# sabarim/STEm-Seg

Measured on AMD Instinct MI355X. Metric: clips/sec (T=8, 480p) embed+cluster, higher is better.
Workload: dtype f16x3: fp32 emulated from 2 fp16 terms per operand (22-bit operand significands; fp32 has 24), power-of-two operand scaling, 3 fp16 MFMA products per fp32 product, fp32 accumulate; |activation| >= 2.6e5 -> non-finite, flagged on the device, clip re-run in bf16x6

## Files before the change

### include/stemseg_hip.h

```cpp
#ifndef STEMSEG_HIP_H
#define STEMSEG_HIP_H

#include <stddef.h>
#include <stdint.h>

#ifdef __cplusplus
extern "C" {
#endif

#define STEMSEG_HIP_ABI_VERSION 11

#define STEMSEG_OK              0
#define STEMSEG_E_INVALID      -1
#define STEMSEG_E_HIP          -2
#define STEMSEG_E_WORKSPACE    -3
#define STEMSEG_E_UNSUPPORTED  -4

#define STEMSEG_MAX_HEAD_OUT   10
#define STEMSEG_MAX_INSTANCES  64
#define STEMSEG_MAX_EMB_DIMS    8
#define STEMSEG_MAX_SEMSEG_CLASSES 128

int         stemseg_hip_version(void);
const char* stemseg_hip_last_error(void);
// ... 62 lines not shown
int stemseg_hip_heads(const float* x, int32_t Cin, int32_t T, int32_t H, int32_t W,
                      const float* w, const float* bias, int32_t n_out, const int32_t* act_host,
                      const int32_t* grid_axis_host, const float* grid_t, const float* grid_y, const float* grid_x,
                      float* out, void* stream);

int stemseg_hip_nonfinite_flags(const float* x, int64_t n, int32_t* flags, int32_t n_flags, void* stream);

typedef struct StemsegDecoderDesc {
    int32_t struct_bytes;
    int32_t in_channels;
    int32_t inter[4];
    int32_t T, H4, W4;
    int32_t gn_groups;
    float   gn_eps;
    int32_t pool[3];
    int32_t t_scale[3];
    int32_t n_out;
    int32_t act[STEMSEG_MAX_EMB_DIMS * 2];
    int32_t grid_axis[STEMSEG_MAX_EMB_DIMS * 2];
    int32_t input_layout;
    int32_t concurrency;
    int32_t detached;
    int32_t precision;
    int32_t n_clips;
    int64_t feat_clip_stride[4];
    int64_t out_clip_stride;
} StemsegDecoderDesc;

typedef struct StemsegDecoderWeights {
    const float* conv_w[7];
    const float* conv_b[7];
    const float* gn_w[7];
    const float* gn_b[7];
    const float* fuse_w[3];
    const float* head_w;
    const float* head_b;
    const float* grid_t;
    const float* grid_y;
    const float* grid_x;
} StemsegDecoderWeights;

size_t stemseg_hip_decoder_workspace_bytes(const StemsegDecoderDesc* desc);
int stemseg_hip_decoder_init_workspace(const StemsegDecoderDesc* desc, void* workspace, size_t ws_bytes, void* stream);
int stemseg_hip_decoder_check_workspace(const StemsegDecoderDesc* desc, const void* workspace, size_t ws_bytes, int32_t* n_bad_host,
                                        int64_t* first_bad_host, void* stream);
int stemseg_hip_decoder_forward(const StemsegDecoderDesc* desc, const StemsegDecoderWeights* weights,
                                const float* const feats[4], float* out,
                                void* workspace, size_t ws_bytes, void* stream);

int stemseg_hip_decoder_join(int32_t concurrency, void* stream);

#define STEMSEG_MAX_ENCODER_BLOCKS 40

typedef struct StemsegEncoderDesc {
    int32_t struct_bytes;
    int32_t blocks[4];
    int32_t T, H, W;
    int32_t out_channels;
    int32_t precision;
    int32_t n_clips;
    int32_t clip_frames;
    int32_t clip_stride;
    int32_t plan_frames;
    int32_t fuse_tail;
    int32_t conv2_groups;
    int32_t width_per_group;
    int32_t stride_in_3x3;
} StemsegEncoderDesc;

typedef struct StemsegEncoderWeights {
    const float* stem_w;
    const float* stem_b;
    const float* stem_w_s2d;
    const float* conv1_w[STEMSEG_MAX_ENCODER_BLOCKS];   const float* conv1_b[STEMSEG_MAX_ENCODER_BLOCKS];
    const float* conv2_w[STEMSEG_MAX_ENCODER_BLOCKS];   const float* conv2_b[STEMSEG_MAX_ENCODER_BLOCKS];
    const float* conv3_w[STEMSEG_MAX_ENCODER_BLOCKS];   const float* conv3_b[STEMSEG_MAX_ENCODER_BLOCKS];
    const float* down_w[STEMSEG_MAX_ENCODER_BLOCKS];    const float* down_b[STEMSEG_MAX_ENCODER_BLOCKS];
    const float* fpn_inner_w[4]; const float* fpn_inner_b[4];
    const float* fpn_layer_w[4]; const float* fpn_layer_b[4];
} StemsegEncoderWeights;

size_t stemseg_hip_encoder_workspace_bytes(const StemsegEncoderDesc* desc);
int stemseg_hip_encoder_plan_offsets(const StemsegEncoderDesc* desc, int64_t* out25);

int stemseg_hip_stem_conv(const float* frames, const float* w_tap_major, const float* bias, float* out, int32_t T, int32_t H, int32_t W,
                          void* stream);
int stemseg_hip_encoder_init_workspace(const StemsegEncoderDesc* desc, void* workspace, size_t ws_bytes, void* stream);
int stemseg_hip_encoder_check_workspace(const StemsegEncoderDesc* desc, const void* workspace, size_t ws_bytes, int32_t* n_bad_host,
                                        int64_t* first_bad_host, void* stream);
int stemseg_hip_encoder_forward(const StemsegEncoderDesc* desc, const StemsegEncoderWeights* weights, const float* frames,
                                const StemsegVolume* out, void* workspace, size_t ws_bytes, void* stream);


int stemseg_hip_seediness_accumulate(float* acc, const float* plane, int64_t n, int32_t first, void* stream);
int stemseg_hip_fg_mask(const float* acc, float count, float thr, uint8_t* mask, int64_t n, void* stream);
int stemseg_hip_fg_mask_frames(const float* acc, const float* counts, float thr, uint8_t* mask, int32_t F, int64_t HW,
                               void* stream);

int stemseg_hip_fg_gather(const float* emb, const float* bw, const float* seed, const uint8_t* fg,
                          int32_t E, int32_t Ev, int32_t T, int64_t HW,
                          float* emb_out, float* bw_out, float* seed_out, int32_t* voxel_index,
                          int64_t* frame_offsets, void* scratch, void* stream);

typedef struct StemsegClusterParams {
    float   primary_prob_thresh;
    float   secondary_prob_thresh;
    float   min_seediness_prob;
    int32_t max_instances;
    int32_t n_free_dims;
    float   free_dim_bandwidths[STEMSEG_MAX_EMB_DIMS];
} StemsegClusterParams;

typedef struct StemsegClusterMeta {
    int32_t K;
    int32_t exhausted;
    int64_t n_points;
    int64_t n_unassigned_last;
    float   centers[STEMSEG_MAX_INSTANCES][STEMSEG_MAX_EMB_DIMS];
    float   bandwidths[STEMSEG_MAX_INSTANCES][STEMSEG_MAX_EMB_DIMS];
    float   seed_prob[STEMSEG_MAX_INSTANCES];
} StemsegClusterMeta;

size_t stemseg_hip_cluster_workspace_bytes(int64_t n_max);
int stemseg_hip_cluster(const float* emb, const float* bw, const float* seed, int64_t n_max,
                        const int64_t* n_points_dev, int32_t E, int32_t Ev,
                        const StemsegClusterParams* params, int64_t label_start,
                        int64_t* labels, StemsegClusterMeta* meta_dev,
                        uint8_t* opt_masks, float* opt_probs,
                        void* workspace, size_t ws_bytes, void* stream);

typedef struct StemsegClusterItem {
    const float*   emb;
    const float*   bw;
    const float*   seed;
    int64_t        n_max;
    const int64_t* n_points_dev;
    int64_t        label_start;
    int64_t*       labels;
    StemsegClusterMeta* meta_dev;
    uint8_t*       opt_masks;
    float*         opt_probs;
    void*          workspace;
    size_t         ws_bytes;
} StemsegClusterItem;
int stemseg_hip_cluster_batch(const StemsegClusterItem* items, int32_t n_items, int32_t E, int32_t Ev,
                              const StemsegClusterParams* params, void* stream);

int stemseg_hip_overlap_counts(const int64_t* labels_a, const int64_t* labels_b, int64_t n,
                               const int32_t* lut_a, int32_t lut_a_len, const int32_t* lut_b, int32_t lut_b_len,
                               int32_t Ka, int32_t Kb, int64_t* inter, int64_t* cnt_a, int64_t* cnt_b, void* stream);

int stemseg_hip_label_presence(const int64_t* labels, int64_t n, uint8_t* present, int32_t cap,
                               int64_t* max_plus_1, int32_t accumulate, void* stream);

int stemseg_hip_relabel(int64_t* labels, int64_t n, const int64_t* map, int32_t map_len, void* stream);


int stemseg_hip_fg_compact(const uint8_t* fg, int32_t T, int64_t HW, int32_t* voxel_index, int64_t* frame_offsets, void* scratch,
                           void* stream);

int stemseg_hip_labels_to_codes(const int64_t* labels, const int32_t* voxel_index, const int64_t* n_points_dev, int64_t n_max,
                                int64_t label_start, uint8_t* codes, int64_t V, void* stream);

int stemseg_hip_pair_tables(const uint8_t* codes, const int32_t* plane_a, const int32_t* plane_b, int32_t n_items, int64_t HW,
                            int32_t B, int32_t* tables, void* stream);

// ... 131 lines not shown
```

### stem-seg_amd/csrc/bottleneck_fused.hip

```cpp
#include "common.h"
#include "split_operand.h"

namespace stemseg {

typedef float f32x16 __attribute__((ext_vector_type(16)));
typedef _Float16 f16x8 __attribute__((ext_vector_type(8)));
typedef unsigned int u32x4 __attribute__((ext_vector_type(4)));

struct FusedTailParams {
    const unsigned int* x16;
    const char* w3;
    const float* b3;
    const float* res;
    float* y;
    const char* w1;
    const float* b1;
    float* z;
    int64_t z_cs, z_ts, z_ys;
    int dec_H, dec_W;
    int V;
    const float* xs;
    const char* wd;
    const float* bd;
};

constexpr SplitLayout FT_WL = SplitLayout(1, STEMSEG_PRECISION_F16X3);
static_assert(FT_WL.CK == 32 && FT_WL.G == 2 && FT_WL.NPL == 2, "the fused tail walks 32-channel chunks of two k-groups, two planes");

template <int MID_, int CT_, int P_, int DS_ = 0>
struct FusedTailCfg {
    static constexpr int MID = MID_, CT = CT_, COUT = 4 * MID_;
    static constexpr int DS = DS_, NCD = DS_ / 32;
    static constexpr int P = P_, NW = P_ / 32, NTHREADS = 64 * NW;
    static constexpr int NC3 = MID / 32;
    static constexpr int NCT = COUT / CT;
    static constexpr int MI3 = CT / 32, MI1 = MID / 32;
    static constexpr int NH = 2 * MI3;
    static constexpr int X_BYTES = 2 * 4 * P * 16;
    static constexpr int W3_BYTES = 8 * CT * 16;
    static constexpr int W1_HALF = 4 * MID * 16;
    static constexpr int LDS_BYTES = 2 * X_BYTES + 2 * W3_BYTES + 2 * W1_HALF;
    static constexpr int NQ = P / 64;
    static constexpr int X_PIECES = X_BYTES / 1024, W3_PIECES = W3_BYTES / 1024, W1_PIECES = W1_HALF / 1024;
    static_assert(NC3 == FT_WL.chunks(MID) && W3_BYTES == FT_WL.slab_bytes(CT, 32) && W1_HALF * FT_WL.G == FT_WL.slab_bytes(MID, 32), "tile byte sizes follow the packed-weight layout");
    static_assert(P % 64 == 0 && MID % 32 == 0 && CT % 32 == 0 && COUT % CT == 0, "tile shapes");
    static_assert(LDS_BYTES <= (P <= 128 ? 80 : 160) * 1024, "LDS: two 128-position workgroups, or one 256-position workgroup, per CU");
    static_assert(W3_BYTES % 1024 == 0 && W1_HALF % 1024 == 0 && X_PIECES % NW == 0, "whole DMA pieces");
    static_assert(MI1 * 16 + MI3 * 16 + (DS ? MI3 * 16 : 0) <= 176, "accumulators must leave room for fragments at 256 registers");
    static_assert(DS % 32 == 0 && 2 * CT * 4 <= W1_HALF, "shortcut: whole K-chunks; its (1 / scale, bias) table waits in a w1 buffer");
};

template <class C>
__global__ __launch_bounds__(C::NTHREADS, 2) void fused_tail_kernel(const FusedTailParams p) {
#pragma clang fp contract(off)
    __shared__ __attribute__((aligned(1024))) char smem[C::LDS_BYTES];
    char* const xbuf = smem;
    char* const w3buf = smem + 2 * C::X_BYTES;
    char* const w1buf = smem + 2 * C::X_BYTES + 2 * C::W3_BYTES;

    const int tid = threadIdx.x, lane = tid & 63;
    const int wave = __builtin_amdgcn_readfirstlane(tid >> 6);
    const int half = lane >> 5, l31 = lane & 31;
    const int pos0 = blockIdx.x * C::P;
    const int pos = pos0 + wave * 32 + l31;
    const bool pos_ok = pos < p.V;
    const int pos_c = min(pos, p.V - 1);
    const int64_t V = p.V;
    const unsigned int lane_off = (unsigned int)(((int64_t)(4 * half) * V + pos_c) * 4);
    auto opaque = [](unsigned int v) __attribute__((always_inline)) { asm volatile("" : "+v"(v)); return v; };

    typedef const __attribute__((address_space(1))) void* gptr_t;
    typedef __attribute__((address_space(3))) void* lptr_t;
    const float* inv3 = reinterpret_cast<const float*>(p.w3 + FT_WL.inv_offset(C::COUT, C::MID));
    const float* inv1 = reinterpret_cast<const float*>(p.w1 + FT_WL.inv_offset(C::MID, C::COUT));

    const int xpos = min(pos0 + lane, p.V - 1);
    auto dma_x = [&](const int c, const int buf) __attribute__((always_inline)) {
#pragma unroll
        for (int k = 0; k < C::X_PIECES / C::NW; ++k) {
            const int idx = wave * (C::X_PIECES / C::NW) + k, q = idx % C::NQ, o = (idx / C::NQ) & 3, pl = idx / (4 * C::NQ);
            const unsigned int xp = (unsigned int)min((int)opaque((unsigned int)xpos) + q * 64, p.V - 1);
            const char* src = reinterpret_cast<const char*>(p.x16) + ((int64_t)(pl * (C::MID / 8) + 4 * c + o)) * V * 16 + (size_t)(xp * 16u);
            __builtin_amdgcn_global_load_lds((gptr_t)src, (lptr_t)(xbuf + buf * C::X_BYTES + ((pl * 4 + o) * C::P + q * 64) * 16), 16, 0, 0);
        }
    };
    auto dma_wc = [&](const char* blob, const int j, const int c, const int buf) __attribute__((always_inline)) {
        constexpr int PER_ROW = C::CT * 16 / 1024;
#pragma unroll
        for (int k = 0; k < (C::W3_PIECES + C::NW - 1) / C::NW; ++k) {
            const int idx = wave + k * C::NW;
            if (idx < C::W3_PIECES) {
                const int row = idx / PER_ROW, part = idx % PER_ROW;
                const char* src = blob + ((int64_t)c * 8 + row) * (C::COUT * 16) + (int64_t)j * (C::CT * 16) + part * 1024 + (size_t)(opaque((unsigned int)lane) * 16u);
                __builtin_amdgcn_global_load_lds((gptr_t)src, (lptr_t)(w3buf + buf * C::W3_BYTES + idx * 1024), 16, 0, 0);
            }
        }
    };
    auto dma_w3 = [&](const int j, const int c, const int buf) __attribute__((always_inline)) { dma_wc(p.w3, j, c, buf); };
    auto dma_wd = [&](const int j, const int c, const int buf) __attribute__((always_inline)) { dma_wc(p.wd, j, c, buf); };
    auto dma_w1 = [&](const int j, const int h, const int buf) __attribute__((always_inline)) {
#pragma unroll
        for (int k = 0; k < (C::W1_PIECES + C::NW - 1) / C::NW; ++k) {
            const int idx = wave + k * C::NW;
            if (idx < C::W1_PIECES) {
                const char* src = p.w1 + ((int64_t)j * C::NH + h) * C::W1_HALF + (int64_t)idx * 1024 + (size_t)(opaque((unsigned int)lane) * 16u);
                __builtin_amdgcn_global_load_lds((gptr_t)src, (lptr_t)(w1buf + buf * C::W1_HALF + idx * 1024), 16, 0, 0);
            }
        }
    };
    auto dma_tab = [&](const int j, const int buf) __attribute__((always_inline)) {
        static_assert(2 * (C::CT / 4) <= 64 && 2 * C::CT * 4 <= C::W3_BYTES, "the table is one DMA piece");
        if (wave == 0 && lane < 2 * (C::CT / 4)) {
            const unsigned int l = opaque((unsigned int)lane);
            const float* src = (l < C::CT / 4 ? inv3 : p.b3 - C::CT) + (int64_t)j * C::CT + (size_t)(l * 4u);
            __builtin_amdgcn_global_load_lds((gptr_t)src, (lptr_t)(w3buf + buf * C::W3_BYTES), 16, 0, 0);
        }
    };
    auto dma_dtab = [&](const int j) __attribute__((always_inline)) {
        if (wave == 0 && lane < 2 * (C::CT / 4)) {
            const unsigned int l = opaque((unsigned int)lane);
            const float* invd = reinterpret_cast<const float*>(p.wd + FT_WL.inv_offset(C::COUT, C::DS));
            const float* src = (l < C::CT / 4 ? invd : p.bd - C::CT) + (int64_t)j * C::CT + (size_t)(l * 4u);
            __builtin_amdgcn_global_load_lds((gptr_t)src, (lptr_t)(w1buf + C::W1_HALF), 16, 0, 0);
        }
    };
    constexpr int NXS = C::DS > 0 ? C::DS / 2 : 1;
    auto load_xs = [&](float (&xr)[NXS]) __attribute__((always_inline)) {
        const unsigned int V4 = (unsigned int)p.V * 4u;
        const __amdgpu_buffer_rsrc_t rs = __builtin_amdgcn_make_buffer_rsrc(const_cast<float*>(p.xs), 0, (int)((unsigned int)C::DS * V4), 0x00020000);
        const unsigned int off = (unsigned int)(8 * half) * V4 + (unsigned int)pos_c * 4u;
#pragma unroll
        for (int i = 0; i < C::DS / 2; ++i)
            xr[i] = __builtin_bit_cast(float, __builtin_amdgcn_raw_buffer_load_b32(rs, off, (unsigned int)(16 * (i >> 3) + (i & 7)) * V4, 0));
    };
    auto dma_tail_tab = [&]() __attribute__((always_inline)) {
        constexpr int PIECES = (2 * C::MID + 255) / 256;
        if (wave < PIECES) {
            const unsigned int f0 = (unsigned int)wave * 256u + opaque((unsigned int)lane) * 4u;
            if (f0 < 2u * C::MID) {
                const float* src = (f0 < (unsigned int)C::MID ? inv1 : p.b1 - C::MID) + (size_t)f0;
                __builtin_amdgcn_global_load_lds((gptr_t)src, (lptr_t)(xbuf + wave * 1024), 16, 0, 0);
            }
        }
    };
    auto stage_sync = [&]() __attribute__((always_inline)) {
        __builtin_amdgcn_s_waitcnt(0x0f70);
        __syncthreads();
    };
    auto load_identity = [&](const int co_first, float (&rres)[16]) __attribute__((always_inline)) {
#pragma unroll
        for (int r = 0; r < 16; ++r)
            rres[r] = *reinterpret_cast<const float*>(reinterpret_cast<const char*>(p.res + (int64_t)(co_first + (r & 3) + 8 * (r >> 2)) * V) + (size_t)lane_off);
    };

    f32x16 acc1[C::MI1];
#pragma unroll
    for (int m = 0; m < C::MI1; ++m)
#pragma unroll
        for (int r = 0; r < 16; ++r) acc1[m][r] = 0.f;

    const f16x8 k2048 = {(_Float16)(1.0f / F16X3_LO_SCALE), (_Float16)(1.0f / F16X3_LO_SCALE), (_Float16)(1.0f / F16X3_LO_SCALE), (_Float16)(1.0f / F16X3_LO_SCALE),
                         (_Float16)(1.0f / F16X3_LO_SCALE), (_Float16)(1.0f / F16X3_LO_SCALE), (_Float16)(1.0f / F16X3_LO_SCALE), (_Float16)(1.0f / F16X3_LO_SCALE)};

    auto mma3 = [&](f32x16& acc, const f16x8 a_hi, const f16x8 a_lo, const f16x8 b_hi, const f16x8 b_lo) __attribute__((always_inline)) {
        const f16x8 a_his = a_hi * k2048;
        acc = __builtin_amdgcn_mfma_f32_32x32x16_f16(a_lo, b_hi, acc, 0, 0, 0);
        acc = __builtin_amdgcn_mfma_f32_32x32x16_f16(a_his, b_lo, acc, 0, 0, 0);
        acc = __builtin_amdgcn_mfma_f32_32x32x16_f16(a_hi, b_hi, acc, 0, 0, 0);
    };

    constexpr bool DSV = C::DS > 0;
    float xr[NXS];
    if constexpr (DSV) { dma_wd(0, 0, 0); load_xs(xr); }
    else { dma_x(0, 0); dma_w3(0, 0, 0); }
    stage_sync();
    int sb = 0;
#pragma unroll 1
    for (int j = 0; j < C::NCT; ++j) {
        f32x16 accd[DSV ? C::MI3 : 1];
        if constexpr (DSV) {
            f16x8 d_hi[2 * C::NCD], d_lo[2 * C::NCD];
#pragma unroll
            for (int G = 0; G < 2 * C::NCD; ++G) {
                u32x4 hw4, lw4;
#pragma unroll
                for (int i = 0; i < 4; ++i) {
                    unsigned int hwd, lwd;
                    split_pair_f16(xr[8 * G + 2 * i], xr[8 * G + 2 * i + 1], hwd, lwd);
                    hw4[i] = hwd; lw4[i] = lwd;
                }
                d_hi[G] = __builtin_bit_cast(f16x8, hw4);
                d_lo[G] = __builtin_bit_cast(f16x8, lw4);
            }
#pragma unroll
            for (int m = 0; m < C::MI3; ++m)
#pragma unroll
                for (int r = 0; r < 16; ++r) accd[m][r] = 0.f;
#pragma unroll
            for (int c = 0; c < C::NCD; ++c) {
                if (c + 1 < C::NCD) dma_wd(j, c + 1, sb ^ 1);
                else { dma_x(0, sb ^ 1); dma_w3(j, 0, sb ^ 1); }
                if (c == 0) dma_dtab(j);
                const char* wb = w3buf + sb * C::W3_BYTES + (half * C::CT + l31) * 16;
                constexpr int NS = 2 * C::MI3;
                f16x8 a_hi[2], a_lo[2];
                auto ld_a = [&](const int st, const int k) __attribute__((always_inline)) {
                    const int g = st / C::MI3, m = st % C::MI3;
                    a_hi[k] = *reinterpret_cast<const f16x8*>(wb + (((g * 2 + 0) * 2) * C::CT + m * 32) * 16);
                    a_lo[k] = *reinterpret_cast<const f16x8*>(wb + (((g * 2 + 1) * 2) * C::CT + m * 32) * 16);
                };
                ld_a(0, 0);
#pragma unroll
                for (int st = 0; st < NS; ++st) {
                    if (st + 1 < NS) ld_a(st + 1, (st + 1) & 1);
                    __builtin_amdgcn_sched_barrier(0);
                    mma3(accd[st % C::MI3], a_hi[st & 1], a_lo[st & 1], d_hi[2 * c + st / C::MI3], d_lo[2 * c + st / C::MI3]);
                    __builtin_amdgcn_sched_barrier(0);
                }
                stage_sync();
                sb ^= 1;
            }
            const float* dtab = reinterpret_cast<const float*>(w1buf + C::W1_HALF);
#pragma unroll
            for (int m = 0; m < C::MI3; ++m)
#pragma unroll
                for (int q = 0; q < 4; ++q) {
                    const float4 sc = *reinterpret_cast<const float4*>(dtab + m * 32 + 8 * q + 4 * half);
                    const float4 bv = *reinterpret_cast<const float4*>(dtab + C::CT + m * 32 + 8 * q + 4 * half);
                    accd[m][4 * q + 0] = __fadd_rn(__fmul_rn(accd[m][4 * q + 0], sc.x), bv.x);
                    accd[m][4 * q + 1] = __fadd_rn(__fmul_rn(accd[m][4 * q + 1], sc.y), bv.y);
                    accd[m][4 * q + 2] = __fadd_rn(__fmul_rn(accd[m][4 * q + 2], sc.z), bv.z);
                    accd[m][4 * q + 3] = __fadd_rn(__fmul_rn(accd[m][4 * q + 3], sc.w), bv.w);
                }
#pragma unroll
            for (int m = 0; m < C::MI3; ++m) asm volatile("" : "+v"(accd[m]));
            __builtin_amdgcn_sched_barrier(0);
        }
        f32x16 acc3[C::MI3];
#pragma unroll
        for (int m = 0; m < C::MI3; ++m)
#pragma unroll
            for (int r = 0; r < 16; ++r) acc3[m][r] = 0.f;
        const int co_j = j * C::CT;
        float rres[16];
#pragma unroll 1
        for (int c = 0; c < C::NC3; ++c) {
            if (c + 1 < C::NC3) { dma_x(c + 1, sb ^ 1); dma_w3(j, c + 1, sb ^ 1); }
            else { dma_w1(j, 0, 0); dma_tab(j, sb ^ 1); if constexpr (!DSV) load_identity(co_j, rres); }
            const char* xb = xbuf + sb * C::X_BYTES + (half * C::P + wave * 32 + l31) * 16;
            const char* wb = w3buf + sb * C::W3_BYTES + (half * C::CT + l31) * 16;
            constexpr int NS = 2 * C::MI3;
            f16x8 b_hi[2], b_lo[2], a_hi[2], a_lo[2];
            auto ld_b = [&](const int g, const int k) __attribute__((always_inline)) {
                b_hi[k] = *reinterpret_cast<const f16x8*>(xb + ((0 * 4 + 2 * g) * C::P) * 16);
                b_lo[k] = *reinterpret_cast<const f16x8*>(xb + ((1 * 4 + 2 * g) * C::P) * 16);
            };
            auto ld_a = [&](const int st, const int k) __attribute__((always_inline)) {
                const int g = st / C::MI3, m = st % C::MI3;
                a_hi[k] = *reinterpret_cast<const f16x8*>(wb + (((g * 2 + 0) * 2) * C::CT + m * 32) * 16);
                a_lo[k] = *reinterpret_cast<const f16x8*>(wb + (((g * 2 + 1) * 2) * C::CT + m * 32) * 16);
            };
            ld_b(0, 0);
            ld_b(1, 1);
            ld_a(0, 0);
#pragma unroll
            for (int st = 0; st < NS; ++st) {
                if (st + 1 < NS) ld_a(st + 1, (st + 1) & 1);
                __builtin_amdgcn_sched_barrier(0);
                mma3(acc3[st % C::MI3], a_hi[st & 1], a_lo[st & 1], b_hi[st / C::MI3], b_lo[st / C::MI3]);
                __builtin_amdgcn_sched_barrier(0);
            }
            stage_sync();
            sb ^= 1;
        }
        f16x8 b_hi[2], b_lo[2];
#pragma unroll
        for (int h = 0; h < C::NH; ++h) {
            const int m = h >> 1, g = h & 1;
            if (g == 0) {
                const int co_m = co_j + m * 32;
                unsigned int hw[8], lw[8];
                const float* tab = reinterpret_cast<const float*>(w3buf + sb * C::W3_BYTES);
                if constexpr (DSV) {
#pragma unroll
                    for (int r = 0; r < 16; ++r) rres[r] = accd[m][r];
                }
                __builtin_amdgcn_sched_barrier(0);
#pragma unroll
                for (int q = 0; q < 4; ++q) {
                    const int co4 = co_m + 8 * q + 4 * half;
                    const float4 sc = *reinterpret_cast<const float4*>(tab + (co4 - co_j));
                    const float4 bv = *reinterpret_cast<const float4*>(tab + C::CT + (co4 - co_j));
                    float v0 = __fmul_rn(acc3[m][4 * q + 0], sc.x), v1 = __fmul_rn(acc3[m][4 * q + 1], sc.y), v2 = __fmul_rn(acc3[m][4 * q + 2], sc.z),
                          v3 = __fmul_rn(acc3[m][4 * q + 3], sc.w);
                    v0 = relu_keep_nan(__fadd_rn(__fadd_rn(v0, bv.x), rres[4 * q + 0]));
                    v1 = relu_keep_nan(__fadd_rn(__fadd_rn(v1, bv.y), rres[4 * q + 1]));
                    v2 = relu_keep_nan(__fadd_rn(__fadd_rn(v2, bv.z), rres[4 * q + 2]));
                    v3 = relu_keep_nan(__fadd_rn(__fadd_rn(v3, bv.w), rres[4 * q + 3]));
                    if (pos_ok) {
                        char* yo = reinterpret_cast<char*>(p.y + (int64_t)(co_m + 8 * q) * V);
                        *reinterpret_cast<float*>(yo + (size_t)lane_off) = v0;
                        *reinterpret_cast<float*>(yo + V * 4 + (size_t)lane_off) = v1;
                        *reinterpret_cast<float*>(yo + V * 8 + (size_t)lane_off) = v2;
                        *reinterpret_cast<float*>(yo + V * 12 + (size_t)lane_off) = v3;
                    }
                    split_pair_f16(v0, v1, hw[2 * q], lw[2 * q]);
                    split_pair_f16(v2, v3, hw[2 * q + 1], lw[2 * q + 1]);
                }
                __builtin_amdgcn_sched_barrier(0);
#pragma unroll
                for (int gg = 0; gg < 2; ++gg) {
                    unsigned int xh[2], yh[2], xl[2], yl[2];
#pragma unroll
                    for (int i = 0; i < 2; ++i) {
                        auto sh = __builtin_amdgcn_permlane32_swap(hw[4 * gg + i], hw[4 * gg + 2 + i], false, false);
                        xh[i] = sh[0]; yh[i] = sh[1];
                        auto sl = __builtin_amdgcn_permlane32_swap(lw[4 * gg + i], lw[4 * gg + 2 + i], false, false);
                        xl[i] = sl[0]; yl[i] = sl[1];
                    }
                    const u32x4 bh = {xh[0], xh[1], yh[0], yh[1]}, bl = {xl[0], xl[1], yl[0], yl[1]};
                    b_hi[gg] = __builtin_bit_cast(f16x8, bh);
                    b_lo[gg] = __builtin_bit_cast(f16x8, bl);
                }
            } else if (m + 1 < C::MI3) {
                if constexpr (!DSV) load_identity(co_j + (m + 1) * 32, rres);
            }
            __builtin_amdgcn_sched_barrier(0);
            if (h + 1 < C::NH) dma_w1(j, h + 1, (h + 1) & 1);
            else if (j + 1 < C::NCT) {
                if constexpr (DSV) { dma_wd(j + 1, 0, sb); load_xs(xr); }
                else { dma_x(0, sb); dma_w3(j + 1, 0, sb); }
            } else dma_tail_tab();
            const char* w1b = w1buf + (h & 1) * C::W1_HALF + (half * C::MID + l31) * 16;
            f16x8 a_hi[2], a_lo[2];
            auto ld_a1 = [&](const int m1, const int k) __attribute__((always_inline)) {
                a_hi[k] = *reinterpret_cast<const f16x8*>(w1b + ((0 * 2) * C::MID + m1 * 32) * 16);
                a_lo[k] = *reinterpret_cast<const f16x8*>(w1b + ((1 * 2) * C::MID + m1 * 32) * 16);
            };
            ld_a1(0, 0);
#pragma unroll
            for (int m1 = 0; m1 < C::MI1; ++m1) {
                if (m1 + 1 < C::MI1) ld_a1(m1 + 1, (m1 + 1) & 1);
                __builtin_amdgcn_sched_barrier(0);
                mma3(acc1[m1], a_hi[m1 & 1], a_lo[m1 & 1], b_hi[g], b_lo[g]);
                __builtin_amdgcn_sched_barrier(0);
            }
            stage_sync();
        }
    }
    if (pos_ok) {
        const int hwp = p.dec_H * p.dec_W;
        const int t2 = pos / hwp, r2 = pos - t2 * hwp, y2 = r2 / p.dec_W, x2 = r2 - y2 * p.dec_W;
        const unsigned int z_off = (unsigned int)(((int64_t)(4 * half) * p.z_cs + (int64_t)t2 * p.z_ts + (int64_t)y2 * p.z_ys + x2) * 4);
#pragma unroll
        for (int m1 = 0; m1 < C::MI1; ++m1)
#pragma unroll
            for (int q = 0; q < 4; ++q) {
                const int co4 = m1 * 32 + 8 * q + 4 * half;
                const float4 sc = *reinterpret_cast<const float4*>(reinterpret_cast<const float*>(xbuf) + co4);
                const float4 bv = *reinterpret_cast<const float4*>(reinterpret_cast<const float*>(xbuf) + C::MID + co4);
                char* zo = reinterpret_cast<char*>(p.z + (int64_t)(m1 * 32 + 8 * q) * p.z_cs);
                *reinterpret_cast<float*>(zo + (size_t)z_off) = relu_keep_nan(__fadd_rn(__fmul_rn(acc1[m1][4 * q + 0], sc.x), bv.x));
                *reinterpret_cast<float*>(zo + p.z_cs * 4 + (size_t)z_off) = relu_keep_nan(__fadd_rn(__fmul_rn(acc1[m1][4 * q + 1], sc.y), bv.y));
                *reinterpret_cast<float*>(zo + p.z_cs * 8 + (size_t)z_off) = relu_keep_nan(__fadd_rn(__fmul_rn(acc1[m1][4 * q + 2], sc.z), bv.z));
                *reinterpret_cast<float*>(zo + p.z_cs * 12 + (size_t)z_off) = relu_keep_nan(__fadd_rn(__fmul_rn(acc1[m1][4 * q + 3], sc.w), bv.w));
            }
    }
}


typedef float f32x4 __attribute__((ext_vector_type(4)));

template <int MID_>
struct FusedTail16Cfg {
    static constexpr int MID = MID_, COUT = 4 * MID_, CT = 128;
    static constexpr int NW = 8, NTHREADS = 512, P = 16 * NW;
    static constexpr int NC3 = MID / 32, NCT = COUT / CT;
    static constexpr int NT3 = CT / 16, NT1 = MID / 16;
    static constexpr int SC = 2;
    static constexpr int NS = NC3 / SC, NU = CT / 32;
    static constexpr int W3_CHUNK = 8 * CT * 16;
    static constexpr int W3_BYTES = SC * W3_CHUNK;
    static constexpr int W1_BYTES = 8 * MID * 16;
    static constexpr int TAB_BYTES = 2 * CT * 4;
    static constexpr int LDS_BYTES = 2 * W3_BYTES + 2 * W1_BYTES + 2 * TAB_BYTES;
    static_assert(NC3 % SC == 0 && W3_BYTES % (1024 * NW) == 0 && W1_BYTES % (1024 * NW) == 0 && TAB_BYTES == 1024, "whole DMA pieces per wave");
    static_assert(W3_CHUNK == FT_WL.slab_bytes(CT, FT_WL.CK) && W1_BYTES == FT_WL.slab_bytes(MID, FT_WL.CK), "tile byte sizes follow the packed-weight layout");
    static_assert(LDS_BYTES <= 160 * 1024 && 2 * MID * 4 <= W3_BYTES, "LDS");
};

template <class C>
__global__ __launch_bounds__(C::NTHREADS, 2) void fused_tail16_kernel(const FusedTailParams p) {
#pragma clang fp contract(off)
    __shared__ __attribute__((aligned(1024))) char smem[C::LDS_BYTES];
    char* const w3buf = smem;
    char* const w1buf = smem + 2 * C::W3_BYTES;
    char* const tabbuf = smem + 2 * C::W3_BYTES + 2 * C::W1_BYTES;

    const int tid = threadIdx.x, lane = tid & 63;
    const int wave = __builtin_amdgcn_readfirstlane(tid >> 6);
    const int n = lane & 15, kb = lane >> 4;
    const int pos = blockIdx.x * C::P + wave * 16 + n;
    const bool pos_ok = pos < p.V;
    const int pos_c = min(pos, p.V - 1);
    const int64_t V = p.V;
    const unsigned int lane_off = (unsigned int)(((int64_t)(4 * kb) * V + pos_c) * 4);
    auto opaque = [](unsigned int v) __attribute__((always_inline)) { asm volatile("" : "+v"(v)); return v; };
    typedef const __attribute__((address_space(1))) void* gptr_t;
    typedef __attribute__((address_space(3))) void* lptr_t;
    const float* inv3 = reinterpret_cast<const float*>(p.w3 + FT_WL.inv_offset(C::COUT, C::MID));
    const float* inv1 = reinterpret_cast<const float*>(p.w1 + FT_WL.inv_offset(C::MID, C::COUT));

    auto dma_w3 = [&](const int j, const int st, const int buf) __attribute__((always_inline)) {
        constexpr int PER_ROW = C::CT * 16 / 1024, PER_CHUNK = C::W3_CHUNK / 1024;
#pragma unroll
        for (int k = 0; k < C::W3_BYTES / 1024 / C::NW; ++k) {
            const int idx = wave + k * C::NW, sc = idx / PER_CHUNK, r = idx % PER_CHUNK, row = r / PER_ROW, part = r % PER_ROW;
            const char* src = p.w3 + ((int64_t)(st * C::SC + sc) * 8 + row) * (C::COUT * 16) + (int64_t)j * (C::CT * 16) + part * 1024 + (size_t)(opaque((unsigned int)lane) * 16u);
            __builtin_amdgcn_global_load_lds((gptr_t)src, (lptr_t)(w3buf + buf * C::W3_BYTES + idx * 1024), 16, 0, 0);
        }
    };
    auto dma_w1 = [&](const int cc, const int buf) __attribute__((always_inline)) {
#pragma unroll
        for (int k = 0; k < C::W1_BYTES / 1024 / C::NW; ++k) {
            const int idx = wave + k * C::NW;
            const char* src = p.w1 + (int64_t)cc * C::W1_BYTES + (int64_t)idx * 1024 + (size_t)(opaque((unsigned int)lane) * 16u);
            __builtin_amdgcn_global_load_lds((gptr_t)src, (lptr_t)(w1buf + buf * C::W1_BYTES + idx * 1024), 16, 0, 0);
        }
    };
    auto dma_tab = [&](const int j) __attribute__((always_inline)) {
        if (wave == 0) {
            const unsigned int l = opaque((unsigned int)lane);
            const float* src = (l < 32 ? inv3 : p.b3 - C::CT) + (int64_t)j * C::CT + (size_t)(l * 4u);
            __builtin_amdgcn_global_load_lds((gptr_t)src, (lptr_t)(tabbuf + (j & 1) * C::TAB_BYTES), 16, 0, 0);
        }
    };
    auto dma_tail_tab = [&]() __attribute__((always_inline)) {
        constexpr int PIECES = (2 * C::MID + 255) / 256;
        if (wave < PIECES) {
            const unsigned int f0 = (unsigned int)wave * 256u + opaque((unsigned int)lane) * 4u;
            if (f0 < 2u * C::MID) {
                const float* src = (f0 < (unsigned int)C::MID ? inv1 : p.b1 - C::MID) + (size_t)f0;
                __builtin_amdgcn_global_load_lds((gptr_t)src, (lptr_t)(w3buf + wave * 1024), 16, 0, 0);
            }
        }
    };
    auto stage_sync = [&]() __attribute__((always_inline)) {
        __builtin_amdgcn_s_waitcnt(0x0f70);
// ... 74 lines not shown
#pragma unroll
            for (int tt = 0; tt < 2; ++tt) {
                const int t = 2 * u + tt, co4 = 16 * t + 4 * kb;
                const float4 sc = *reinterpret_cast<const float4*>(tab + co4);
                const float4 bv = *reinterpret_cast<const float4*>(tab + C::CT + co4);
                float v0 = __fmul_rn(acc3[t][0], sc.x), v1 = __fmul_rn(acc3[t][1], sc.y), v2 = __fmul_rn(acc3[t][2], sc.z), v3 = __fmul_rn(acc3[t][3], sc.w);
                v0 = relu_keep_nan(__fadd_rn(__fadd_rn(v0, bv.x), rres[4 * tt + 0]));
                v1 = relu_keep_nan(__fadd_rn(__fadd_rn(v1, bv.y), rres[4 * tt + 1]));
                v2 = relu_keep_nan(__fadd_rn(__fadd_rn(v2, bv.z), rres[4 * tt + 2]));
                v3 = relu_keep_nan(__fadd_rn(__fadd_rn(v3, bv.w), rres[4 * tt + 3]));
                if (pos_ok) {
                    char* yo = reinterpret_cast<char*>(p.y + (int64_t)(co_j + 16 * t) * V);
                    *reinterpret_cast<float*>(yo + (size_t)lane_off) = v0;
                    *reinterpret_cast<float*>(yo + V * 4 + (size_t)lane_off) = v1;
                    *reinterpret_cast<float*>(yo + V * 8 + (size_t)lane_off) = v2;
                    *reinterpret_cast<float*>(yo + V * 12 + (size_t)lane_off) = v3;
                }
                split_pair_f16(v0, v1, hw[2 * tt], lw[2 * tt]);
                split_pair_f16(v2, v3, hw[2 * tt + 1], lw[2 * tt + 1]);
            }
            unsigned int bw[2][4];
#pragma unroll
            for (int pl = 0; pl < 2; ++pl)
#pragma unroll
                for (int i = 0; i < 2; ++i) {
                    const unsigned int t0 = pl ? lw[i] : hw[i], t1 = pl ? lw[2 + i] : hw[2 + i];
                    auto s32 = __builtin_amdgcn_permlane32_swap(t0, t1, false, false);
                    auto s16 = __builtin_amdgcn_permlane16_swap(s32[0], s32[1], false, false);
                    bw[pl][i] = s16[0];
                    bw[pl][2 + i] = s16[1];
                }
            const u32x4 bh = {bw[0][0], bw[0][1], bw[0][2], bw[0][3]}, bl = {bw[1][0], bw[1][1], bw[1][2], bw[1][3]};
            const f16x8 b_hi = __builtin_bit_cast(f16x8, bh), b_lo = __builtin_bit_cast(f16x8, bl);
            __builtin_amdgcn_sched_barrier(0);
            if (u + 1 < C::NU) { dma_w1(j * C::NU + u + 1, eb ^ 1); load_identity(co_j + 32 * (u + 1), rres); }
            else if (j + 1 < C::NCT) dma_w3(j + 1, 0, sb);
            else dma_tail_tab();
            __builtin_amdgcn_sched_barrier(0);
            const char* w1b = w1buf + eb * C::W1_BYTES + (((kb >> 1) * 2 * 2 + (kb & 1)) * C::MID + n) * 16;
            f16x8 a_hi[1][2], a_lo[1][2];
            auto ld_a1 = [&](const int i, const int k) __attribute__((always_inline)) {
#pragma unroll
                for (int e = 0; e < 2; ++e) {
                    a_hi[k][e] = *reinterpret_cast<const f16x8*>(w1b + (0 * 2 * C::MID + (2 * i + e) * 16) * 16);
                    a_lo[k][e] = *reinterpret_cast<const f16x8*>(w1b + (1 * 2 * C::MID + (2 * i + e) * 16) * 16);
                }
            };
#pragma unroll
            for (int i = 0; i < C::NT1 / 2; ++i) {
                ld_a1(i, 0);
                __builtin_amdgcn_sched_barrier(0);
                mma3x2(acc1[2 * i], acc1[2 * i + 1], a_hi[0][0], a_lo[0][0], a_hi[0][1], a_lo[0][1], b_hi, b_lo);
                __builtin_amdgcn_sched_barrier(0);
            }
            stage_sync();
            eb ^= 1;
        }
    }
    if (pos_ok) {
        const int hwp = p.dec_H * p.dec_W;
        const int t2 = pos / hwp, r2 = pos - t2 * hwp, y2 = r2 / p.dec_W, x2 = r2 - y2 * p.dec_W;
        const unsigned int z_off = (unsigned int)(((int64_t)(4 * kb) * p.z_cs + (int64_t)t2 * p.z_ts + (int64_t)y2 * p.z_ys + x2) * 4);
        const float* ttab = reinterpret_cast<const float*>(w3buf);
#pragma unroll
        for (int m1 = 0; m1 < C::NT1; ++m1) {
            const int co4 = m1 * 16 + 4 * kb;
            const float4 sc = *reinterpret_cast<const float4*>(ttab + co4);
            const float4 bv = *reinterpret_cast<const float4*>(ttab + C::MID + co4);
            char* zo = reinterpret_cast<char*>(p.z + (int64_t)(m1 * 16) * p.z_cs);
            *reinterpret_cast<float*>(zo + (size_t)z_off) = relu_keep_nan(__fadd_rn(__fmul_rn(acc1[m1][0], sc.x), bv.x));
            *reinterpret_cast<float*>(zo + p.z_cs * 4 + (size_t)z_off) = relu_keep_nan(__fadd_rn(__fmul_rn(acc1[m1][1], sc.y), bv.y));
            *reinterpret_cast<float*>(zo + p.z_cs * 8 + (size_t)z_off) = relu_keep_nan(__fadd_rn(__fmul_rn(acc1[m1][2], sc.z), bv.z));
            *reinterpret_cast<float*>(zo + p.z_cs * 12 + (size_t)z_off) = relu_keep_nan(__fadd_rn(__fmul_rn(acc1[m1][3], sc.w), bv.w));
        }
    }
}


typedef __amdgpu_buffer_rsrc_t ft_rsrc_t;
#define FT_VMCNT_(n) __builtin_amdgcn_s_waitcnt(((n) & 15) | (((n) >> 4) << 14) | 0x0F70)
#define FT_VMCNT(n) FT_VMCNT_(n)
#define FT_SGB(mask, n) __builtin_amdgcn_sched_group_barrier(mask, n, 0)

template <int MID_, int CT_, int DS_ = 0>
struct FusedTailR1Cfg {
    static constexpr int MID = MID_, CT = CT_, COUT = 4 * MID_;
    static constexpr int DS = DS_, NGD = DS_ / 16;
    static constexpr int NW = 4, NTHREADS = 64 * NW, P = 32 * NW;
    static constexpr int NC3 = MID / 32, NG = MID / 16, NCT = COUT / CT;
    static constexpr int MI3 = CT / 32, MI1 = MID / 32;
    static constexpr int SC = 2;
    static constexpr int NS = NC3 / SC, NU = CT / 32;
    static constexpr int NSD = DS / 32 / SC;
    static_assert(DS % (32 * SC) == 0, "shortcut: whole stages");
    static constexpr int NX3 = SC * 2 * (MI3 / 2), NX1 = 2 * (MI1 / 2);
    static constexpr int W3_CHUNK = 8 * CT * 16, W3_BYTES = SC * W3_CHUNK;
    static constexpr int W1_BYTES = 8 * MID * 16;
    static_assert(W3_CHUNK == FT_WL.slab_bytes(CT, FT_WL.CK) && W1_BYTES == FT_WL.slab_bytes(MID, FT_WL.CK), "tile byte sizes follow the packed-weight layout");
    static constexpr int TAB_BYTES = 1024;
    static constexpr int LDS_BYTES = 2 * W3_BYTES + 2 * W1_BYTES + 2 * TAB_BYTES;
    static constexpr int W3_PIECES = W3_BYTES / 1024 / NW, W1_PIECES = W1_BYTES / 1024 / NW;
    static constexpr int SL = 8 / NX1, S0 = NX1 / 4, M_PPS = 8 / S0;
    static_assert(NC3 % SC == 0 && MI3 % 2 == 0 && MI1 % 2 == 0 && W3_BYTES % (1024 * NW) == 0 && W1_BYTES % (1024 * NW) == 0 && 2 * CT * 4 <= TAB_BYTES, "whole DMA pieces per wave");
    static_assert(LDS_BYTES <= 160 * 1024 && 2 * MID * 4 <= W3_BYTES && (NX1 == 8 || NX1 == 4) && NX3 == 8 && MI3 == 4 && NS >= 2 && NU >= 2 && NU % 2 == 0, "LDS / slice placement / identity buffer parity");
    static_assert(W3_PIECES == 8 && W1_PIECES <= 8, "the pieces of a stage are requested in its first steps");
    static_assert(NG * 8 + MI1 * 16 <= 256, "the conv3 input and conv1's accumulators are the AGPR half of the register file");
};

template <class C>
__global__ __launch_bounds__(C::NTHREADS, 1) void fused_tail_r1_kernel(const FusedTailParams p) {
#pragma clang fp contract(off)
    __shared__ __attribute__((aligned(1024))) char smem[C::LDS_BYTES];
    char* const w3buf = smem;
    char* const w1buf = smem + 2 * C::W3_BYTES;
    char* const tabbuf = smem + 2 * C::W3_BYTES + 2 * C::W1_BYTES;

    const int tid = threadIdx.x, lane = tid & 63;
    const int wave = __builtin_amdgcn_readfirstlane(tid >> 6);
    const int half = lane >> 5, l31 = lane & 31;
    const int pos = blockIdx.x * C::P + wave * 32 + l31;
    const bool pos_ok = pos < p.V;
    const int pos_c = min(pos, p.V - 1);
    const int64_t V = p.V;
    const unsigned int V4 = (unsigned int)p.V * 4u;
    const unsigned int lane_ld = (unsigned int)(4 * half) * V4 + (unsigned int)pos_c * 4u;
    const unsigned int lane_st = pos_ok ? lane_ld : 0xFFFFFF00u;
    const unsigned int tile_bytes = (unsigned int)C::CT * V4;
    typedef __attribute__((address_space(3))) void* lptr_t;
    const float* inv3 = reinterpret_cast<const float*>(p.w3 + FT_WL.inv_offset(C::COUT, C::MID));
    const float* inv1 = reinterpret_cast<const float*>(p.w1 + FT_WL.inv_offset(C::MID, C::COUT));

    const unsigned int lane16 = (unsigned int)lane * 16u;
    const unsigned int lds_w3 = (unsigned int)(uintptr_t)(lptr_t)w3buf, lds_w1 = (unsigned int)(uintptr_t)(lptr_t)w1buf;
    auto dma_piece = [&](const char* sbase, const unsigned int lds_addr) __attribute__((always_inline)) {
        asm volatile("s_mov_b32 m0, %0\n\ts_nop 0\n\tglobal_load_lds_dwordx4 %1, %2" : : "s"(lds_addr), "v"(lane16), "s"(sbase) : "memory");
    };
    auto dma_w3 = [&](const int j, const int st, const int buf, const int k) __attribute__((always_inline)) {
        constexpr int PER_ROW = C::CT * 16 / 1024, PER_CHUNK = C::W3_CHUNK / 1024;
        const int idx = wave + k * C::NW, sc = idx / PER_CHUNK, r = idx % PER_CHUNK, row = r / PER_ROW, part = r % PER_ROW;
        dma_piece(p.w3 + ((int64_t)(st * C::SC + sc) * 8 + row) * (C::COUT * 16) + (int64_t)j * (C::CT * 16) + part * 1024, lds_w3 + buf * C::W3_BYTES + idx * 1024);
    };
    auto dma_wd = [&](const int j, const int st, const int buf, const int k) __attribute__((always_inline)) {
        constexpr int PER_ROW = C::CT * 16 / 1024, PER_CHUNK = C::W3_CHUNK / 1024;
        const int idx = wave + k * C::NW, sc = idx / PER_CHUNK, r = idx % PER_CHUNK, row = r / PER_ROW, part = r % PER_ROW;
        dma_piece(p.wd + ((int64_t)(st * C::SC + sc) * 8 + row) * (C::COUT * 16) + (int64_t)j * (C::CT * 16) + part * 1024, lds_w3 + buf * C::W3_BYTES + idx * 1024);
    };
    auto dma_w1 = [&](const int cc, const int buf, const int k) __attribute__((always_inline)) {
        const int idx = wave + k * C::NW;
        dma_piece(p.w1 + (int64_t)cc * C::W1_BYTES + (int64_t)idx * 1024, lds_w1 + buf * C::W1_BYTES + idx * 1024);
    };
    float4 tabv = {0.f, 0.f, 0.f, 0.f};
    auto tab_fetch = [&](const int j) __attribute__((always_inline)) {
        if (wave == 0 && lane < 2 * (C::CT / 4))
            tabv = *reinterpret_cast<const float4*>((lane < C::CT / 4 ? inv3 : p.b3 - C::CT) + (int64_t)j * C::CT + lane * 4);
    };
    auto tab_store = [&](const int j) __attribute__((always_inline)) {
        if (wave == 0 && lane < 2 * (C::CT / 4)) *reinterpret_cast<float4*>(tabbuf + (j & 1) * C::TAB_BYTES + lane * 16) = tabv;
    };
    constexpr bool DSV = C::DS > 0;
    float4 tabdv = {0.f, 0.f, 0.f, 0.f};
    auto tabd_fetch = [&](const int j) __attribute__((always_inline)) {
        const float* invd = reinterpret_cast<const float*>(p.wd + FT_WL.inv_offset(C::COUT, C::DS));
        if (wave == 0 && lane < 2 * (C::CT / 4))
            tabdv = *reinterpret_cast<const float4*>((lane < C::CT / 4 ? invd : p.bd - C::CT) + (int64_t)j * C::CT + lane * 4);
    };
    auto tabd_store = [&](const int j) __attribute__((always_inline)) {
        if (wave == 0 && lane < 2 * (C::CT / 4)) *reinterpret_cast<float4*>(tabbuf + ((j + 1) & 1) * C::TAB_BYTES + lane * 16) = tabdv;
    };
    auto rsrc_of = [&](const float* base, const int jj) __attribute__((always_inline)) {
        return __builtin_amdgcn_make_buffer_rsrc(const_cast<float*>(base + (int64_t)jj * C::CT * V), 0, (int)tile_bytes, 0x00020000);
    };
    auto load_identity = [&](const int jj, const int u, float (&rr)[16]) __attribute__((always_inline)) {
        const ft_rsrc_t rs = rsrc_of(p.res, jj);
#pragma unroll
        for (int r = 0; r < 16; ++r)
            rr[r] = __builtin_bit_cast(float, __builtin_amdgcn_raw_buffer_load_b32(rs, lane_ld, (unsigned int)(32 * u + (r & 3) + 8 * (r >> 2)) * V4, 0));
    };
    const f16x8 k2048 = {(_Float16)(1.0f / F16X3_LO_SCALE), (_Float16)(1.0f / F16X3_LO_SCALE), (_Float16)(1.0f / F16X3_LO_SCALE), (_Float16)(1.0f / F16X3_LO_SCALE),
                         (_Float16)(1.0f / F16X3_LO_SCALE), (_Float16)(1.0f / F16X3_LO_SCALE), (_Float16)(1.0f / F16X3_LO_SCALE), (_Float16)(1.0f / F16X3_LO_SCALE)};
    auto mma6 = [&](f32x16& c0, f32x16& c1, const f16x8 (&a_hi)[2], const f16x8 (&a_lo)[2], const f16x8 (&a_his)[2], const f16x8 b_hi, const f16x8 b_lo)
        __attribute__((always_inline)) {
        c0 = __builtin_amdgcn_mfma_f32_32x32x16_f16(a_lo[0], b_hi, c0, 0, 0, 0);
        c1 = __builtin_amdgcn_mfma_f32_32x32x16_f16(a_lo[1], b_hi, c1, 0, 0, 0);
        c0 = __builtin_amdgcn_mfma_f32_32x32x16_f16(a_his[0], b_lo, c0, 0, 0, 0);
        c1 = __builtin_amdgcn_mfma_f32_32x32x16_f16(a_his[1], b_lo, c1, 0, 0, 0);
        c0 = __builtin_amdgcn_mfma_f32_32x32x16_f16(a_hi[0], b_hi, c0, 0, 0, 0);
        c1 = __builtin_amdgcn_mfma_f32_32x32x16_f16(a_hi[1], b_hi, c1, 0, 0, 0);
    };

#pragma unroll
    for (int k = 0; k < C::W3_PIECES; ++k) {
        if constexpr (DSV) dma_wd(0, 0, 0, k);
        else dma_w3(0, 0, 0, k);
    }
    float rres[2][16];
    if constexpr (!DSV) {
        load_identity(0, 0, rres[0]);
        load_identity(0, 1, rres[1]);
    }
    f16x8 xh[C::NG], xl[C::NG];
    {
        const char* xs = reinterpret_cast<const char*>(p.x16) + (size_t)((unsigned int)pos_c * 16u);
#pragma unroll
        for (int G = 0; G < C::NG; ++G) {
            xh[G] = *reinterpret_cast<const f16x8*>(xs + ((int64_t)(2 * G + half)) * V * 16);
            xl[G] = *reinterpret_cast<const f16x8*>(xs + ((int64_t)(C::MID / 8 + 2 * G + half)) * V * 16);
        }
    }
    f16x8 xdh[DSV ? C::NGD : 1], xdl[DSV ? C::NGD : 1];
    if constexpr (DSV) {
        const ft_rsrc_t rx = __builtin_amdgcn_make_buffer_rsrc(const_cast<float*>(p.xs), 0, (int)((unsigned int)C::DS * V4), 0x00020000);
        const unsigned int lane_xs = (unsigned int)(8 * half) * V4 + (unsigned int)pos_c * 4u;
#pragma unroll
// ... 14 lines not shown
    }
    f32x16 acc1[C::MI1];
#pragma unroll
    for (int m = 0; m < C::MI1; ++m)
#pragma unroll
        for (int r = 0; r < 16; ++r) acc1[m][r] = 0.f;
    FT_VMCNT(0);
    __syncthreads();
    int sb = 0, eb = 0;
#pragma unroll 1
    for (int j = 0; j < C::NCT; ++j) {
        f32x16 accd[DSV ? C::MI3 : 1];
        if constexpr (DSV) {
#pragma unroll
            for (int m = 0; m < C::MI3; ++m)
#pragma unroll
                for (int r = 0; r < 16; ++r) accd[m][r] = 0.f;
#pragma unroll
            for (int st = 0; st < C::NSD; ++st) {
                if (st == 0) tabd_fetch(j);
                const char* wb = w3buf + sb * C::W3_BYTES + (half * C::CT + l31) * 16;
                f16x8 a_hi[3][2], a_lo[3][2], a_his[2][2];
                auto ld3 = [&](const int s, const int k) __attribute__((always_inline)) {
                    const int mp = s / (2 * C::SC), sc = (s % (2 * C::SC)) / 2, g = s % 2;
#pragma unroll
                    for (int e = 0; e < 2; ++e) {
                        a_hi[k][e] = *reinterpret_cast<const f16x8*>(wb + sc * C::W3_CHUNK + (((g * 2 + 0) * 2) * C::CT + (2 * mp + e) * 32) * 16);
                        a_lo[k][e] = *reinterpret_cast<const f16x8*>(wb + sc * C::W3_CHUNK + (((g * 2 + 1) * 2) * C::CT + (2 * mp + e) * 32) * 16);
                    }
                };
                ld3(0, 0);
                ld3(1, 1);
                a_his[0][0] = a_hi[0][0] * k2048;
                a_his[0][1] = a_hi[0][1] * k2048;
#pragma unroll
                for (int s = 0; s < C::NX3; ++s) {
                    __builtin_amdgcn_sched_barrier(0);
                    if (s < 2) {
#pragma unroll
                        for (int k = 4 * s; k < 4 * s + 4; ++k) {
                            if (st + 1 < C::NSD) dma_wd(j, st + 1, sb ^ 1, k);
                            else dma_w3(j, 0, sb ^ 1, k);
                        }
                    }
                    if (s + 2 < C::NX3) ld3(s + 2, (s + 2) % 3);
                    if (s + 1 < C::NX3) {
                        a_his[(s + 1) & 1][0] = a_hi[(s + 1) % 3][0] * k2048;
                        a_his[(s + 1) & 1][1] = a_hi[(s + 1) % 3][1] * k2048;
                    }
                    const int mp = s / (2 * C::SC), sc = (s % (2 * C::SC)) / 2, g = s % 2, G = 2 * (st * C::SC + sc) + g;
                    mma6(accd[2 * mp], accd[2 * mp + 1], a_hi[s % 3], a_lo[s % 3], a_his[s & 1], xdh[G], xdl[G]);
#pragma unroll
                    for (int i = 0; i < 6; ++i) { FT_SGB(0x008, 1); FT_SGB(0x100, 1); FT_SGB(0x002, 2); }
                }
                __builtin_amdgcn_sched_barrier(0);
                FT_VMCNT(0);
                if (st == 0) tabd_store(j);
                __syncthreads();
                sb ^= 1;
            }
            const float* tabd = reinterpret_cast<const float*>(tabbuf + ((j + 1) & 1) * C::TAB_BYTES) + 4 * half;
#pragma unroll
            for (int u = 0; u < C::MI3; ++u)
#pragma unroll
                for (int q4 = 0; q4 < 4; ++q4) {
                    const float4 sc = *reinterpret_cast<const float4*>(tabd + 32 * u + 8 * q4);
                    const float4 bv = *reinterpret_cast<const float4*>(tabd + C::CT + 32 * u + 8 * q4);
                    accd[u][4 * q4 + 0] = __fadd_rn(__fmul_rn(accd[u][4 * q4 + 0], sc.x), bv.x);
                    accd[u][4 * q4 + 1] = __fadd_rn(__fmul_rn(accd[u][4 * q4 + 1], sc.y), bv.y);
                    accd[u][4 * q4 + 2] = __fadd_rn(__fmul_rn(accd[u][4 * q4 + 2], sc.z), bv.z);
                    accd[u][4 * q4 + 3] = __fadd_rn(__fmul_rn(accd[u][4 * q4 + 3], sc.w), bv.w);
                }
#pragma unroll
            for (int u = 0; u < C::MI3; ++u) asm volatile("" : "+v"(accd[u]));
            __builtin_amdgcn_sched_barrier(0);
        }
        f32x16 acc3[C::MI3];
#pragma unroll
        for (int m = 0; m < C::MI3; ++m)
#pragma unroll
            for (int r = 0; r < 16; ++r) acc3[m][r] = 0.f;
        const float* tab = reinterpret_cast<const float*>(tabbuf + (j & 1) * C::TAB_BYTES) + 4 * half;
        const ft_rsrc_t ry = rsrc_of(p.y, j);
        unsigned int hw[8], lw[8];
        f16x8 b_hi[2][2], b_lo[2][2];
        auto e_slice = [&](const int u, const int q4) __attribute__((always_inline)) {
            const int c4 = 32 * u + 8 * q4;
            const float4 sc = *reinterpret_cast<const float4*>(tab + c4);
            const float4 bv = *reinterpret_cast<const float4*>(tab + C::CT + c4);
            float rr[4];
#pragma unroll
            for (int i = 0; i < 4; ++i) rr[i] = DSV ? accd[DSV ? u : 0][4 * q4 + i] : rres[u & 1][4 * q4 + i];
            float v0 = __fmul_rn(acc3[u][4 * q4 + 0], sc.x), v1 = __fmul_rn(acc3[u][4 * q4 + 1], sc.y), v2 = __fmul_rn(acc3[u][4 * q4 + 2], sc.z),
                  v3 = __fmul_rn(acc3[u][4 * q4 + 3], sc.w);
            v0 = relu_keep_nan(__fadd_rn(__fadd_rn(v0, bv.x), rr[0]));
            v1 = relu_keep_nan(__fadd_rn(__fadd_rn(v1, bv.y), rr[1]));
            v2 = relu_keep_nan(__fadd_rn(__fadd_rn(v2, bv.z), rr[2]));
            v3 = relu_keep_nan(__fadd_rn(__fadd_rn(v3, bv.w), rr[3]));
            __builtin_amdgcn_raw_buffer_store_b32(__builtin_bit_cast(unsigned int, v0), ry, lane_st, (unsigned int)(c4 + 0) * V4, 0);
            __builtin_amdgcn_raw_buffer_store_b32(__builtin_bit_cast(unsigned int, v1), ry, lane_st, (unsigned int)(c4 + 1) * V4, 0);
            __builtin_amdgcn_raw_buffer_store_b32(__builtin_bit_cast(unsigned int, v2), ry, lane_st, (unsigned int)(c4 + 2) * V4, 0);
            __builtin_amdgcn_raw_buffer_store_b32(__builtin_bit_cast(unsigned int, v3), ry, lane_st, (unsigned int)(c4 + 3) * V4, 0);
            split_pair_f16(v0, v1, hw[2 * q4], lw[2 * q4]);
            split_pair_f16(v2, v3, hw[2 * q4 + 1], lw[2 * q4 + 1]);
        };
        auto e_perm = [&](const int gg, f16x8& bh, f16x8& bl) __attribute__((always_inline)) {
            unsigned int xh_[2], yh_[2], xl_[2], yl_[2];
#pragma unroll
            for (int i = 0; i < 2; ++i) {
                auto sh = __builtin_amdgcn_permlane32_swap(hw[4 * gg + i], hw[4 * gg + 2 + i], false, false);
                xh_[i] = sh[0]; yh_[i] = sh[1];
                auto sl = __builtin_amdgcn_permlane32_swap(lw[4 * gg + i], lw[4 * gg + 2 + i], false, false);
                xl_[i] = sl[0]; yl_[i] = sl[1];
            }
            const u32x4 bh4 = {xh_[0], xh_[1], yh_[0], yh_[1]}, bl4 = {xl_[0], xl_[1], yl_[0], yl_[1]};
            bh = __builtin_bit_cast(f16x8, bh4);
            bl = __builtin_bit_cast(f16x8, bl4);
        };
#pragma unroll
        for (int st = 0; st < C::NS; ++st) {
            if (st + 2 == C::NS) tab_fetch(j);
            const char* wb = w3buf + sb * C::W3_BYTES + (half * C::CT + l31) * 16;
            f16x8 a_hi[3][2], a_lo[3][2], a_his[2][2];
            auto ld3 = [&](const int s, const int k) __attribute__((always_inline)) {
                const int mp = s / (2 * C::SC), sc = (s % (2 * C::SC)) / 2, g = s % 2;
#pragma unroll
                for (int e = 0; e < 2; ++e) {
                    a_hi[k][e] = *reinterpret_cast<const f16x8*>(wb + sc * C::W3_CHUNK + (((g * 2 + 0) * 2) * C::CT + (2 * mp + e) * 32) * 16);
                    a_lo[k][e] = *reinterpret_cast<const f16x8*>(wb + sc * C::W3_CHUNK + (((g * 2 + 1) * 2) * C::CT + (2 * mp + e) * 32) * 16);
                }
            };
            ld3(0, 0);
            ld3(1, 1);
            a_his[0][0] = a_hi[0][0] * k2048;
            a_his[0][1] = a_hi[0][1] * k2048;
#pragma unroll
            for (int s = 0; s < C::NX3; ++s) {
                __builtin_amdgcn_sched_barrier(0);
                if (s < 2) {
#pragma unroll
                    for (int k = 4 * s; k < 4 * s + 4; ++k) {
                        if (st + 1 < C::NS) dma_w3(j, st + 1, sb ^ 1, k);
                        else if (k < C::W1_PIECES) dma_w1(j * C::NU, eb, k);
                    }
                }
                if (s + 2 < C::NX3) ld3(s + 2, (s + 2) % 3);
                if (s + 1 < C::NX3) {
                    a_his[(s + 1) & 1][0] = a_hi[(s + 1) % 3][0] * k2048;
                    a_his[(s + 1) & 1][1] = a_hi[(s + 1) % 3][1] * k2048;
                }
                if (st + 1 == C::NS && s >= C::NX3 / 2) e_slice(0, s - C::NX3 / 2);
                const int mp = s / (2 * C::SC), sc = (s % (2 * C::SC)) / 2, g = s % 2, G = 2 * (st * C::SC + sc) + g;
                mma6(acc3[2 * mp], acc3[2 * mp + 1], a_hi[s % 3], a_lo[s % 3], a_his[s & 1], xh[G], xl[G]);
#pragma unroll
                for (int i = 0; i < 6; ++i) {
                    FT_SGB(0x008, 1); FT_SGB(0x100, 1);
                    if (st + 1 == C::NS && s >= C::NX3 / 2) { FT_SGB(0x002, 7); FT_SGB(0x040, 1); }
                    else FT_SGB(0x002, 2);
                }
            }
            __builtin_amdgcn_sched_barrier(0);
            if (st + 1 == C::NS) FT_VMCNT(16);
            else FT_VMCNT(0);
            if (st + 2 == C::NS) tab_store(j);
            __syncthreads();
            sb ^= 1;
        }
        e_perm(0, b_hi[0][0], b_lo[0][0]);
        e_perm(1, b_hi[0][1], b_lo[0][1]);
#pragma unroll
        for (int u = 0; u < C::NU; ++u) {
            const char* w1b = w1buf + eb * C::W1_BYTES + (half * C::MID + l31) * 16;
            f16x8 a_hi[3][2], a_lo[3][2], a_his[2][2];
            auto ld1 = [&](const int s, const int k) __attribute__((always_inline)) {
                const int g = s / (C::MI1 / 2), mp = s % (C::MI1 / 2);
#pragma unroll
                for (int e = 0; e < 2; ++e) {
                    a_hi[k][e] = *reinterpret_cast<const f16x8*>(w1b + (((g * 2 + 0) * 2) * C::MID + (2 * mp + e) * 32) * 16);
                    a_lo[k][e] = *reinterpret_cast<const f16x8*>(w1b + (((g * 2 + 1) * 2) * C::MID + (2 * mp + e) * 32) * 16);
                }
            };
            ld1(0, 0);
            ld1(1, 1);
            a_his[0][0] = a_hi[0][0] * k2048;
            a_his[0][1] = a_hi[0][1] * k2048;
#pragma unroll
            for (int s = 0; s < C::NX1; ++s) {
                __builtin_amdgcn_sched_barrier(0);
                if (s < C::S0) {
#pragma unroll
                    for (int k = C::M_PPS * s; k < C::M_PPS * s + C::M_PPS; ++k) {
                        if (u + 1 < C::NU) { if (k < C::W1_PIECES) dma_w1(j * C::NU + u + 1, eb ^ 1, k); }
                        else if (j + 1 < C::NCT) { if constexpr (DSV) dma_wd(j + 1, 0, sb, k); else dma_w3(j + 1, 0, sb, k); }
                    }
                }
                if (!DSV && s == C::S0) load_identity(u + 2 < C::NU ? j : min(j + 1, C::NCT - 1), (u + 2) % C::NU, rres[u & 1]);
                if (s + 2 < C::NX1) ld1(s + 2, (s + 2) % 3);
                if (s + 1 < C::NX1) {
                    a_his[(s + 1) & 1][0] = a_hi[(s + 1) % 3][0] * k2048;
                    a_his[(s + 1) & 1][1] = a_hi[(s + 1) % 3][1] * k2048;
                }
                if (u + 1 < C::NU) {
                    constexpr int SE = C::S0 + 4 / C::SL;
                    if (s >= C::S0 && s < SE) {
#pragma unroll
                        for (int q = 0; q < C::SL; ++q) e_slice(u + 1, (s - C::S0) * C::SL + q);
                    }
                    if (C::SL == 1 ? s == SE : s == SE) e_perm(0, b_hi[(u + 1) & 1][0], b_lo[(u + 1) & 1][0]);
                    if (C::SL == 1 ? s == SE + 1 : s == SE) e_perm(1, b_hi[(u + 1) & 1][1], b_lo[(u + 1) & 1][1]);
                }
                const int g = s / (C::MI1 / 2), mp = s % (C::MI1 / 2);
                mma6(acc1[2 * mp], acc1[2 * mp + 1], a_hi[s % 3], a_lo[s % 3], a_his[s & 1], b_hi[u & 1][g], b_lo[u & 1][g]);
#pragma unroll
                for (int i = 0; i < 6; ++i) { FT_SGB(0x008, 1); FT_SGB(0x100, 1); FT_SGB(0x002, 7 * C::SL); FT_SGB(0x040, C::SL); FT_SGB(0x020, 3); }
            }
            __builtin_amdgcn_sched_barrier(0);
            if (u + 1 < C::NU) FT_VMCNT(DSV ? 16 : 32);
            else FT_VMCNT(DSV ? 0 : 16);
            __syncthreads();
            eb ^= 1;
        }
    }
    static_assert(C::MID / 4 <= 64, "one lane per four channels");
    if (wave < 2 && lane < C::MID / 4)
        *reinterpret_cast<float4*>(w3buf + wave * (C::MID * 4) + lane * 16) = *reinterpret_cast<const float4*>((wave == 0 ? inv1 : p.b1) + lane * 4);
    __syncthreads();
    if (pos_ok) {
        const int hwp = p.dec_H * p.dec_W;
        const int t2 = pos / hwp, r2 = pos - t2 * hwp, y2 = r2 / p.dec_W, x2 = r2 - y2 * p.dec_W;
        const unsigned int z_off = (unsigned int)(((int64_t)(4 * half) * p.z_cs + (int64_t)t2 * p.z_ts + (int64_t)y2 * p.z_ys + x2) * 4);
        const float* ttab = reinterpret_cast<const float*>(w3buf);
#pragma unroll
        for (int m1 = 0; m1 < C::MI1; ++m1)
#pragma unroll
            for (int q = 0; q < 4; ++q) {
                const int co4 = m1 * 32 + 8 * q + 4 * half;
                const float4 sc = *reinterpret_cast<const float4*>(ttab + co4);
                const float4 bv = *reinterpret_cast<const float4*>(ttab + C::MID + co4);
                char* zo = reinterpret_cast<char*>(p.z + (int64_t)(m1 * 32 + 8 * q) * p.z_cs);
                *reinterpret_cast<float*>(zo + (size_t)z_off) = relu_keep_nan(__fadd_rn(__fmul_rn(acc1[m1][4 * q + 0], sc.x), bv.x));
                *reinterpret_cast<float*>(zo + p.z_cs * 4 + (size_t)z_off) = relu_keep_nan(__fadd_rn(__fmul_rn(acc1[m1][4 * q + 1], sc.y), bv.y));
                *reinterpret_cast<float*>(zo + p.z_cs * 8 + (size_t)z_off) = relu_keep_nan(__fadd_rn(__fmul_rn(acc1[m1][4 * q + 2], sc.z), bv.z));
                *reinterpret_cast<float*>(zo + p.z_cs * 12 + (size_t)z_off) = relu_keep_nan(__fadd_rn(__fmul_rn(acc1[m1][4 * q + 3], sc.w), bv.w));
            }
    }
}

template <class C>
static int launch_fused_r1_cfg(const FusedTailParams& p, hipStream_t s) {
    const double flops = 2.0 * 2.0 * (double)C::MID * C::COUT * (double)p.V;
    void* ev = profile_begin(19, flops, s);
    hipLaunchKernelGGL(fused_tail_r1_kernel<C>, dim3((unsigned)ceil_div(p.V, C::P)), dim3(C::NTHREADS), 0, s, p);
    profile_end(ev, s);
    SS_LAUNCH_CHECK();
    return STEMSEG_OK;
}

template <class C>
static int launch_fused16_cfg(const FusedTailParams& p, hipStream_t s) {
    const double flops = 2.0 * 2.0 * (double)C::MID * C::COUT * (double)p.V;
    void* ev = profile_begin(19, flops, s);
    hipLaunchKernelGGL(fused_tail16_kernel<C>, dim3((unsigned)ceil_div(p.V, C::P)), dim3(C::NTHREADS), 0, s, p);
    profile_end(ev, s);
    SS_LAUNCH_CHECK();
    return STEMSEG_OK;
}

template <class C>
static int launch_fused_cfg(const FusedTailParams& p, hipStream_t s) {
    const double flops = 2.0 * 2.0 * (double)C::MID * C::COUT * (double)p.V;
    void* ev = profile_begin(19, flops, s);
    hipLaunchKernelGGL(fused_tail_kernel<C>, dim3((unsigned)ceil_div(p.V, C::P)), dim3(C::NTHREADS), 0, s, p);
    profile_end(ev, s);
    SS_LAUNCH_CHECK();
    return STEMSEG_OK;
}

bool fused_tail_supported(int mid) { return mid == 64 || mid == 128 || mid == 256; }

bool fused_shortcut_supported(int mid, int cin, int64_t V) {
    return ((mid == 64 && cin == 64) || (mid == 128 && cin == 256)) && (int64_t)cin * V * 4 < (1ll << 32) - (1 << 20) && (int64_t)128 * V * 4 < (1ll << 32) - (1 << 20);
}

int launch_fused_tail(int mid, const unsigned int* x16, const float* w3, const float* b3, const float* res, float* y, const float* w1, const float* b1,
                      const StemsegVolume& z, int dec_H, int dec_W, int64_t V, int form, hipStream_t s, const float* ds_x, int ds_cin, const float* ds_w,
                      const float* ds_b) {
    SS_CHECK_ARG(x16 && w3 && b3 && y && w1 && b1 && z.ptr, "fused_tail: null pointer");
    SS_CHECK_ARG(ds_x ? (!res && ds_w && ds_b && fused_shortcut_supported(mid, ds_cin, V) && reinterpret_cast<uintptr_t>(ds_w) % 16 == 0 && reinterpret_cast<uintptr_t>(ds_b) % 16 == 0)
                      : res != nullptr, "fused_tail: identity map, or a shortcut (mid %d, %d input channels) this library has a kernel for", mid, ds_cin);
    SS_CHECK_ARG(fused_tail_supported(mid), "fused_tail: mid = %d (64, 128 or 256)", mid);
    SS_CHECK_ARG(V > 0 && V <= (1ll << 27) && z.c_stride <= (1ll << 27) && dec_H > 0 && dec_W > 0 && V % ((int64_t)dec_H * dec_W) == 0, "fused_tail: V = %lld positions of %d x %d planes",
                 (long long)V, dec_H, dec_W);
    SS_CHECK_ARG(z.C == mid, "fused_tail: consumer volume has %d channels, conv1 makes %d", z.C, mid);
    SS_CHECK_ARG(reinterpret_cast<uintptr_t>(x16) % 16 == 0 && reinterpret_cast<uintptr_t>(w3) % 16 == 0 && reinterpret_cast<uintptr_t>(w1) % 16 == 0 &&
                 reinterpret_cast<uintptr_t>(b3) % 16 == 0 && reinterpret_cast<uintptr_t>(b1) % 16 == 0, "fused_tail: 16-byte aligned operands");
    FusedTailParams p;
    p.x16 = x16; p.w3 = reinterpret_cast<const char*>(w3); p.b3 = b3; p.res = res; p.y = y;
    p.w1 = reinterpret_cast<const char*>(w1); p.b1 = b1;
    p.z = z.ptr; p.z_cs = z.c_stride; p.z_ts = z.t_stride; p.z_ys = z.y_stride; p.dec_H = dec_H; p.dec_W = dec_W;
    p.V = (int)V;
    p.xs = ds_x; p.wd = reinterpret_cast<const char*>(ds_w); p.bd = ds_b;
    if (ds_x && mid == 128) return launch_fused_r1_cfg<FusedTailR1Cfg<128, 128, 256>>(p, s);
    if (ds_x) return launch_fused_cfg<FusedTailCfg<64, 128, 128, 64>>(p, s);
    if (mid == 256) {
        const bool r1_fits = (int64_t)128 * V * 4 < (1ll << 32) - (1 << 20);
        if (form != 1 && r1_fits) return launch_fused_r1_cfg<FusedTailR1Cfg<256, 128>>(p, s);
        return launch_fused16_cfg<FusedTail16Cfg<256>>(p, s);
    }
    if (mid == 128 && form != 1 && (int64_t)128 * V * 4 < (1ll << 32) - (1 << 20)) return launch_fused_r1_cfg<FusedTailR1Cfg<128, 128>>(p, s);
    if (mid == 128) return launch_fused_cfg<FusedTailCfg<128, 128, 128>>(p, s);
    return launch_fused_cfg<FusedTailCfg<64, 128, 128>>(p, s);
}

}
```

### stem-seg_amd/csrc/common.h

```cpp
#pragma once
#include <hip/hip_runtime.h>
#include <cstdarg>
#include <cstdint>
#include <cstdio>
#include <cstring>

#include "../../include/stemseg_hip.h"

#if defined(__HIP_DEVICE_COMPILE__) && defined(__AMDGCN_WAVEFRONT_SIZE) && __AMDGCN_WAVEFRONT_SIZE != 64
#error "libstemseg_hip is written for 64-lane wavefronts (gfx950): shuffles, ballots and MFMA layouts assume it"
#endif

namespace stemseg {

void set_error(const char* fmt, ...);

#define SS_CHECK_ARG(cond, ...)                                     \
    do {                                                            \
        if (!(cond)) {                                              \
            ::stemseg::set_error(__VA_ARGS__);                      \
            return STEMSEG_E_INVALID;                               \
        }                                                           \
    } while (0)

#define SS_HIP(call)                                                                            \
    do {                                                                                        \
        hipError_t e_ = (call);                                                                 \
        if (e_ != hipSuccess) {                                                                 \
            ::stemseg::set_error("%s failed: %s (%s:%d)", #call, hipGetErrorString(e_),         \
                                 __FILE__, __LINE__);                                           \
            return STEMSEG_E_HIP;                                                               \
        }                                                                                       \
    } while (0)

#define SS_LAUNCH_CHECK() SS_HIP(hipGetLastError())

static inline hipStream_t as_stream(void* s) { return reinterpret_cast<hipStream_t>(s); }
static inline int64_t ceil_div(int64_t a, int64_t b) { return (a + b - 1) / b; }
static inline int64_t round_up(int64_t a, int64_t b) { return ceil_div(a, b) * b; }

__device__ __forceinline__ float relu_keep_nan(float v) { return v < 0.f ? 0.f : v; }
__device__ __forceinline__ float max_keep_nan(float a, float b) { return (a > b || a != a) ? a : b; }

struct PaddedGeom {
    int64_t pitch, ts, cs, total, interior;
    PaddedGeom() = default;
    PaddedGeom(int C, int T, int H, int W) {
        pitch = round_up((int64_t)W + 2, 4);
        ts = (int64_t)(H + 2) * pitch;
        cs = (int64_t)(T + 2) * ts;
        total = (int64_t)C * cs + 64;
        interior = ts + pitch + 1;
    }
};

static inline StemsegVolume make_volume(float* ptr, int64_t cs, int64_t ts, int64_t ys, int C, int T, int H, int W,
                                        int64_t limit) {
    StemsegVolume v;
    v.ptr = ptr; v.c_stride = cs; v.t_stride = ts; v.y_stride = ys; v.C = C; v.T = T; v.H = H; v.W = W; v.limit = limit;
    return v;
}
static inline StemsegVolume dense_volume(float* ptr, int C, int T, int H, int W) {
    return make_volume(ptr, (int64_t)T * H * W, (int64_t)H * W, W, C, T, H, W, (int64_t)C * T * H * W);
}
static inline StemsegVolume padded_halo_view(float* base, int C, int T, int H, int W) {
    PaddedGeom g(C, T, H, W);
    return make_volume(base, g.cs, g.ts, g.pitch, C, T + 2, H + 2, W + 2, g.total);
}
static inline StemsegVolume padded_interior_view(float* base, int C, int T, int H, int W) {
    PaddedGeom g(C, T, H, W);
    return make_volume(base + g.interior, g.cs, g.ts, g.pitch, C, T, H, W, g.total - g.interior);
}

constexpr int WS_GUARD_FLOATS = 64;
constexpr uint32_t WS_CANARY = 0x7fc5ca7au;
constexpr int WS_MAX_GUARDS = 64;
struct GuardList {
    int n = 0;
    int64_t off[WS_MAX_GUARDS];
    bool full = false;
    void push(int64_t o) { if (n < WS_MAX_GUARDS) off[n++] = o; else full = true; }
};
int launch_canary_fill(float* ws, const GuardList& g, hipStream_t s);
int canary_check(const float* ws, const GuardList& g, int32_t* n_bad_host, int64_t* first_bad_host, hipStream_t s);

void* profile_begin(int tag, double work, hipStream_t s);
void profile_end(void* handle, hipStream_t s);

struct ConvEpilogue {
    int relu = 0;
    const float* res = nullptr;
    int64_t res_cs = 0, res_ts = 0, res_ys = 0;
    int dec_H = 0, dec_W = 0;
    int precision = 0;
    int frames = 0, plan_frames = 0;
    int64_t plan_scratch_floats = 0;
    double* gn_part = nullptr;
    int gn_cpg = 0, gn_cap = 0;
    int* gn_used = nullptr;
    int nb = 1;
    int64_t in_bs = 0, out_bs = 0, gn_bs = 0;
    unsigned int* p16_out = nullptr;
    int* p16_done = nullptr;
    int zero_t_halo = 0;
};
int launch_conv3d(const StemsegVolume& in, const float* packed_w, const float* bias, const StemsegVolume& out,
                  int kt, int kh, int kw, int tile_cfg, hipStream_t s, float* splitk_scratch = nullptr, int64_t splitk_scratch_floats = 0,
                  const ConvEpilogue* epi = nullptr);
int launch_grouped_conv(const StemsegVolume& in, const void* packed_w, const float* bias, const StemsegVolume& out, int groups, int stride,
                        int relu, int precision, hipStream_t s);
bool fused_tail_supported(int mid);
int launch_fused_tail(int mid, const unsigned int* x16, const float* w3, const float* b3, const float* res, float* y, const float* w1, const float* b1,
                      const StemsegVolume& z, int dec_H, int dec_W, int64_t V, int form, hipStream_t s, const float* ds_x = nullptr, int ds_cin = 0,
                      const float* ds_w = nullptr, const float* ds_b = nullptr);
bool fused_shortcut_supported(int mid, int cin, int64_t V);
int launch_gn_stats(const float* x, int C, int64_t S, int groups, float eps, float* stats, double* scratch, hipStream_t s);
constexpr int GN_SLOT_CAP = 32768;
static inline int64_t gn_scratch_doubles(int Cout, int groups) { return (int64_t)groups * GN_SLOT_CAP * 2 > (int64_t)groups * 128 ? (int64_t)groups * GN_SLOT_CAP * 2 : (int64_t)groups * 128; }
int launch_conv3d_gn(const StemsegVolume& in, const float* packed_w, const float* bias, const StemsegVolume& out, int kt, int kh, int kw,
                     int tile_cfg, hipStream_t s, float* splitk_scratch, int64_t splitk_scratch_floats, const ConvEpilogue* epi, int groups,
                     float eps, float* stats, double* gn_scratch, int64_t stats_bs = 0);
int launch_gn_identity_stats(float* stats, int groups, hipStream_t s);
struct ClipBatch {
    int nb = 1;
    int64_t in_bs = 0, out_bs = 0, stats_bs = 0;
};
int launch_gn_finalize_slots(const double* part, int groups, int cap, int used, double group_elems, float eps, float* stats, hipStream_t s,
                             int nb = 1, int64_t part_bs = 0, int64_t stats_bs = 0);
int launch_gn_relu_pool(const float* x, int C, int T, int H, int W, int groups, const float* stats, const float* gamma,
                        const float* beta, int pool, const StemsegVolume& out, hipStream_t s, const ClipBatch& cb = ClipBatch());
int launch_upsample(const float* in, int C, int T, int H, int W, int st, int sy, int sx, const StemsegVolume& out,
                    hipStream_t s, const ClipBatch& cb = ClipBatch());
int launch_copy_to_volume(const float* in, int layout, const StemsegVolume& out, hipStream_t s);
int launch_copy_strided(const float* in, int64_t in_c_stride, int64_t in_t_stride, const StemsegVolume& out, hipStream_t s);
struct HeadSpec {
    int n_out;
    int act[STEMSEG_MAX_EMB_DIMS * 2];
    int grid_axis[STEMSEG_MAX_EMB_DIMS * 2];
};
struct HeadsGN {
    const float* stats;
    const float* gamma;
    const float* beta;
    int cpg;
    int64_t stats_bs;
};
int launch_heads(const float* x, int Cin, int T, int H, int W, const float* w, const float* bias, const HeadSpec& hs,
                 const float* gt, const float* gy, const float* gx, float* out, hipStream_t s, const ClipBatch& cb = ClipBatch(),
                 const float* add = nullptr, int64_t add_bs = 0, const HeadsGN* gn = nullptr);
int launch_level_head(const float* x, int Cin, int64_t V, const float* w, int n_out, const float* add, float* out, hipStream_t s, int nb, int64_t x_bs,
                      int64_t add_bs, int64_t out_bs);

}
```

### stem-seg_amd/csrc/conv_igemm.h

```cpp
#pragma once
#include "common.h"
#include "split_operand.h"
#include <algorithm>
#include <type_traits>

namespace stemseg {

typedef float f32x16 __attribute__((ext_vector_type(16)));

constexpr int MIN_WG4 = 4;

struct ConvKParams {
    const float* in;
    int64_t in_cs, in_ts, in_ys, in_limit;
    int in_H;
    const float* wpk;
    const float* bias;
    float* out;
    int64_t out_cs, out_ts, out_ys;
    int Cin, Cout, T, H, W;
    int tiles_x, tiles_y;
    int vec4;
    int chunks_per_split;
    int64_t out_split_stride;
// ... 879 lines not shown
        }
        if (y < p.H && x < p.W) {
            int64_t off, roff = 0;
            if (p.dec_W > 0) {
                const int hw = p.dec_H * p.dec_W;
                const int t2 = x / hw, r2 = x - t2 * hw, y2 = r2 / p.dec_W, x2 = r2 - y2 * p.dec_W;
                off = (int64_t)t2 * p.out_ts + (int64_t)y2 * p.out_ys + x2;
                roff = (int64_t)t2 * p.res_ts + (int64_t)y2 * p.res_ys + x2;
            } else {
                off = (int64_t)te * p.out_ts + (int64_t)y * p.out_ys + x;
                roff = (int64_t)te * p.res_ts + (int64_t)y * p.res_ys + x;
            }
            if constexpr (C::F16) {
                if (p.out_p16) {
                    const int64_t plane_words = (int64_t)(p.Cout / 8) * p.out_cs * 4;
#pragma unroll
                    for (int mi = 0; mi < C::MI; ++mi)
#pragma unroll
                        for (int q = 0; q < 4; ++q) {
                            const int co4 = co_base + mi * 32 + 8 * q + 4 * half;
                            if (co4 < p.Cout) {
                                float v[4];
#pragma unroll
                                for (int k = 0; k < 4; ++k) {
                                    v[k] = acc[mi][ni][4 * q + k] + (p.bias ? p.bias[co4 + k] : 0.f);
                                    if (p.relu) v[k] = relu_keep_nan(v[k]);
                                }
                                uint2 hw, lw;
                                split_pair_f16(v[0], v[1], hw.x, lw.x);
                                split_pair_f16(v[2], v[3], hw.y, lw.y);
                                unsigned int* d = p.out_p16 + ((int64_t)(co4 / 8) * p.out_cs + off) * 4 + 2 * half;
                                *reinterpret_cast<uint2*>(d) = hw;
                                *reinterpret_cast<uint2*>(d + plane_words) = lw;
                            }
                        }
                    continue;
                }
            }
            float* o = p.out + (int64_t)blockIdx.y * p.out_bs + (int64_t)blockIdx.z * p.out_split_stride + off;
#pragma unroll
            for (int mi = 0; mi < C::MI; ++mi) {
#pragma unroll
                for (int r = 0; r < 16; ++r) {
                    const int co = co_base + mi * 32 + (r & 3) + 8 * (r >> 2) + 4 * half;
                    if (co < p.Cout) {
                        float v = acc[mi][ni][r] + (p.bias ? p.bias[co] : 0.f);
                        if (p.res) v += p.res[(int64_t)co * p.res_cs + roff];
                        if (p.relu) v = relu_keep_nan(v);
                        o[(int64_t)co * p.out_cs] = v;
                    }
                }
            }
        }
    }
}

struct SplitReduceParams {
    const float* partial;
    const float* bias;
    const float* res;
    float* out;
    int64_t out_cs, out_ts, out_ys, res_cs, res_ts, res_ys, slab;
    int C, H, W, ksplit, relu;
    int64_t V;
    unsigned per_c;
    double* gn_part;
    int gn_cpg, gn_cap, gn_slot0;
    int64_t part_bs, out_bs, gn_bs;
};
void launch_splitk_reduce(const SplitReduceParams& rp, bool vec, unsigned blocks_per_channel, unsigned clips, hipStream_t s);

constexpr double CU_FLOPS_F32 = 0.46e12;

struct PlanCtx {
    ConvKParams shape;
    int64_t scratch_floats;
};

struct LaunchCtx {
    hipStream_t s;
    float* scratch;
    int64_t scratch_floats;
    const PlanCtx* plan;
    LaunchCtx without_scratch() const { return LaunchCtx{s, nullptr, 0, plan}; }
    LaunchCtx without_plan() const { return LaunchCtx{s, scratch, scratch_floats, nullptr}; }
};

template <class C>
static int64_t tile_workgroups(const ConvKParams& d, int flat_t = 0) {
    int64_t tx = C::FLAT ? ceil_div((int64_t)d.H * d.in_ys, C::NT) : ceil_div(d.W, C::TW);
    const int64_t ty = C::FLAT ? 1 : ceil_div(d.H, C::ROWS);
    int64_t T = d.T;
    if (C::FLAT && flat_t) { tx = ceil_div((int64_t)d.T * d.in_ts, C::NT); T = 1; }
    return tx * ty * T * ceil_div(d.Cout, C::MT);
}

template <class C>
static int plan_ksplit(const ConvKParams& p, const LaunchCtx& L, int flat_t, int nchunks) {
    int ksplit = 1;
    const PlanCtx* plan = L.plan;
    float* const scratch = L.scratch;
    const ConvKParams& d = plan ? plan->shape : p;
    const int64_t d_T = plan ? d.T : p.T_all;
    ConvKParams dd = d;
    dd.T = (int)d_T;
    const int64_t wgs = tile_workgroups<C>(dd, flat_t);
    const int64_t slab_plan = (int64_t)d.Cout * d_T * d.H * d.W;
    const int64_t plan_scratch = plan ? plan->scratch_floats : L.scratch_floats / p.nb;
    const int64_t wg_target = (C::X6 && C::NWAVES >= 8) ? 320 : 640;
    while (scratch && ksplit * 2 <= 16 && ksplit * 2 <= nchunks && wgs * ksplit * 2 <= wg_target && slab_plan * ksplit * 2 <= plan_scratch) ksplit *= 2;
    if (p.out_p16 && C::F16 && wgs >= 128) ksplit = 1;
    return ksplit;
}

template <class C>
static int launch_cfg(ConvKParams p, const LaunchCtx& L, int force_ksplit = 0) {
    hipStream_t s = L.s;
    float* const scratch = L.scratch;
    const int64_t scratch_floats = L.scratch_floats;
    p.tiles_x = C::FLAT ? (int)ceil_div((int64_t)p.H * p.in_ys, C::NT) : (int)ceil_div(p.W, C::TW);
    p.tiles_y = C::FLAT ? 1 : (int)ceil_div(p.H, C::ROWS);
    p.T_all = p.T;
    const int flat_t = (C::FLAT && p.flat_t) ? 1 : 0;
    if (flat_t) {
        p.tiles_x = (int)ceil_div((int64_t)p.T * p.in_ts, C::NT);
        p.T = 1;
    }
    p.flat_t = flat_t;
    const int out_vec = p.vec_epi;
    if (C::FLAT) p.vec_epi = 0;
    const int nchunks = (int)ceil_div(p.Cin, C::CK);
    const int64_t slab = (int64_t)p.Cout * p.T_all * p.H * p.W;
    int ksplit = plan_ksplit<C>(p, L, flat_t, nchunks);
    if (force_ksplit > 0) ksplit = (scratch && (int64_t)p.nb * force_ksplit * slab <= scratch_floats) ? std::min(force_ksplit, nchunks) : 1;
    p.chunks_per_split = (int)ceil_div(nchunks, ksplit);
    ksplit = (int)ceil_div(nchunks, p.chunks_per_split);
    SS_CHECK_ARG(ksplit == 1 || (int64_t)p.nb * ksplit * slab <= scratch_floats, "conv3d: split-K scratch too small (%lld floats needed, %lld given)",
                 (long long)((int64_t)p.nb * ksplit * slab), (long long)scratch_floats);
    if (p.out_p16) {
        if (ksplit > 1 || !C::F16) p.out_p16 = nullptr;
        else { p.vec_epi = 0; if (p.gn_used_host) *p.gn_used_host = 1; }
    }
    SplitReduceParams rp;
    const bool rp_vec = out_vec && p.dec_W == 0 && (reinterpret_cast<uintptr_t>(scratch) % 16 == 0) && (slab % 4 == 0);
    if (ksplit > 1) {
        rp.partial = scratch; rp.bias = p.bias; rp.res = p.res; rp.out = p.out;
        rp.out_cs = p.out_cs; rp.out_ts = p.out_ts; rp.out_ys = p.out_ys; rp.res_cs = p.res_cs; rp.res_ts = p.res_ts; rp.res_ys = p.res_ys;
        rp.slab = slab; rp.C = p.Cout; rp.V = (int64_t)p.T_all * p.H * p.W; rp.ksplit = ksplit; rp.relu = p.relu;
        rp.H = p.dec_W > 0 ? p.dec_H : p.H; rp.W = p.dec_W > 0 ? p.dec_W : p.W;
        rp.gn_part = nullptr; rp.gn_cpg = rp.gn_cap = rp.gn_slot0 = 0;
        rp.part_bs = (int64_t)ksplit * slab; rp.out_bs = p.out_bs; rp.gn_bs = p.gn_bs;
        p.out_bs = (int64_t)ksplit * slab;
        p.out = scratch; p.bias = nullptr; p.res = nullptr; p.relu = 0; p.dec_H = p.dec_W = 0;
        p.out_cs = (int64_t)p.T_all * p.H * p.W; p.out_ts = (int64_t)p.H * p.W; p.out_ys = p.W;
        p.out_split_stride = slab;
        p.vec_epi = !C::FLAT && (p.W % 4 == 0) && (reinterpret_cast<uintptr_t>(scratch) % 16 == 0);
    } else p.out_split_stride = 0;
    p.n_co = (int)ceil_div(p.Cout, C::MT);
    const int64_t red_items = slab / p.Cout / (rp_vec ? 4 : 1);
    const unsigned red_bx = (unsigned)ceil_div(red_items, 256);
    if (p.gn_part) {
        const int slot0 = *p.gn_used_host;
        const int64_t slots = ksplit > 1 ? (int64_t)p.gn_cpg * red_bx : (int64_t)p.tiles_x * p.tiles_y * p.T;
        SS_CHECK_ARG(slot0 + slots <= p.gn_cap, "conv3d: GroupNorm partial table too small (%lld slots needed, %d available)",
                     (long long)(slot0 + slots), p.gn_cap);
        if (ksplit > 1) { rp.gn_part = p.gn_part; rp.gn_cpg = p.gn_cpg; rp.gn_cap = p.gn_cap; rp.gn_slot0 = slot0; p.gn_part = nullptr; }
        else p.gn_slot0 = slot0;
        *p.gn_used_host = slot0 + (int)slots;
    }
    dim3 grid((unsigned)((int64_t)p.tiles_x * p.tiles_y * p.T * p.n_co), (unsigned)p.nb, (unsigned)ksplit);
    const double flops = 2.0 * p.Cin * C::TAPS * (double)p.Cout * p.T_all * p.H * p.W * p.nb;
    constexpr int tile_rows = (C::FLAT || C::BLK) ? C::NSEG : C::ROWS;
    const int tag = C::TAPS == 16 ? -1 : C::TAPS == 1 ? 10 + C::NSEG : (C::KT == 1 ? 20 + tile_rows : (tile_rows == 16 ? 9 : tile_rows));
    void* ev = profile_begin(tag, flops, s);
    hipLaunchKernelGGL(conv_igemm_kernel<C>, grid, dim3(C::NTHREADS), 0, s, p);
    if (ksplit > 1) {
        SS_CHECK_ARG(red_items < (1ll << 32) - 256 && p.Cout <= 65535, "conv3d: split-K output too large (%lld elements)", (long long)slab);
        rp.per_c = (unsigned)red_items;
        launch_splitk_reduce(rp, rp_vec, red_bx, (unsigned)p.nb, s);
    }
    profile_end(ev, s);
    SS_LAUNCH_CHECK();
    return STEMSEG_OK;
}

struct RowPlan { double cost; int nA, k; };

template <class C>
static RowPlan plan_rows(const ConvKParams& d, bool have_scratch, int64_t scratch_floats, double cu_flops, int occ, double eff) {
    const int64_t slots = 256 * occ;
    const int tiles_x = (int)ceil_div(d.W, C::TW);
    const int n = (int)ceil_div(d.H, C::ROWS);
    const int64_t c = (int64_t)tiles_x * d.T * ceil_div(d.Cout, C::MT);
    const int nchunks = (int)ceil_div(d.Cin, C::CK);
// ... 62 lines not shown
```

### stem-seg_amd/csrc/conv_igemm.hip

```cpp
#include "conv_igemm.h"

namespace stemseg {

template <bool VEC>
__global__ __launch_bounds__(256) void splitk_reduce_kernel(const SplitReduceParams p) {
    constexpr int VW = VEC ? 4 : 1;
    const unsigned wq = (unsigned)p.W / VW;
    const unsigned c = blockIdx.y;
    const unsigned j = blockIdx.x * 256u + threadIdx.x;
    const bool active = j < p.per_c;
    const float* const partial = p.partial + (int64_t)blockIdx.z * p.part_bs;
    float* const outp = p.out + (int64_t)blockIdx.z * p.out_bs;
    float s1 = 0.f, s2 = 0.f;
    if (active) {
        const unsigned r2 = j / wq, x = (j - r2 * wq) * VW;
        const unsigned t = r2 / (unsigned)p.H, y = r2 - t * (unsigned)p.H;
        const int64_t i = (int64_t)c * p.V + (int64_t)r2 * p.W + x;
        const int64_t o = (int64_t)c * p.out_cs + (int64_t)t * p.out_ts + (int64_t)y * p.out_ys + x;
        if constexpr (VEC) {
            float4 acc = *reinterpret_cast<const float4*>(partial + i);
            for (int z = 1; z < p.ksplit; ++z) {
                const float4 v = *reinterpret_cast<const float4*>(partial + (int64_t)z * p.slab + i);
                acc.x += v.x; acc.y += v.y; acc.z += v.z; acc.w += v.w;
            }
// ... 70 lines not shown
template <class GLCfg, class Cfg>
static int launch_gl(const ConvKParams& p, const LaunchCtx& L) {
    if (p.vec4 && p.Cin % GLCfg::CK == 0 && p.Cout % GLCfg::MT == 0) return launch_cfg<GLCfg>(p, L);
    return launch_cfg<Cfg>(p, L);
}

int launch_conv3d(const StemsegVolume& in, const float* packed_w, const float* bias, const StemsegVolume& out,
                  int kt, int kh, int kw, int tile_cfg, hipStream_t s, float* scratch, int64_t scratch_floats, const ConvEpilogue* epi) {
    SS_CHECK_ARG(in.ptr && out.ptr && packed_w, "conv3d: null pointer");
    const int prec = epi ? epi->precision : STEMSEG_PRECISION_F32;
    SS_CHECK_ARG(prec == STEMSEG_PRECISION_F32 || prec == STEMSEG_PRECISION_BF16X6 || prec == STEMSEG_PRECISION_F16X3,
                 "conv3d: precision %d (0 f32, 2 bf16x6, 3 f16x3)", prec);
    const bool k3 = (kt == 3 && kh == 3 && kw == 3), k1 = (kt == 1 && kh == 1 && kw == 1), k2 = (kt == 1 && kh == 3 && kw == 3);
    const bool k4 = (kt == 1 && kh == 4 && kw == 4);
    SS_CHECK_ARG(k3 || k1 || k2 || (k4 && prec == STEMSEG_PRECISION_F16X3), "conv3d: kernel %dx%dx%d unsupported (3x3x3, 1x3x3, 1x1x1; 1x4x4 in f16x3 mode)", kt, kh, kw);
    const bool flat = epi && epi->dec_W > 0;
    if (flat) {
        SS_CHECK_ARG(k1 && in.T == 1 && in.H == 1 && epi->dec_H > 0 && (int64_t)out.T * out.H * out.W == in.W &&
                     out.H == epi->dec_H && out.W == epi->dec_W, "conv3d: flat-decode epilogue needs a 1x1x1 conv on a [C][V] input with V == T*H*W of `out`");
    } else {
        SS_CHECK_ARG(in.T == out.T + kt - 1 && in.H == out.H + kh - 1 && in.W == out.W + kw - 1,
                     "conv3d: input extents (%d,%d,%d) must be output (%d,%d,%d) + kernel - 1", in.T, in.H, in.W, out.T, out.H, out.W);
    }
    SS_CHECK_ARG(in.C % 4 == 0 && out.C % 32 == 0, "conv3d: Cin %% 4 == 0 and Cout %% 32 == 0 required (got %d, %d)", in.C, out.C);
    ConvKParams p;
    p.in = in.ptr; p.in_cs = in.c_stride; p.in_ts = in.t_stride; p.in_ys = in.y_stride; p.in_limit = in.limit; p.in_H = in.H;
    p.wpk = packed_w; p.bias = bias;
    p.out = out.ptr; p.out_cs = out.c_stride; p.out_ts = out.t_stride; p.out_ys = out.y_stride;
    p.Cin = in.C; p.Cout = out.C; p.T = out.T; p.H = out.H; p.W = out.W;
    if (flat) { p.T = 1; p.H = 1; p.W = in.W; }
    p.relu = epi ? epi->relu : 0;
    p.res = epi ? epi->res : nullptr;
    p.res_cs = epi ? epi->res_cs : 0; p.res_ts = epi ? epi->res_ts : 0; p.res_ys = epi ? epi->res_ys : 0;
    p.dec_H = flat ? epi->dec_H : 0; p.dec_W = flat ? epi->dec_W : 0;
    p.gn_part = epi ? epi->gn_part : nullptr;
    p.gn_cpg = epi ? epi->gn_cpg : 0; p.gn_cap = epi ? epi->gn_cap : 0; p.gn_slot0 = 0;
    p.gn_used_host = epi ? epi->gn_used : nullptr;
    p.zero_t_halo = (epi && epi->zero_t_halo && k3) ? 1 : 0;
    p.out_p16 = nullptr;
    if (epi && epi->p16_out) {
        const bool dense = out.t_stride == (int64_t)out.H * out.W && out.y_stride == out.W && out.c_stride == (int64_t)out.T * out.H * out.W;
        SS_CHECK_ARG(epi->p16_done && dense && !flat && !epi->res && !epi->gn_part && out.C % 8 == 0 && prec == STEMSEG_PRECISION_F16X3 && (!epi || epi->nb <= 1),
                     "conv3d: the pair-plane output needs f16x3, a dense output volume, no residual / statistics / clip batch");
        *epi->p16_done = 0;
        p.out_p16 = epi->p16_out;
        p.gn_used_host = epi->p16_done;
    }
    p.nb = (epi && epi->nb > 1) ? epi->nb : 1;
    p.in_bs = p.nb > 1 ? epi->in_bs : 0; p.out_bs = p.nb > 1 ? epi->out_bs : 0; p.gn_bs = p.nb > 1 ? epi->gn_bs : 0;
    SS_CHECK_ARG(p.nb == 1 || (!p.res && p.nb <= 65535 && p.in_bs % 4 == 0 && p.out_bs % 4 == 0), "conv3d: a clip batch takes no residual and 16-byte aligned clip strides");
    SS_CHECK_ARG(!p.gn_part || ((p.gn_cpg == 4 || p.gn_cpg == 8) && p.gn_used_host && p.Cout % p.gn_cpg == 0 && !(epi->relu || epi->res)),
                 "conv3d: fused GroupNorm statistics need groups of 4 or 8 channels and a plain (bias-only) epilogue");
    auto al16 = [](const void* ptr, int64_t cs, int64_t ts, int64_t ys, int T, int H) {
        return (reinterpret_cast<uintptr_t>(ptr) % 16 == 0) && (cs % 4 == 0) && (T == 1 || ts % 4 == 0) && (H == 1 || ys % 4 == 0);
    };
    p.vec_epi = (!flat && p.W % 4 == 0 && al16(p.out, p.out_cs, p.out_ts, p.out_ys, p.T, p.H) &&
                 (!p.res || al16(p.res, p.res_cs, p.res_ts, p.res_ys, p.T, p.H))) ? 1 : 0;
    p.tiles_x = p.tiles_y = 0;
    p.t_fastest = 1;
    p.flat_t = 0; p.T_all = p.T;
    const bool aligned = (reinterpret_cast<uintptr_t>(in.ptr) % 16 == 0) && (in.c_stride % 4 == 0) &&
                         (in.T == 1 || in.t_stride % 4 == 0) && (in.H == 1 || in.y_stride % 4 == 0);
    p.vec4 = aligned ? 1 : 0;
    SS_CHECK_ARG(reinterpret_cast<uintptr_t>(packed_w) % 16 == 0, "conv3d: packed weights must be 16-byte aligned");
    PlanCtx pc_store;
    const PlanCtx* pc = nullptr;
    if (epi && epi->plan_frames > 0) {
        SS_CHECK_ARG(epi->frames > 0 && epi->plan_scratch_floats >= 0, "conv3d: plan_frames needs the launch's own frame count");
        pc_store.shape = p;
        pc_store.scratch_floats = epi->plan_scratch_floats;
        if (p.T == 1 && p.H == 1) {
            SS_CHECK_ARG(p.W % epi->frames == 0, "conv3d: flat volume of %d voxels is not %d whole frames", p.W, epi->frames);
            const int64_t Wp = (int64_t)(p.W / epi->frames) * epi->plan_frames;
            SS_CHECK_ARG(Wp < (1ll << 31), "conv3d: planning volume too large");
            pc_store.shape.W = (int)Wp;
        } else {
            SS_CHECK_ARG(p.T == epi->frames, "conv3d: launch of %d t-planes announced as %d frames", p.T, epi->frames);
            pc_store.shape.T = epi->plan_frames;
        }
        pc_store.shape.T_all = pc_store.shape.T;
        pc = &pc_store;
    }
    const ConvKParams& d = pc ? pc->shape : p;
    const LaunchCtx L{s, scratch, scratch_floats, pc};
    if (k4) return launch_stem_f16x3(p, L);
    if (prec == STEMSEG_PRECISION_BF16X6) return launch_split_family<2>(p, d, L, tile_cfg, k3, k2);
    if (prec == STEMSEG_PRECISION_F16X3) return launch_split_family<3>(p, d, L, tile_cfg, k3, k2);
    const bool auto_cfg = tile_cfg <= 0 || tile_cfg > 3;
    if (k3) {
        int cfg = tile_cfg;
        if (auto_cfg) {
            if (tile_workgroups<K3Big>(d) >= 512) cfg = 1;
            else if (tile_workgroups<K3Med>(d) >= 384) cfg = 2;
            else cfg = 3;
        }
        if (cfg == 2 && prefer_flat<K3FlatMed56, K3Med>(p, tile_cfg)) return launch_cfg<K3FlatMed56>(p, L);
        if (cfg == 3 && prefer_flat<K3FlatSmall56, K3Small>(p, tile_cfg)) return launch_cfg<K3FlatSmall56>(p, L);
        if (cfg == 2 && prefer_flat<K3FlatMed, K3Med>(p, tile_cfg)) return launch_cfg<K3FlatMed>(p, L);
        if (cfg == 3 && prefer_flat<K3FlatSmall, K3Small>(p, tile_cfg)) return launch_cfg<K3FlatSmall>(p, L);
        if (cfg == 1 && p.vec4 && p.Cout % 128 == 0) {
            if (auto_cfg) return launch_planned<K3BigGL, K3Med>(p, d, L, 2, 2);
            return launch_cfg<K3BigGL>(p, L);
        }
        if (cfg == 1 && auto_cfg) return launch_planned<K3Big, K3Med>(p, d, L, 2, 2);
        if (cfg == 1) return launch_cfg<K3Big>(p, L);
        if (cfg == 2) return launch_cfg<K3Med>(p, L);
        return launch_cfg<K3Small>(p, L);
    }
    if (k2) {
        if (p.Cout <= 64) return launch_cfg<K2M64>(p, L);
        int cfg = tile_cfg;
        if (auto_cfg) {
            const int64_t need = scratch ? 96 : 384;
            if (tile_workgroups<K2Big>(d) >= need) cfg = 1;
            else if (tile_workgroups<K2Med>(d) >= need) cfg = 2;
            else cfg = 3;
        }
        if (cfg == 1 && prefer_flat<K2FlatBig56, K2Big>(p, tile_cfg)) return launch_cfg<K2FlatBig56>(p, L);
        if (cfg >= 2 && prefer_flat<K2FlatMed56, K2Med>(p, tile_cfg)) return launch_cfg<K2FlatMed56>(p, L);
        if (cfg == 1 && prefer_flat<K2FlatBig, K2Big>(p, tile_cfg)) return launch_cfg<K2FlatBig>(p, L);
        if (cfg >= 2 && prefer_flat<K2FlatMed, K2Med>(p, tile_cfg)) return launch_cfg<K2FlatMed>(p, L);
        if (cfg == 1 && auto_cfg && tile_workgroups<K2Big>(d) >= 512) return launch_planned<K2Big, K2Med>(p, d, L, 3, 3);
        if (cfg == 1) return launch_cfg<K2Big>(p, L);
        if (cfg == 2) return launch_cfg<K2Med>(p, L);
        return launch_cfg<K2Small>(p, L);
    }
    if (p.Cout <= 64) return launch_gl<K1M64GL, K1M64>(p, L);
    int cfg = tile_cfg;
    if (cfg <= 0 || cfg > 2) {
        cfg = (tile_workgroups<K1Big>(d) >= (scratch ? 96 : 512)) ? 1 : 2;
        if (p.Cin <= 256 && p.Cout >= 4 * p.Cin && tile_workgroups<K1Big>(d) < 2048) cfg = 2;
    }
    if (cfg == 1) return launch_gl<K1BigGL, K1Big>(p, L);
    return launch_gl<K1SmallGL, K1Small>(p, L);
}

int launch_conv3d_gn(const StemsegVolume& in, const float* packed_w, const float* bias, const StemsegVolume& out, int kt, int kh, int kw,
                     int tile_cfg, hipStream_t s, float* splitk_scratch, int64_t splitk_scratch_floats, const ConvEpilogue* epi, int groups,
                     float eps, float* stats, double* gn_scratch, int64_t stats_bs) {
    SS_CHECK_ARG(stats && gn_scratch && groups > 0 && out.C % groups == 0, "conv3d_gn: bad GroupNorm arguments");
    const int cpg = out.C / groups;
    const int64_t S = (int64_t)out.T * out.H * out.W;
    const bool dense = out.t_stride == (int64_t)out.H * out.W && out.y_stride == out.W && out.c_stride == S;
    const int64_t slot_bound = ceil_div(out.W, 32) * ceil_div(out.H, 2) * out.T + (int64_t)cpg * ceil_div(S, 256);
    if ((cpg != 4 && cpg != 8) || slot_bound > GN_SLOT_CAP || (epi && (epi->relu || epi->res || epi->dec_W > 0))) {
        SS_CHECK_ARG(dense, "conv3d_gn: the separate statistics pass needs a dense output");
        int rc = launch_conv3d(in, packed_w, bias, out, kt, kh, kw, tile_cfg, s, splitk_scratch, splitk_scratch_floats, epi);
        const int nb = (epi && epi->nb > 1) ? epi->nb : 1;
        for (int b = 0; b < nb && !rc; ++b)
            rc = launch_gn_stats(out.ptr + (nb > 1 ? b * epi->out_bs : 0), out.C, S, groups, eps, stats + (int64_t)b * stats_bs, gn_scratch + (nb > 1 ? b * epi->gn_bs : 0), s);
        return rc;
    }
    ConvEpilogue e = epi ? *epi : ConvEpilogue();
    int used = 0;
    e.gn_part = gn_scratch; e.gn_cpg = cpg; e.gn_cap = GN_SLOT_CAP; e.gn_used = &used;
    const int rc = launch_conv3d(in, packed_w, bias, out, kt, kh, kw, tile_cfg, s, splitk_scratch, splitk_scratch_floats, &e);
    if (rc) return rc;
    return launch_gn_finalize_slots(gn_scratch, groups, GN_SLOT_CAP, used, (double)cpg * (double)S, eps, stats, s, e.nb, e.gn_bs, stats_bs);
}

static ConvEpilogue epilogue_from_abi(const StemsegConvEpilogue* epilogue) {
    ConvEpilogue e;
    if (epilogue) {
        e.relu = epilogue->relu; e.res = epilogue->residual; e.res_cs = epilogue->res_c_stride; e.res_ts = epilogue->res_t_stride;
        e.res_ys = epilogue->res_y_stride; e.dec_H = epilogue->decode_H; e.dec_W = epilogue->decode_W;
        e.precision = epilogue->precision;
        e.frames = epilogue->frames; e.plan_frames = epilogue->plan_frames; e.plan_scratch_floats = epilogue->plan_scratch_floats;
// ... 46 lines not shown
```

### stem-seg_amd/csrc/encoder.hip

```cpp
#include "common.h"
#include <algorithm>
#include <cstddef>

namespace stemseg {

struct Padded2D {
    int64_t pitch, ts, cs, total, interior;
    Padded2D() = default;
    Padded2D(int C, int T, int H, int W) {
        pitch = round_up((int64_t)W + 2, 4);
        ts = (int64_t)(H + 2) * pitch;
        cs = (int64_t)T * ts;
        total = (int64_t)C * cs + 64;
        interior = pitch + 1;
    }
};
static inline StemsegVolume halo2d_view(float* base, int C, int T, int H, int W) {
    Padded2D g(C, T, H, W);
    return make_volume(base, g.cs, g.ts, g.pitch, C, T, H + 2, W + 2, g.total);
}
static inline StemsegVolume interior2d_view(float* base, int C, int T, int H, int W) {
    Padded2D g(C, T, H, W);
    return make_volume(base + g.interior, g.cs, g.ts, g.pitch, C, T, H, W, g.total - g.interior);
}
// ... 247 lines not shown
    const int m = (int)(rowp - pl * (unsigned)(Hc + 1));
    const bool row_a = m >= 1, row_b = m < Hc;
    const int y0 = m >= 1 ? m - 1 : 0, y1 = y0 + (y0 < Hc - 1 ? 1 : 0);
    const float wy_a = 0.25f, wy_b = m >= 1 ? 0.75f : 0.f;
    const float* c0 = coarse + (int64_t)pl * c_ts + (int64_t)y0 * c_pitch;
    const float* c1 = coarse + (int64_t)pl * c_ts + (int64_t)y1 * c_pitch;
    const int xa = min(max(2 * k - 1, 0), Wc - 1), xb = min(2 * k, Wc - 1), xc = min(2 * k + 1, Wc - 1);
    const float a0 = c0[xa], b0 = c0[xb], d0 = c0[xc], a1 = c1[xa], b1 = c1[xb], d1 = c1[xc];
    float* fbase = fine_halo + (int64_t)pl * f_ts + 4 * k;
    float4 fa = {0.f, 0.f, 0.f, 0.f}, fb = {0.f, 0.f, 0.f, 0.f};
    if (row_a) fa = *reinterpret_cast<const float4*>(fbase + (int64_t)(2 * m) * f_pitch);
    if (row_b) fb = *reinterpret_cast<const float4*>(fbase + (int64_t)(2 * m + 1) * f_pitch);
    float* va = reinterpret_cast<float*>(&fa);
    float* vb = reinterpret_cast<float*>(&fb);
#pragma unroll
    for (int j = 0; j < 4; ++j) {
        const int x = 4 * k - 1 + j;
        if (x < 0 || x >= W) continue;
        const bool first = j < 2 && x > 0;
        const float p0 = first ? a0 : (x == 0 ? a0 : b0), p1 = first ? b0 : d0;
        const float q0 = first ? a1 : (x == 0 ? a1 : b1), q1 = first ? b1 : d1;
        const float wx = x == 0 ? 0.f : ((x & 1) ? 0.25f : 0.75f);
        if (row_a) va[j] = __fadd_rn(va[j], up2_blend(p0, p1, q0, q1, wx, wy_a));
        if (row_b) vb[j] = __fadd_rn(vb[j], up2_blend(p0, p1, q0, q1, wx, wy_b));
    }
    if (row_a) *reinterpret_cast<float4*>(fbase + (int64_t)(2 * m) * f_pitch) = fa;
    if (row_b) *reinterpret_cast<float4*>(fbase + (int64_t)(2 * m + 1) * f_pitch) = fb;
}

__global__ __launch_bounds__(256) void upsample2x_add_dense_vec4x2_kernel(float* __restrict__ fine_halo, const float* __restrict__ fine_dense,
                                                                           const float* __restrict__ coarse, int H, int W, unsigned gq, unsigned n_items,
                                                                           int64_t f_ts, int f_pitch, int64_t c_ts, int c_pitch) {
    const unsigned idx = blockIdx.x * 256u + threadIdx.x;
    if (idx >= n_items) return;
    const int Hc = H / 2, Wc = W / 2;
    const unsigned rowp = idx / gq;
    const int k = (int)(idx - rowp * gq);
    const unsigned pl = rowp / (unsigned)(Hc + 1);
    const int m = (int)(rowp - pl * (unsigned)(Hc + 1));
    const bool row_a = m >= 1, row_b = m < Hc;
    const int y0 = m >= 1 ? m - 1 : 0, y1 = y0 + (y0 < Hc - 1 ? 1 : 0);
    const float wy_a = 0.25f, wy_b = m >= 1 ? 0.75f : 0.f;
    const float* c0 = coarse + (int64_t)pl * c_ts + (int64_t)y0 * c_pitch;
    const float* c1 = coarse + (int64_t)pl * c_ts + (int64_t)y1 * c_pitch;
    const int xa = min(max(2 * k - 1, 0), Wc - 1), xb = min(2 * k, Wc - 1), xc = min(2 * k + 1, Wc - 1);
    const float a0 = c0[xa], b0 = c0[xb], d0 = c0[xc], a1 = c1[xa], b1 = c1[xb], d1 = c1[xc];
    const float* dbase = fine_dense + (int64_t)pl * H * W;
    float va[4] = {0.f, 0.f, 0.f, 0.f}, vb[4] = {0.f, 0.f, 0.f, 0.f};
    const bool g_lo = k >= 1, g_hi = 4 * k < W;
    if (row_a) {
        const float* r = dbase + (int64_t)(2 * m - 1) * W;
        if (g_lo) va[0] = reinterpret_cast<const float4*>(r)[k - 1].w;
        if (g_hi) { const float4 q = reinterpret_cast<const float4*>(r)[k]; va[1] = q.x; va[2] = q.y; va[3] = q.z; }
    }
    if (row_b) {
        const float* r = dbase + (int64_t)(2 * m) * W;
        if (g_lo) vb[0] = reinterpret_cast<const float4*>(r)[k - 1].w;
        if (g_hi) { const float4 q = reinterpret_cast<const float4*>(r)[k]; vb[1] = q.x; vb[2] = q.y; vb[3] = q.z; }
    }
#pragma unroll
    for (int j = 0; j < 4; ++j) {
        const int x = 4 * k - 1 + j;
        if (x < 0 || x >= W) { va[j] = 0.f; vb[j] = 0.f; continue; }
        const bool first = j < 2 && x > 0;
        const float p0 = first ? a0 : (x == 0 ? a0 : b0), p1 = first ? b0 : d0;
        const float q0 = first ? a1 : (x == 0 ? a1 : b1), q1 = first ? b1 : d1;
        const float wx = x == 0 ? 0.f : ((x & 1) ? 0.25f : 0.75f);
        if (row_a) va[j] = __fadd_rn(va[j], up2_blend(p0, p1, q0, q1, wx, wy_a));
        if (row_b) vb[j] = __fadd_rn(vb[j], up2_blend(p0, p1, q0, q1, wx, wy_b));
    }
    float* fbase = fine_halo + (int64_t)pl * f_ts + 4 * k;
    if (row_a) *reinterpret_cast<float4*>(fbase + (int64_t)(2 * m) * f_pitch) = make_float4(va[0], va[1], va[2], va[3]);
    if (row_b) *reinterpret_cast<float4*>(fbase + (int64_t)(2 * m + 1) * f_pitch) = make_float4(vb[0], vb[1], vb[2], vb[3]);
}

static int grid1d(int64_t n) { return (int)std::max<int64_t>(1, std::min<int64_t>(ceil_div(n, 256), 256 * 16)); }

struct EncoderPlan {
    GuardList guards;
    int T, H, W, nblk[4], total_blocks;
    int h[4], w[4];
    int64_t V[4];
    int64_t S0, X1, A, B, Cst[4], M1[4], M2, DS, XS, L[4], FO[4], SK, SKfloats, total;
    int64_t S2D, s2d_ts, s2d_pitch;
    int groups, s3, mid[4];
    int64_t M1S[4];
    int plan_frames;
    int64_t plan_SKfloats;
};
constexpr int64_t ENC_PLAN_SK_FLOATS = 32ll << 20;

static int make_encoder_plan(const StemsegEncoderDesc* d, EncoderPlan& p) {
    SS_CHECK_ARG(d, "encoder: null descriptor");
    constexpr int32_t old_bytes = (int32_t)offsetof(StemsegEncoderDesc, conv2_groups);
    SS_CHECK_ARG(d->struct_bytes == (int32_t)sizeof(StemsegEncoderDesc) || d->struct_bytes == old_bytes,
                 "encoder: descriptor size mismatch (%d vs %d or %d): ABI skew", d->struct_bytes, (int)sizeof(StemsegEncoderDesc), (int)old_bytes);
    const bool has_arch = d->struct_bytes == (int32_t)sizeof(StemsegEncoderDesc);
    const int groups = has_arch && d->conv2_groups > 0 ? d->conv2_groups : 1;
    const int wpg = has_arch && d->width_per_group > 0 ? d->width_per_group : 64;
    SS_CHECK_ARG(!has_arch || (d->conv2_groups >= 0 && d->width_per_group >= 0 && (d->stride_in_3x3 == 0 || d->stride_in_3x3 == 1)),
                 "encoder: conv2_groups=%d width_per_group=%d stride_in_3x3=%d", d->conv2_groups, d->width_per_group, d->stride_in_3x3);
    if (groups == 1) {
        SS_CHECK_ARG(wpg == 64, "encoder: width_per_group=%d with one group (64 only)", wpg);
    } else {
        SS_CHECK_ARG((wpg == 4 || wpg == 8) && groups <= 1024 && (groups * wpg) % 32 == 0,
                     "encoder: %d groups x %d channels (width_per_group 4 or 8: 4..64 channels per group over the stages; groups x width a multiple of 32)",
                     groups, wpg);
    }
    p.groups = groups;
    p.s3 = has_arch ? d->stride_in_3x3 : 0;
    for (int i = 0; i < 4; ++i) p.mid[i] = (groups * wpg) << i;
    SS_CHECK_ARG(d->n_clips >= 1 && d->clip_frames >= 0 && d->clip_stride >= 0, "encoder: bad clip layout");
    if (d->clip_frames > 0) {
        SS_CHECK_ARG(d->clip_stride > 0 && (d->n_clips - 1) * d->clip_stride + d->clip_frames == d->T,
                     "encoder: %d windows of %d frames every %d frames do not cover T=%d", d->n_clips, d->clip_frames, d->clip_stride, d->T);
    } else {
        SS_CHECK_ARG(d->T % d->n_clips == 0, "encoder: T=%d is not n_clips=%d whole clips", d->T, d->n_clips);
    }
    SS_CHECK_ARG(d->T >= 1 && d->H >= 32 && d->W >= 32 && d->H % 32 == 0 && d->W % 32 == 0, "encoder: T=%d H=%d W=%d (H, W multiples of 32)", d->T, d->H, d->W);
    p.T = d->T; p.H = d->H; p.W = d->W;
    p.total_blocks = 0;
    for (int i = 0; i < 4; ++i) {
        SS_CHECK_ARG(d->blocks[i] >= 1 && d->blocks[i] <= 64, "encoder: blocks[%d]=%d", i, d->blocks[i]);
        p.nblk[i] = d->blocks[i];
        p.total_blocks += d->blocks[i];
        p.h[i] = d->H >> (2 + i); p.w[i] = d->W >> (2 + i);
        p.V[i] = (int64_t)d->T * p.h[i] * p.w[i];
    }
    SS_CHECK_ARG(p.total_blocks <= STEMSEG_MAX_ENCODER_BLOCKS, "encoder: more than %d bottleneck blocks", STEMSEG_MAX_ENCODER_BLOCKS);
    int64_t off = 0;
    p.guards.n = 0;
    auto take = [&](int64_t floats) {
        int64_t o = off;
        off += round_up(floats, 64);
        p.guards.push(off);
        off += WS_GUARD_FLOATS;
        return o;
    };
    p.S0 = take(64 * 4 * p.V[0]);
    p.s2d_pitch = round_up(d->W / 2 + 3, 4);
    p.s2d_ts = (int64_t)(d->H / 2 + 3) * p.s2d_pitch;
    p.S2D = take(12 * (int64_t)d->T * p.s2d_ts + 64);
    p.X1 = take(64 * p.V[0]);
    p.A = take(256 * p.V[0]);
    p.B = take(256 * p.V[0]);
    for (int i = 0; i < 4; ++i) {
        p.Cst[i] = take((int64_t)(256 << i) * p.V[i]);
        p.M1[i] = take(Padded2D(p.mid[i], p.T, p.h[i], p.w[i]).total);
    }
    p.M2 = take((int64_t)p.mid[0] * p.V[0]);
    p.DS = take(256 * p.V[0]);
    p.XS = take(256 * p.V[1]);
    for (int i = 0; i < 4; ++i) p.L[i] = take(Padded2D(256, p.T, p.h[i], p.w[i]).total);
    const bool shared_out = d->clip_frames > 0 && d->clip_stride < d->clip_frames && d->n_clips > 1;
    for (int i = 0; i < 4; ++i) p.FO[i] = shared_out ? take(256 * p.V[i]) : -1;
    for (int i = 0; i < 4; ++i) p.M1S[i] = (p.s3 && i > 0) ? take(Padded2D(p.mid[i], p.T, p.h[i - 1], p.w[i - 1]).total) : -1;
    SS_CHECK_ARG(d->plan_frames >= 0 && d->plan_frames <= 4096, "encoder: plan_frames=%d", d->plan_frames);
    p.plan_frames = d->plan_frames;
    p.plan_SKfloats = ENC_PLAN_SK_FLOATS;
    p.SKfloats = ENC_PLAN_SK_FLOATS * (d->plan_frames > 0 ? std::max<int64_t>(1, ceil_div(d->T, d->plan_frames)) : 1);
    p.SK = take(p.SKfloats);
    p.total = off;
    SS_CHECK_ARG(!p.guards.full, "encoder: the plan has more than %d workspace slices (GuardList)", WS_MAX_GUARDS);
    return STEMSEG_OK;
}

}

using namespace stemseg;

extern "C" size_t stemseg_hip_encoder_workspace_bytes(const StemsegEncoderDesc* desc) {
    EncoderPlan p;
    if (make_encoder_plan(desc, p) != STEMSEG_OK) return 0;
    return (size_t)p.total * sizeof(float);
}

extern "C" int stemseg_hip_encoder_plan_offsets(const StemsegEncoderDesc* desc, int64_t* out25) {
    EncoderPlan p;
    int rc = make_encoder_plan(desc, p);
    if (rc) return rc;
    SS_CHECK_ARG(out25, "encoder_plan_offsets: null pointer");
    int n = 0;
    out25[n++] = p.S0; out25[n++] = p.X1; out25[n++] = p.A; out25[n++] = p.B;
    for (int i = 0; i < 4; ++i) out25[n++] = p.Cst[i];
    for (int i = 0; i < 4; ++i) out25[n++] = p.M1[i];
    out25[n++] = p.M2; out25[n++] = p.DS; out25[n++] = p.XS;
    for (int i = 0; i < 4; ++i) out25[n++] = p.L[i];
    for (int i = 0; i < 4; ++i) out25[n++] = p.FO[i];
    out25[n++] = p.SK; out25[n++] = p.total;
    return STEMSEG_OK;
}

extern "C" int stemseg_hip_encoder_init_workspace(const StemsegEncoderDesc* desc, void* workspace, size_t ws_bytes, void* stream) {
    EncoderPlan p;
    int rc = make_encoder_plan(desc, p);
    if (rc) return rc;
    SS_CHECK_ARG(workspace && (reinterpret_cast<uintptr_t>(workspace) % 256 == 0), "encoder: workspace must be 256-byte aligned");
    if (ws_bytes < (size_t)p.total * sizeof(float)) {
        set_error("encoder: workspace too small (%zu < %zu bytes)", ws_bytes, (size_t)p.total * sizeof(float));
        return STEMSEG_E_WORKSPACE;
    }
    SS_HIP(hipMemsetAsync(workspace, 0, (size_t)p.total * sizeof(float), as_stream(stream)));
    return launch_canary_fill(reinterpret_cast<float*>(workspace), p.guards, as_stream(stream));
}

extern "C" int stemseg_hip_encoder_check_workspace(const StemsegEncoderDesc* desc, const void* workspace, size_t ws_bytes, int32_t* n_bad_host,
                                                   int64_t* first_bad_host, void* stream) {
    EncoderPlan p;
    int rc = make_encoder_plan(desc, p);
    if (rc) return rc;
    SS_CHECK_ARG(workspace && ws_bytes >= (size_t)p.total * sizeof(float), "encoder_check_workspace: bad workspace");
    return canary_check(reinterpret_cast<const float*>(workspace), p.guards, n_bad_host, first_bad_host, as_stream(stream));
}

extern "C" int stemseg_hip_stem_conv(const float* frames, const float* w_tap_major, const float* bias, float* out, int32_t T, int32_t H, int32_t W,
                                     void* stream) {
    SS_CHECK_ARG(frames && w_tap_major && bias && out, "stem_conv: null pointer");
    SS_CHECK_ARG(T >= 1 && H >= 2 && W >= 2 && H % 2 == 0 && W % 2 == 0, "stem_conv: T=%d H=%d W=%d (H, W even)", T, H, W);
    const int Ho = H / 2, Wo = W / 2;
    const int64_t blocks = ceil_div(Wo, ST_COLS) * ceil_div(Ho, ST_ROWS) * T;
    SS_CHECK_ARG(blocks < (1ll << 31), "stem_conv: too many tiles");
    hipLaunchKernelGGL(stem_conv7x7_mfma_kernel, dim3((unsigned)blocks), dim3(256), 0, as_stream(stream), frames, w_tap_major, bias, out, T, H, W);
    SS_LAUNCH_CHECK();
    return STEMSEG_OK;
}

extern "C" int stemseg_hip_encoder_forward(const StemsegEncoderDesc* desc, const StemsegEncoderWeights* wts, const float* frames,
                                           const StemsegVolume* out, void* workspace, size_t ws_bytes, void* stream) {
    EncoderPlan p;
    int rc = make_encoder_plan(desc, p);
    if (rc) return rc;
    SS_CHECK_ARG(wts && frames && out && workspace, "encoder_forward: null pointer");
    if (ws_bytes < (size_t)p.total * sizeof(float)) {
        set_error("encoder: workspace too small (%zu < %zu bytes)", ws_bytes, (size_t)p.total * sizeof(float));
        return STEMSEG_E_WORKSPACE;
    }
    SS_CHECK_ARG(wts->stem_w && wts->stem_b, "encoder_forward: null stem weights");
    for (int i = 0; i < 4; ++i) {
        for (int c = 0; c < desc->n_clips; ++c) {
            const StemsegVolume& o = out[4 * c + i];
            const int Tc_ = desc->clip_frames > 0 ? desc->clip_frames : p.T / desc->n_clips;
            SS_CHECK_ARG(o.ptr && o.C == desc->out_channels && o.T == Tc_ && o.H == p.h[i] && o.W == p.w[i],
                         "encoder_forward: output volume %d of clip %d must be [%d][%d][%d][%d]", i, c, desc->out_channels, Tc_, p.h[i], p.w[i]);
        }
        SS_CHECK_ARG(wts->fpn_inner_w[i] && wts->fpn_inner_b[i] && wts->fpn_layer_w[i] && wts->fpn_layer_b[i], "encoder_forward: null FPN weights %d", i);
    }
    SS_CHECK_ARG(desc->out_channels == 256, "encoder: out_channels must be 256");
    SS_CHECK_ARG(desc->precision == STEMSEG_PRECISION_F32 || desc->precision == STEMSEG_PRECISION_BF16X6 || desc->precision == STEMSEG_PRECISION_F16X3,
                 "encoder: precision must be 0 (f32), 2 (bf16x6) or 3 (f16x3)");
    const int prec = desc->precision;
    auto epi_for = [&](int frames) {
        ConvEpilogue e;
        e.precision = prec;
        if (p.plan_frames > 0) { e.frames = frames; e.plan_frames = p.plan_frames; e.plan_scratch_floats = p.plan_SKfloats; }
        return e;
    };
    hipStream_t s = as_stream(stream);
    float* ws = reinterpret_cast<float*>(workspace);
    const int T = p.T;

    {
        const int Ho = p.H / 2, Wo = p.W / 2;
        const int blocks = (int)(ceil_div(Wo, ST_COLS) * ceil_div(Ho, ST_ROWS) * T);
        void* ev = profile_begin(47, 4.0 * ((double)3 * T * p.H * p.W + 64.0 * T * Ho * Wo), s);
        if (wts->stem_w_s2d && prec == STEMSEG_PRECISION_F16X3 && p.W % 2 == 0) {
            hipLaunchKernelGGL(stem_s2d_kernel, dim3(grid1d((int64_t)T * 3 * p.H * (p.W / 2))), dim3(256), 0, s, frames, ws + p.S2D, T, p.H, p.W, p.s2d_ts, (int)p.s2d_pitch);
            SS_LAUNCH_CHECK();
            const StemsegVolume in = make_volume(ws + p.S2D, (int64_t)T * p.s2d_ts, p.s2d_ts, p.s2d_pitch, 12, T, Ho + 3, Wo + 3, 12 * (int64_t)T * p.s2d_ts + 64);
            ConvEpilogue es = epi_for(T);
            es.relu = 1;
            rc = launch_conv3d(in, wts->stem_w_s2d, wts->stem_b, dense_volume(ws + p.S0, 64, T, Ho, Wo), 1, 4, 4, 0, s, nullptr, 0, &es);
            if (rc) return rc;
        } else {
            hipLaunchKernelGGL(stem_conv7x7_mfma_kernel, dim3((unsigned)blocks), dim3(256), 0, s, frames, wts->stem_w, wts->stem_b, ws + p.S0, T, p.H, p.W);
        }
        profile_end(ev, s);
        SS_LAUNCH_CHECK();
        ev = profile_begin(48, 4.0 * 64.0 * T * ((double)Ho * Wo + (double)p.V[0] / T), s);
        const int64_t mp_items = (int64_t)64 * T * (Ho / 2) * (Wo / 8);
        if (Wo % 8 == 0 && mp_items < (1ll << 31))
            hipLaunchKernelGGL(maxpool3x3s2_vec4_kernel, dim3((unsigned)ceil_div(mp_items, 256)), dim3(256), 0, s, (const float*)(ws + p.S0), ws + p.X1, Ho,
                               Wo, (unsigned)mp_items);
        else
            hipLaunchKernelGGL(maxpool3x3s2_kernel, dim3(grid1d(64 * p.V[0])), dim3(256), 0, s, (const float*)(ws + p.S0), ws + p.X1, (int64_t)64 * T, Ho, Wo);
        profile_end(ev, s);
        SS_LAUNCH_CHECK();
    }
    float* x = ws + p.X1;
    int cin = 64, bi = 0;
    bool conv1_done = false;
    for (int st = 0; st < 4; ++st) {
        const int mid = p.mid[st], cout = 256 << st, h = p.h[st], w = p.w[st];
        const int64_t V = p.V[st];
        for (int b = 0; b < p.nblk[st]; ++b, ++bi) {
            const bool first = (b == 0), stride2 = first && st > 0;
            const bool s3 = stride2 && p.s3;
            const bool grouped = p.groups > 1 || s3;
            SS_CHECK_ARG(wts->conv1_w[bi] && wts->conv1_b[bi] && wts->conv2_w[bi] && wts->conv2_b[bi] && wts->conv3_w[bi] && wts->conv3_b[bi],
                         "encoder_forward: null weights for block %d", bi);
            SS_CHECK_ARG(!first || (wts->down_w[bi] && wts->down_b[bi]), "encoder_forward: block %d needs a projection shortcut", bi);
            float* xin = x;
            if (stride2) {
                void* ev = profile_begin(49, 4.0 * 2.0 * (double)cin * V, s);
                const int64_t ss_items = (int64_t)cin * T * h * (w / 4);
                if (w % 4 == 0 && ss_items < (1ll << 31))
                    hipLaunchKernelGGL(subsample2_vec4_kernel, dim3((unsigned)ceil_div(ss_items, 256)), dim3(256), 0, s, (const float*)x, ws + p.XS, 2 * h,
                                       2 * w, (unsigned)ss_items);
                else
                    hipLaunchKernelGGL(subsample2_kernel, dim3(grid1d((int64_t)cin * V)), dim3(256), 0, s, (const float*)x, ws + p.XS, (int64_t)cin * T, 2 * h, 2 * w);
                profile_end(ev, s);
                SS_LAUNCH_CHECK();
                xin = ws + p.XS;
            }
            float* y = (b == p.nblk[st] - 1) ? ws + p.Cst[st] : ((b & 1) ? ws + p.B : ws + p.A);
            const int h1 = s3 ? 2 * h : h, w1 = s3 ? 2 * w : w;
            float* m1 = ws + (s3 ? p.M1S[st] : p.M1[st]);
            if (!conv1_done) {
                ConvEpilogue e1 = epi_for(T);
                e1.relu = 1; e1.dec_H = h1; e1.dec_W = w1;
                rc = launch_conv3d(flat_view(s3 ? x : xin, cin, (int64_t)T * h1 * w1), wts->conv1_w[bi], wts->conv1_b[bi], interior2d_view(m1, mid, T, h1, w1), 1, 1,
                                   1, 0, s, ws + p.SK, p.SKfloats, &e1);
                if (rc) return rc;
            }
            const bool want_fuse = ((desc->fuse_tail >> st) & 1) && prec == STEMSEG_PRECISION_F16X3 && b + 1 < p.nblk[st] && !grouped && p.groups == 1 &&
                                   mid * 4 == cout && fused_tail_supported(mid) && V <= (1ll << 27) && (int64_t)T * (h + 2) * (w + 4) <= (1ll << 27);
            int p16_done = 0;
            if (grouped) {
                rc = launch_grouped_conv(halo2d_view(m1, mid, T, h1, w1), wts->conv2_w[bi], wts->conv2_b[bi], dense_volume(ws + p.M2, mid, T, h, w), p.groups,
                                         s3 ? 2 : 1, 1, prec, s);
            } else {
                ConvEpilogue e2 = epi_for(T);
                e2.relu = 1;
                if (want_fuse) { e2.p16_out = reinterpret_cast<unsigned int*>(ws + p.M2); e2.p16_done = &p16_done; }
                rc = launch_conv3d(halo2d_view(m1, mid, T, h, w), wts->conv2_w[bi], wts->conv2_b[bi], dense_volume(ws + p.M2, mid, T, h, w), 1, 3, 3, 0, s,
                                   ws + p.SK, p.SKfloats, &e2);
            }
            if (rc) return rc;
            const float* idt = xin;
            ConvEpilogue ed = epi_for(T);
            const bool ds_in_tail = first && want_fuse && p16_done && !(desc->fuse_tail & 32) && st < 2 && !(st == 1 && ((desc->fuse_tail >> 3) & 3) == 1) &&
                                    fused_shortcut_supported(mid, cin, V);
            if (first && !ds_in_tail) {
                rc = launch_conv3d(flat_view(xin, cin, V), wts->down_w[bi], wts->down_b[bi], flat_view(ws + p.DS, cout, V), 1, 1, 1, 0, s, ws + p.SK, p.SKfloats,
                                   &ed);
                if (rc) return rc;
                idt = ws + p.DS;
            }
            if (want_fuse && p16_done) {
                SS_CHECK_ARG(wts->conv1_w[bi + 1] && wts->conv1_b[bi + 1], "encoder_forward: null weights for block %d", bi + 1);
                rc = launch_fused_tail(mid, reinterpret_cast<const unsigned int*>(ws + p.M2), wts->conv3_w[bi], wts->conv3_b[bi], ds_in_tail ? nullptr : idt, y,
                                       wts->conv1_w[bi + 1], wts->conv1_b[bi + 1], interior2d_view(ws + p.M1[st], mid, T, h, w), h, w, V, (desc->fuse_tail >> 3) & 3, s,
                                       ds_in_tail ? xin : nullptr, cin, ds_in_tail ? wts->down_w[bi] : nullptr, ds_in_tail ? wts->down_b[bi] : nullptr);
                if (rc) return rc;
                conv1_done = true;
            } else {
                ConvEpilogue e3 = epi_for(T);
                e3.relu = 1; e3.res = idt; e3.res_cs = V; e3.res_ts = 0; e3.res_ys = 0;
                rc = launch_conv3d(flat_view(ws + p.M2, mid, V), wts->conv3_w[bi], wts->conv3_b[bi], flat_view(y, cout, V), 1, 1, 1, 0, s, ws + p.SK, p.SKfloats, &e3);
                if (rc) return rc;
                conv1_done = false;
            }
            x = y;
            cin = cout;
        }
    }
    for (int k = 3; k >= 0; --k) {
        const int h = p.h[k], w = p.w[k];
        ConvEpilogue e = epi_for(T), el = epi_for(T);
        e.dec_H = h; e.dec_W = w;
        Padded2D gf0(256, T, h, w);
        const unsigned gq0 = (unsigned)((w + 1) / 4 + 1);
        const bool lat_dense = k < 3 && h % 2 == 0 && w % 4 == 0 && p.h[k + 1] == h / 2 && p.w[k + 1] == w / 2 && gf0.pitch % 4 == 0 &&
                               (int64_t)4 * gq0 <= gf0.pitch && (int64_t)256 * T * (h / 2 + 1) * gq0 < (1ll << 32) - 256 &&
                               (reinterpret_cast<uintptr_t>(ws + p.L[k]) % 16 == 0) && gf0.ts % 4 == 0 && (reinterpret_cast<uintptr_t>(ws + p.A) % 16 == 0);
        if (lat_dense) {
            ConvEpilogue ed = epi_for(T);
            rc = launch_conv3d(flat_view(ws + p.Cst[k], 256 << k, p.V[k]), wts->fpn_inner_w[k], wts->fpn_inner_b[k], flat_view(ws + p.A, 256, p.V[k]), 1, 1, 1, 0, s,
                               ws + p.SK, p.SKfloats, &ed);
            if (rc) return rc;
            Padded2D gc0(256, T, p.h[k + 1], p.w[k + 1]);
            void* ev = profile_begin(50, 4.0 * 256.0 * (2.0 * p.V[k] + p.V[k + 1]), s);
            const int64_t items = (int64_t)256 * T * (h / 2 + 1) * gq0;
            hipLaunchKernelGGL(upsample2x_add_dense_vec4x2_kernel, dim3((unsigned)ceil_div(items, 256)), dim3(256), 0, s, ws + p.L[k], (const float*)(ws + p.A),
                               (const float*)(ws + p.L[k + 1] + gc0.interior), h, w, gq0, (unsigned)items, gf0.ts, (int)gf0.pitch, gc0.ts, (int)gc0.pitch);
            profile_end(ev, s);
            SS_LAUNCH_CHECK();
        } else {
        rc = launch_conv3d(flat_view(ws + p.Cst[k], 256 << k, p.V[k]), wts->fpn_inner_w[k], wts->fpn_inner_b[k], interior2d_view(ws + p.L[k], 256, T, h, w), 1, 1, 1, 0, s,
                           ws + p.SK, p.SKfloats, &e);
        if (rc) return rc;
        }
        if (k < 3 && !lat_dense) {
            Padded2D gf(256, T, h, w), gc(256, T, p.h[k + 1], p.w[k + 1]);
            void* ev = profile_begin(50, 4.0 * 256.0 * (2.0 * p.V[k] + p.V[k + 1]), s);
            const unsigned gq = (unsigned)((w + 1) / 4 + 1);
            const int64_t ua_items = (int64_t)256 * T * h * gq;
            const bool ua_vec = gf.pitch % 4 == 0 && (int64_t)4 * gq <= gf.pitch && ua_items < (1ll << 32) - 256 && (reinterpret_cast<uintptr_t>(ws + p.L[k]) % 16 == 0) && gf.ts % 4 == 0;
            const int64_t ua2_items = (int64_t)256 * T * (h / 2 + 1) * gq;
            if (ua_vec && h % 2 == 0 && w % 2 == 0 && p.h[k + 1] == h / 2 && p.w[k + 1] == w / 2)
                hipLaunchKernelGGL(upsample2x_add_vec4x2_kernel, dim3((unsigned)ceil_div(ua2_items, 256)), dim3(256), 0, s, ws + p.L[k],
                                   (const float*)(ws + p.L[k + 1] + gc.interior), h, w, gq, (unsigned)ua2_items, gf.ts, (int)gf.pitch, gc.ts, (int)gc.pitch);
            else if (ua_vec)
                hipLaunchKernelGGL(upsample2x_add_vec4_kernel, dim3((unsigned)ceil_div(ua_items, 256)), dim3(256), 0, s, ws + p.L[k],
                                   (const float*)(ws + p.L[k + 1] + gc.interior), h, w, gq, (unsigned)ua_items, gf.ts, (int)gf.pitch, gc.ts, (int)gc.pitch);
            else
                hipLaunchKernelGGL(upsample2x_add_kernel, dim3(grid1d(256 * p.V[k])), dim3(256), 0, s, ws + p.L[k] + gf.interior,
                                   (const float*)(ws + p.L[k + 1] + gc.interior), (int64_t)256 * T, h, w, gf.ts, gf.pitch, gc.ts, gc.pitch);
            profile_end(ev, s);
            SS_LAUNCH_CHECK();
        }
        const int Tc = desc->clip_frames > 0 ? desc->clip_frames : T / desc->n_clips;
        const int Ts = desc->clip_frames > 0 ? desc->clip_stride : Tc;
        if (p.FO[k] >= 0) {
            rc = launch_conv3d(halo2d_view(ws + p.L[k], 256, T, h, w), wts->fpn_layer_w[k], wts->fpn_layer_b[k], dense_volume(ws + p.FO[k], 256, T, h, w), 1, 3, 3,
                               0, s, ws + p.SK, p.SKfloats, &el);
            if (rc) return rc;
            for (int c = 0; c < desc->n_clips; ++c) {
                rc = launch_copy_strided(ws + p.FO[k] + (int64_t)c * Ts * h * w, (int64_t)T * h * w, (int64_t)h * w, out[4 * c + k], s);
                if (rc) return rc;
            }
            continue;
        }
        bool uniform = desc->n_clips > 1 && desc->n_clips <= 65535;
        const int64_t obs = uniform ? out[4 + k].ptr - out[k].ptr : 0;
        for (int c = 1; c < desc->n_clips && uniform; ++c) {
            const StemsegVolume &a = out[4 * c + k], &b = out[k];
            uniform = a.ptr == b.ptr + c * obs && a.c_stride == b.c_stride && a.t_stride == b.t_stride && a.y_stride == b.y_stride && a.limit == b.limit;
        }
        if (uniform && obs > 0 && obs % 4 == 0) {
            StemsegVolume in = halo2d_view(ws + p.L[k], 256, T, h, w);
            ConvEpilogue ec = epi_for(Tc);
            ec.nb = desc->n_clips;
            ec.in_bs = (int64_t)Ts * in.t_stride;
            ec.out_bs = obs;
            in.limit -= (int64_t)(desc->n_clips - 1) * ec.in_bs;
            in.T = Tc;
            rc = launch_conv3d(in, wts->fpn_layer_w[k], wts->fpn_layer_b[k], out[k], 1, 3, 3, 0, s, ws + p.SK, p.SKfloats, &ec);
            if (rc) return rc;
            continue;
        }
        for (int c = 0; c < desc->n_clips; ++c) {
            StemsegVolume in = halo2d_view(ws + p.L[k], 256, T, h, w);
            in.ptr += (int64_t)c * Ts * in.t_stride;
            in.limit -= (int64_t)c * Ts * in.t_stride;
            in.T = Tc;
            const ConvEpilogue ec = epi_for(Tc);
            rc = launch_conv3d(in, wts->fpn_layer_w[k], wts->fpn_layer_b[k], out[4 * c + k], 1, 3, 3, 0, s, ws + p.SK, p.SKfloats, &ec);
            if (rc) return rc;
        }
    }
    return STEMSEG_OK;
}
```

### stem-seg_amd/stemseg_amd/hip.py

```python
import ctypes as C
import os

import torch

_HERE = os.path.dirname(os.path.abspath(__file__))
LIB_PATH = os.environ.get("STEMSEG_HIP_LIB") or os.path.join(_HERE, "lib", "libstemseg_hip.so")

MAX_INSTANCES = 64
MAX_EMB_DIMS = 8
ABI_VERSION = 11


class Volume(C.Structure):
    _fields_ = [("ptr", C.c_void_p), ("c_stride", C.c_int64), ("t_stride", C.c_int64), ("y_stride", C.c_int64),
                ("C", C.c_int32), ("T", C.c_int32), ("H", C.c_int32), ("W", C.c_int32), ("limit", C.c_int64)]


class DecoderDesc(C.Structure):
    _fields_ = [("struct_bytes", C.c_int32), ("in_channels", C.c_int32), ("inter", C.c_int32 * 4),
                ("T", C.c_int32), ("H4", C.c_int32), ("W4", C.c_int32), ("gn_groups", C.c_int32), ("gn_eps", C.c_float),
                ("pool", C.c_int32 * 3), ("t_scale", C.c_int32 * 3), ("n_out", C.c_int32),
                ("act", C.c_int32 * (2 * MAX_EMB_DIMS)), ("grid_axis", C.c_int32 * (2 * MAX_EMB_DIMS)),
                ("input_layout", C.c_int32), ("concurrency", C.c_int32), ("detached", C.c_int32), ("precision", C.c_int32),
                ("n_clips", C.c_int32), ("feat_clip_stride", C.c_int64 * 4), ("out_clip_stride", C.c_int64)]


class DecoderWeights(C.Structure):
    _fields_ = [("conv_w", C.c_void_p * 7), ("conv_b", C.c_void_p * 7), ("gn_w", C.c_void_p * 7), ("gn_b", C.c_void_p * 7),
                ("fuse_w", C.c_void_p * 3), ("head_w", C.c_void_p), ("head_b", C.c_void_p),
                ("grid_t", C.c_void_p), ("grid_y", C.c_void_p), ("grid_x", C.c_void_p)]


MAX_ENCODER_BLOCKS = 40


class ConvEpilogue(C.Structure):
    _fields_ = [("relu", C.c_int32), ("residual", C.c_void_p), ("res_c_stride", C.c_int64), ("res_t_stride", C.c_int64),
                ("res_y_stride", C.c_int64), ("decode_H", C.c_int32), ("decode_W", C.c_int32), ("precision", C.c_int32),
                ("frames", C.c_int32), ("plan_frames", C.c_int32), ("plan_scratch_floats", C.c_int64)]


class EncoderDesc(C.Structure):
    _fields_ = [("struct_bytes", C.c_int32), ("blocks", C.c_int32 * 4), ("T", C.c_int32), ("H", C.c_int32), ("W", C.c_int32),
                ("out_channels", C.c_int32), ("precision", C.c_int32), ("n_clips", C.c_int32), ("clip_frames", C.c_int32),
                ("clip_stride", C.c_int32), ("plan_frames", C.c_int32), ("fuse_tail", C.c_int32),
                ("conv2_groups", C.c_int32), ("width_per_group", C.c_int32), ("stride_in_3x3", C.c_int32)]


_BLK = C.c_void_p * MAX_ENCODER_BLOCKS


class EncoderWeights(C.Structure):
    _fields_ = [("stem_w", C.c_void_p), ("stem_b", C.c_void_p), ("stem_w_s2d", C.c_void_p),
                ("conv1_w", _BLK), ("conv1_b", _BLK), ("conv2_w", _BLK), ("conv2_b", _BLK), ("conv3_w", _BLK), ("conv3_b", _BLK),
                ("down_w", _BLK), ("down_b", _BLK),
                ("fpn_inner_w", C.c_void_p * 4), ("fpn_inner_b", C.c_void_p * 4), ("fpn_layer_w", C.c_void_p * 4), ("fpn_layer_b", C.c_void_p * 4)]


class ClusterParams(C.Structure):
    _fields_ = [("primary_prob_thresh", C.c_float), ("secondary_prob_thresh", C.c_float), ("min_seediness_prob", C.c_float),
                ("max_instances", C.c_int32), ("n_free_dims", C.c_int32), ("free_dim_bandwidths", C.c_float * MAX_EMB_DIMS)]


class ClusterMeta(C.Structure):
    _fields_ = [("K", C.c_int32), ("exhausted", C.c_int32), ("n_points", C.c_int64), ("n_unassigned_last", C.c_int64),
                ("centers", (C.c_float * MAX_EMB_DIMS) * MAX_INSTANCES), ("bandwidths", (C.c_float * MAX_EMB_DIMS) * MAX_INSTANCES),
                ("seed_prob", C.c_float * MAX_INSTANCES)]


class ClusterItem(C.Structure):
    _fields_ = [("emb", C.c_void_p), ("bw", C.c_void_p), ("seed", C.c_void_p), ("n_max", C.c_int64), ("n_points_dev", C.c_void_p),
                ("label_start", C.c_int64), ("labels", C.c_void_p), ("meta_dev", C.c_void_p), ("opt_masks", C.c_void_p), ("opt_probs", C.c_void_p),
                ("workspace", C.c_void_p), ("ws_bytes", C.c_size_t)]


class EmbeddingLossDesc(C.Structure):
    _fields_ = [("struct_bytes", C.c_int32), ("embedding_size", C.c_int32), ("n_free_dims", C.c_int32), ("n_instances", C.c_int32),
                ("T", C.c_int32), ("H", C.c_int32), ("W", C.c_int32), ("reserved", C.c_int32), ("free_dim_bandwidths", C.c_float * MAX_EMB_DIMS)]


class TargetPrepDesc(C.Structure):
    _fields_ = [("struct_bytes", C.c_int32), ("n_instances", C.c_int32), ("T", C.c_int32), ("H", C.c_int32), ("W", C.c_int32),
                ("reserved", C.c_int32)]


class SemsegLossDesc(C.Structure):
    _fields_ = [("struct_bytes", C.c_int32), ("n_classes", C.c_int32), ("has_foreground_channel", C.c_int32), ("T", C.c_int32),
                ("H", C.c_int32), ("W", C.c_int32), ("reserved", C.c_int32), ("reserved2", C.c_int32), ("stride_c", C.c_int64),
                ("stride_t", C.c_int64), ("stride_h", C.c_int64), ("stride_w", C.c_int64)]


_P, _I32, _I64, _F = C.c_void_p, C.c_int32, C.c_int64, C.c_float
SIGNATURES = {
    "stemseg_hip_version": (C.c_int, []),
    "stemseg_hip_last_error": (C.c_char_p, []),
    "stemseg_hip_device_count": (C.c_int, []),
    "stemseg_hip_profile_enable": (C.c_int, [_I32]),
    "stemseg_hip_profile_read": (C.c_int, [C.POINTER(C.c_double), _I32]),
    "stemseg_hip_padded_geometry": (C.c_int, [_I32, _I32, _I32, _I32, C.POINTER(_I64)]),
    "stemseg_hip_pack_conv_weight": (C.c_int, [_P, _P, _I32, _I32, _I32, _P]),
    "stemseg_hip_encoder_plan_offsets": (C.c_int, [_P, _P]),
    "stemseg_hip_packed_weight_bytes_prec": (C.c_int64, [_I32, _I32, _I32, _I32]),
    "stemseg_hip_pack_conv_weight_prec": (C.c_int, [_P, _P, _I32, _I32, _I32, _I32, _P]),
    "stemseg_hip_conv3d": (C.c_int, [C.POINTER(Volume), _P, _P, C.POINTER(Volume), _I32, _I32, _I32, _I32, _P, _I64, C.POINTER(ConvEpilogue), _P]),
    "stemseg_hip_packed_grouped_weight_bytes": (C.c_int64, [_I32, _I32, _I32, _I32]),
    "stemseg_hip_pack_grouped_conv_weight": (C.c_int, [_P, _P, _I32, _I32, _I32, _I32, _P]),
    "stemseg_hip_conv2d_grouped": (C.c_int, [C.POINTER(Volume), _P, _P, C.POINTER(Volume), _I32, _I32, _I32, _I32, _I32, _P]),
    "stemseg_hip_conv3d_gn_scratch_doubles": (C.c_int64, [_I32, _I32]),
    "stemseg_hip_conv3d_zero_t_halo": (C.c_int, [C.POINTER(Volume), _P, _P, C.POINTER(Volume), _I32, _I32, _I32, _I32, _P, _I64, C.POINTER(ConvEpilogue),
                                                _I32, _F, _P, _P, _P]),
    "stemseg_hip_conv3d_gn": (C.c_int, [C.POINTER(Volume), _P, _P, C.POINTER(Volume), _I32, _I32, _I32, _I32, _P, _I64, _I32, _I32, _F, _P, _P, _P]),
    "stemseg_hip_stem_conv": (C.c_int, [_P, _P, _P, _P, _I32, _I32, _I32, _P]),
    "stemseg_hip_encoder_workspace_bytes": (C.c_size_t, [C.POINTER(EncoderDesc)]),
    "stemseg_hip_encoder_init_workspace": (C.c_int, [C.POINTER(EncoderDesc), _P, C.c_size_t, _P]),
    "stemseg_hip_encoder_check_workspace": (C.c_int, [C.POINTER(EncoderDesc), _P, C.c_size_t, C.POINTER(_I32), C.POINTER(_I64), _P]),
    "stemseg_hip_encoder_forward": (C.c_int, [C.POINTER(EncoderDesc), C.POINTER(EncoderWeights), _P, C.POINTER(Volume), _P, C.c_size_t, _P]),
    "stemseg_hip_groupnorm_stats": (C.c_int, [_P, _I32, _I64, _I32, _F, _P, _P, _P]),
    "stemseg_hip_gn_relu_pool": (C.c_int, [_P, _I32, _I32, _I32, _I32, _I32, _P, _P, _P, _I32, C.POINTER(Volume), _P]),
    "stemseg_hip_upsample_trilinear": (C.c_int, [_P, _I32, _I32, _I32, _I32, _I32, _I32, _I32, C.POINTER(Volume), _P]),
    "stemseg_hip_copy_to_volume": (C.c_int, [_P, _I32, C.POINTER(Volume), _P]),
    "stemseg_hip_heads": (C.c_int, [_P, _I32, _I32, _I32, _I32, _P, _P, _I32, C.POINTER(_I32), C.POINTER(_I32), _P, _P, _P, _P, _P]),
    "stemseg_hip_nonfinite_flags": (C.c_int, [_P, _I64, _P, _I32, _P]),
    "stemseg_hip_decoder_workspace_bytes": (C.c_size_t, [C.POINTER(DecoderDesc)]),
    "stemseg_hip_decoder_init_workspace": (C.c_int, [C.POINTER(DecoderDesc), _P, C.c_size_t, _P]),
    "stemseg_hip_decoder_check_workspace": (C.c_int, [C.POINTER(DecoderDesc), _P, C.c_size_t, C.POINTER(_I32), C.POINTER(_I64), _P]),
    "stemseg_hip_decoder_forward": (C.c_int, [C.POINTER(DecoderDesc), C.POINTER(DecoderWeights), C.POINTER(_P), _P, _P, C.c_size_t, _P]),
    "stemseg_hip_decoder_join": (C.c_int, [_I32, _P]),
    "stemseg_hip_seediness_accumulate": (C.c_int, [_P, _P, _I64, _I32, _P]),
    "stemseg_hip_fg_mask": (C.c_int, [_P, _F, _F, _P, _I64, _P]),
    "stemseg_hip_fg_mask_frames": (C.c_int, [_P, _P, _F, _P, _I32, _I64, _P]),
    "stemseg_hip_fg_gather": (C.c_int, [_P, _P, _P, _P, _I32, _I32, _I32, _I64, _P, _P, _P, _P, _P, _P, _P]),
    "stemseg_hip_cluster_workspace_bytes": (C.c_size_t, [_I64]),
    "stemseg_hip_cluster": (C.c_int, [_P, _P, _P, _I64, _P, _I32, _I32, C.POINTER(ClusterParams), _I64, _P, _P, _P, _P, _P, C.c_size_t, _P]),
    "stemseg_hip_cluster_batch": (C.c_int, [C.POINTER(ClusterItem), _I32, _I32, _I32, C.POINTER(ClusterParams), _P]),
    "stemseg_hip_overlap_counts": (C.c_int, [_P, _P, _I64, _P, _I32, _P, _I32, _I32, _I32, _P, _P, _P, _P]),
    "stemseg_hip_label_presence": (C.c_int, [_P, _I64, _P, _I32, _P, _I32, _P]),
    "stemseg_hip_relabel": (C.c_int, [_P, _I64, _P, _I32, _P]),
    "stemseg_hip_fg_compact": (C.c_int, [_P, _I32, _I64, _P, _P, _P, _P]),
    "stemseg_hip_labels_to_codes": (C.c_int, [_P, _P, _P, _I64, _I64, _P, _I64, _P]),
    "stemseg_hip_pair_tables": (C.c_int, [_P, _P, _P, _I32, _I64, _I32, _P, _P]),
    "stemseg_hip_codes_to_labels": (C.c_int, [_P, _P, _P, _I32, _I64, _P, _I64, _I32, _P, _P]),
    "stemseg_hip_semseg_accumulate": (C.c_int, [_P, _P, _I32, _I32, _I64, C.POINTER(C.c_int32), _I32, _P]),
    "stemseg_hip_semseg_masks": (C.c_int, [_P, _P, _I32, _I32, _I64, _I32, _P, _P, _P]),
    "stemseg_hip_semseg_fg_clip": (C.c_int, [_P, _I32, _I32, _I64, _F, _P, _P, _P]),
    "stemseg_hip_preprocess_frames": (C.c_int, [_P, _I32, _I32, _I32, _I32, _I32, _I32, _I32, C.POINTER(C.c_float), C.POINTER(C.c_float), _I32, _I32, _P, _P]),
    "stemseg_hip_scatter_instance_index": (C.c_int, [_P, _P, _P, _I64, _P, _I32, _P, _I32, _I32, _P]),
    "stemseg_hip_resample_instance_masks": (C.c_int, [_P, _I32, _I32, C.c_float, _I32, _I32, _I32, _I32, _P, _P]),
    "stemseg_hip_scatter_instance_index_ex": (C.c_int, [_P, _P, _P, _I64, _P, _I32, _P, _I32, _I32, _I32, _P]),
    "stemseg_hip_resample_instance_masks_ex": (C.c_int, [_P, _I32, _I32, _I32, C.c_float, _I32, _I32, _I32, _I32, _P, _P]),
    "stemseg_hip_rle_workspace_bytes": (C.c_size_t, [_I32, _I32, _I32, _I32, _I64]),
    "stemseg_hip_rle_plan": (C.c_int, [_P, _I32, _I32, _I32, _I32, _I32, _I64, _P, C.c_size_t, _P, _P, _P, _P]),
    "stemseg_hip_rle_encode": (C.c_int, [_P, _I32, _I32, _I32, _I32, _I32, _I64, _P, C.c_size_t, _P, _P, _P, _P, _P, _P, _P]),
    "stemseg_hip_instance_class_stats": (C.c_int, [_P, _P, _P, _P, _I32, _I64, _P, _I32, _I32, _I32, _I32, _P, _I32, _P, _P, _P, _I32, _P, _P, _P]),
    "stemseg_hip_vis_composite": (C.c_int, [_P, _P, _I32, _I32, _I32, _I32, _P, _I32, _P, _P]),
    "stemseg_hip_jpeg_workspace_bytes": (C.c_size_t, [_I32, _I32, _I32]),
    "stemseg_hip_jpeg_plan": (C.c_int, [_P, _I32, _I32, _I32, _I32, _P, C.c_size_t, _P, _P, _P]),
    "stemseg_hip_jpeg_encode": (C.c_int, [_I32, _I32, _I32, _I32, _P, C.c_size_t, _P, _I64, _P, _P]),
    "stemseg_hip_jpeg_decode_workspace_bytes": (C.c_size_t, [_I32, _I32, _I32, _I32, _I64, _I64, _I32]),
    "stemseg_hip_jpeg_decode": (C.c_int, [_P, _P, _P, _I32, _I32, _I32, _I32, _I64, _I64, _I32, _I32, _P, C.c_size_t, _P, _P, _P]),
    "stemseg_hip_png_decode_workspace_bytes": (C.c_size_t, [_I32, _I32, _I32, _I32, _I64, _I32, _I32]),
    "stemseg_hip_png_decode": (C.c_int, [_P, _P, _P, _I32, _I32, _I32, _I32, _I64, _I32, _I32, _P, C.c_size_t, _P, _P, _P]),
    "stemseg_hip_embedding_loss_workspace_bytes": (C.c_size_t, [C.POINTER(EmbeddingLossDesc)]),
    "stemseg_hip_embedding_loss_forward": (C.c_int, [C.POINTER(EmbeddingLossDesc), _P, _P, _P, _P, C.c_size_t, _P, C.POINTER(_I32), _P]),
    "stemseg_hip_embedding_loss_backward": (C.c_int, [C.POINTER(EmbeddingLossDesc), _P, _P, _P, _P, C.c_size_t, _P, _I32, _I32, _P, _P]),
    "stemseg_hip_prepare_targets": (C.c_int, [C.POINTER(TargetPrepDesc), _P, _P, _P, _P, _P, _P, _P, _P]),
    "stemseg_hip_semseg_loss_workspace_bytes": (C.c_size_t, [C.POINTER(SemsegLossDesc)]),
    "stemseg_hip_semseg_loss_forward": (C.c_int, [C.POINTER(SemsegLossDesc), _P, _P, _P, _P, C.c_size_t, _P, _P, _P]),
    "stemseg_hip_semseg_loss_backward": (C.c_int, [C.POINTER(SemsegLossDesc), _P, _P, _P, _P, C.c_size_t, _P, _I32, _P, _P]),
    "stemseg_hip_level_head": (C.c_int, [_P, _I32, _I64, _P, _I32, _P, _P, _P]),
    "stemseg_hip_heads_backward_workspace_bytes": (C.c_size_t, [_I32, _I32, _I64]),
    "stemseg_hip_heads_backward": (C.c_int, [_P, _I32, _I32, _I32, _I32, _P, _P, _I32, C.POINTER(_I32), C.POINTER(_I32), _P, _P, _P, _P, _P, _P,
                                             _P, _P, _P, C.c_size_t, _P]),
    "stemseg_hip_upsample_trilinear_backward": (C.c_int, [_P, _I32, _I32, _I32, _I32, _I32, _I32, _I32, _P, _P]),
    "stemseg_hip_gn_relu_pool_backward_workspace_bytes": (C.c_size_t, [_I32, _I32, _I32, _I32, _I32]),
    "stemseg_hip_gn_relu_pool_backward": (C.c_int, [_P, _I32, _I32, _I32, _I32, _I32, _P, _P, _P, _I32, _P, _P, _P, _P, _P, C.c_size_t, _P]),
}

SEMSEG_OUTPUT_TYPES = {None: 0, "none": 0, "logits": 1, "probs": 2, "argmax": 3}

_lib = None


def lib():
    global _lib
    if _lib is None:
        if not os.path.exists(LIB_PATH):
            raise RuntimeError("libstemseg_hip.so not found at %s -- build it with `python stem-seg_amd/build.py` "
                               "(hipcc --offload-arch=gfx950); the hot path has no CPU fallback" % LIB_PATH)
        l = C.CDLL(LIB_PATH)
        for name, (res, args) in SIGNATURES.items():
            fn = getattr(l, name)
            fn.restype, fn.argtypes = res, args
        v = l.stemseg_hip_version()
        if v != ABI_VERSION:
            raise RuntimeError("libstemseg_hip.so ABI version %d != binding %d" % (v, ABI_VERSION))
        _lib = l
    return _lib


def require_gpu():
    l = lib()
    n = l.stemseg_hip_device_count()
    if n <= 0 or not torch.cuda.is_available():
        raise RuntimeError("stemseg_amd: no MI355X visible (hip device count %d, torch.cuda.is_available()=%s): %s"
                           % (n, torch.cuda.is_available(), l.stemseg_hip_last_error().decode()))
    return n


def check(rc):
    if rc != 0:
        raise RuntimeError("libstemseg_hip error %d: %s" % (rc, lib().stemseg_hip_last_error().decode()))


def stream():
    return C.c_void_p(torch.cuda.current_stream().cuda_stream)


def ptr(t, dtype=None):
    if t is None:
        return None
    assert t.is_cuda, "device tensor required"
    assert t.is_contiguous(), "contiguous tensor required"
    assert t.device.index == torch.cuda.current_device(), "tensor on %s but the current device is cuda:%d" % (t.device, torch.cuda.current_device())
    if dtype is not None:
        assert t.dtype == dtype, "expected %s, got %s" % (dtype, t.dtype)
    return C.c_void_p(t.data_ptr())


def profile_enable(on):
    check(lib().stemseg_hip_profile_enable(int(on)))


PROFILE_CONV_TAGS = {"conv3x3x3": (9, 8, 4, 2), "conv1x3x3": (36, 28, 27, 24, 22), "conv1x1x1": (18, 17, 14, 16, 12, 19)}
PROFILE_HBM_TAGS = {40: "upsample_trilinear", 41: "gn_stats (partial + finalize)", 42: "gn_relu (apply)", 43: "gn_relu_pool (apply + AvgPool3d)",
                    44: "heads", 45: "fg_gather (count + scan + scatter)", 46: "cluster (all rounds + final)", 47: "stem_conv7x7",
                    48: "maxpool3x3s2", 49: "subsample2", 50: "upsample2x_add (FPN top-down)"}


def profile_read(n_tags=64):
    buf = (C.c_double * (3 * n_tags))()
    check(lib().stemseg_hip_profile_read(buf, n_tags))
    return {t: (buf[3 * t], buf[3 * t + 1], int(buf[3 * t + 2])) for t in range(n_tags) if buf[3 * t + 2] > 0}


def padded_geometry(Cn, T, H, W):
    out = (C.c_int64 * 5)()
    check(lib().stemseg_hip_padded_geometry(Cn, T, H, W, out))
    return dict(pitch=out[0], ts=out[1], cs=out[2], total=out[3], interior=out[4])


def dense_volume(t):
    Cn, T, H, W = t.shape
    return Volume(t.data_ptr(), T * H * W, H * W, W, Cn, T, H, W, t.numel())


def flat_volume(t):
    Cn, V = t.shape[0], t[0].numel()
    return Volume(t.data_ptr(), V, 0, 0, Cn, 1, 1, V, t.numel())


def alloc_padded(Cn, T, H, W, device="cuda"):
    g = padded_geometry(Cn, T, H, W)
    return torch.zeros(g["total"], dtype=torch.float32, device=device), g


def alloc_padded_batch(n, Cn, T, H, W, device="cuda"):
    g = padded_geometry(Cn, T, H, W)
    stride = (g["total"] + 63) // 64 * 64
    whole = torch.zeros(n * stride, dtype=torch.float32, device=device)
    return [whole[c * stride:c * stride + g["total"]] for c in range(n)], g, stride


def padded_halo_view(buf, g, Cn, T, H, W):
    return Volume(buf.data_ptr(), g["cs"], g["ts"], g["pitch"], Cn, T + 2, H + 2, W + 2, g["total"])


def padded_interior_view(buf, g, Cn, T, H, W):
    return Volume(buf.data_ptr() + 4 * g["interior"], g["cs"], g["ts"], g["pitch"], Cn, T, H, W, g["total"] - g["interior"])


def padded_to_dense(buf, g, Cn, T, H, W):
    v = buf[:Cn * g["cs"]].view(Cn, T + 2, H + 2, g["pitch"])
    return v[:, 1:T + 1, 1:H + 1, 1:W + 1].contiguous()


def pack_conv_weight(w):
    w = w.contiguous()
    Cout, Cin = w.shape[0], w.shape[1]
    taps = w[0, 0].numel()
    out = torch.empty(Cout * Cin * taps, dtype=torch.float32, device=w.device)
    check(lib().stemseg_hip_pack_conv_weight(ptr(w, torch.float32), ptr(out), Cout, Cin, taps, stream()))
    return out


PRECISIONS = {"f32": 0, "bf16x6": 2, "f16x3": 3}
PRECISION_INFO = {
    "f32": dict(operand_significand_bits=24, products_per_fp32_product=1, mfma="v_mfma_f32_32x32x2_f32", exponent_range="fp32"),
    "bf16x6": dict(operand_significand_bits=24, products_per_fp32_product=6, mfma="v_mfma_f32_32x32x16_bf16", exponent_range="fp32"),
    "f16x3": dict(operand_significand_bits=22, products_per_fp32_product=3, mfma="v_mfma_f32_32x32x16_f16",
                  exponent_range="2.5e-4 <= |activation| < 2.6e5 at full width; beyond: non-finite output, flagged, re-run in bf16x6"),
}
DEFAULT_PRECISION = os.environ.get("STEMSEG_PRECISION", "f16x3")
assert DEFAULT_PRECISION in PRECISIONS, DEFAULT_PRECISION


def pack_conv_weight_any(w, precision="f32"):
    if precision == "f32":
        return pack_conv_weight(w)
    assert precision in ("bf16x6", "f16x3"), precision
    code = PRECISIONS[precision]
    w = w.contiguous()
    Cout, Cin = w.shape[0], w.shape[1]
    taps = w[0, 0].numel()
    nbytes = lib().stemseg_hip_packed_weight_bytes_prec(Cout, Cin, taps, code)
    if nbytes <= 0:
        raise ValueError("pack_conv_weight_any: unsupported shape / precision (%s, Cout %d, Cin %d, taps %d)" % (precision, Cout, Cin, taps))
# ... 876 lines not shown
```

Measured before the change: 124.9.

## Fuse stage-end conv3 with FPN lateral conv and stride-2 subsample

At the last bottleneck block of stages 0-2, the fused tail kernel now computes the conv3+residual output and, in the same launch, applies the FPN inner (lateral) 1x1 conv to it without ReLU. It also writes the even-position subsample of the stage output for the next stage's stride-2 input. This removes the separate lateral conv launch, the separate subsample kernel, and the extra HBM reads of the stage output. In exchange it adds extra scattered stores inside the epilogue, a more complex gating condition, and extra workspace buffers.

```diff
diff --git a/include/stemseg_hip.h b/include/stemseg_hip.h
--- a/include/stemseg_hip.h
+++ b/include/stemseg_hip.h
@@ -168,6 +168,7 @@
 
 size_t stemseg_hip_encoder_workspace_bytes(const StemsegEncoderDesc* desc);
 int stemseg_hip_encoder_plan_offsets(const StemsegEncoderDesc* desc, int64_t* out25);
+int stemseg_hip_encoder_stage_end_mask(const StemsegEncoderDesc* desc, int32_t* mask_out);
 
 int stemseg_hip_stem_conv(const float* frames, const float* w_tap_major, const float* bias, float* out, int32_t T, int32_t H, int32_t W,
                           void* stream);
diff --git a/stem-seg_amd/csrc/bottleneck_fused.hip b/stem-seg_amd/csrc/bottleneck_fused.hip
--- a/stem-seg_amd/csrc/bottleneck_fused.hip
+++ b/stem-seg_amd/csrc/bottleneck_fused.hip
@@ -22,28 +22,36 @@
     const float* xs;
     const char* wd;
     const float* bd;
+    float* xsub;
+    int sub_V;
 };
 
 constexpr SplitLayout FT_WL = SplitLayout(1, STEMSEG_PRECISION_F16X3);
 static_assert(FT_WL.CK == 32 && FT_WL.G == 2 && FT_WL.NPL == 2, "the fused tail walks 32-channel chunks of two k-groups, two planes");
 
-template <int MID_, int CT_, int P_, int DS_ = 0>
+template <bool LAT>
+__device__ __forceinline__ float slot_act(const float v) { return LAT ? v : relu_keep_nan(v); }
+
+template <int MID_, int CT_, int P_, int DS_ = 0, int N1_ = MID_, bool LAT_ = false>
 struct FusedTailCfg {
     static constexpr int MID = MID_, CT = CT_, COUT = 4 * MID_;
+    static constexpr int N1 = N1_;
+    static constexpr bool LAT = LAT_;
     static constexpr int DS = DS_, NCD = DS_ / 32;
     static constexpr int P = P_, NW = P_ / 32, NTHREADS = 64 * NW;
     static constexpr int NC3 = MID / 32;
     static constexpr int NCT = COUT / CT;
-    static constexpr int MI3 = CT / 32, MI1 = MID / 32;
+    static constexpr int MI3 = CT / 32, MI1 = N1 / 32;
     static constexpr int NH = 2 * MI3;
+    static constexpr int UNROLL3 = LAT && NC3 <= 2 ? NC3 : 1;
     static constexpr int X_BYTES = 2 * 4 * P * 16;
     static constexpr int W3_BYTES = 8 * CT * 16;
-    static constexpr int W1_HALF = 4 * MID * 16;
+    static constexpr int W1_HALF = 4 * N1 * 16;
     static constexpr int LDS_BYTES = 2 * X_BYTES + 2 * W3_BYTES + 2 * W1_HALF;
     static constexpr int NQ = P / 64;
     static constexpr int X_PIECES = X_BYTES / 1024, W3_PIECES = W3_BYTES / 1024, W1_PIECES = W1_HALF / 1024;
-    static_assert(NC3 == FT_WL.chunks(MID) && W3_BYTES == FT_WL.slab_bytes(CT, 32) && W1_HALF * FT_WL.G == FT_WL.slab_bytes(MID, 32), "tile byte sizes follow the packed-weight layout");
-    static_assert(P % 64 == 0 && MID % 32 == 0 && CT % 32 == 0 && COUT % CT == 0, "tile shapes");
+    static_assert(NC3 == FT_WL.chunks(MID) && W3_BYTES == FT_WL.slab_bytes(CT, 32) && W1_HALF * FT_WL.G == FT_WL.slab_bytes(N1, 32), "tile byte sizes follow the packed-weight layout");
+    static_assert(P % 64 == 0 && MID % 32 == 0 && N1 % 32 == 0 && CT % 32 == 0 && COUT % CT == 0 && 2 * N1 * 4 <= 2 * X_BYTES, "tile shapes");
     static_assert(LDS_BYTES <= (P <= 128 ? 80 : 160) * 1024, "LDS: two 128-position workgroups, or one 256-position workgroup, per CU");
     static_assert(W3_BYTES % 1024 == 0 && W1_HALF % 1024 == 0 && X_PIECES % NW == 0, "whole DMA pieces");
     static_assert(MI1 * 16 + MI3 * 16 + (DS ? MI3 * 16 : 0) <= 176, "accumulators must leave room for fragments at 256 registers");
@@ -68,11 +76,17 @@
     const int64_t V = p.V;
     const unsigned int lane_off = (unsigned int)(((int64_t)(4 * half) * V + pos_c) * 4);
     auto opaque = [](unsigned int v) __attribute__((always_inline)) { asm volatile("" : "+v"(v)); return v; };
+    const unsigned int SV4 = C::LAT ? (unsigned int)p.sub_V * 4u : 0u;
+    unsigned int sub_off = 0xFFFFFF00u;
+    if constexpr (C::LAT) {
+        const int hwp = p.dec_H * p.dec_W, t2 = pos_c / hwp, r2 = pos_c - t2 * hwp, y2 = r2 / p.dec_W, x2 = r2 - y2 * p.dec_W;
+        if (pos_ok && !((y2 | x2) & 1)) sub_off = (unsigned int)(4 * half) * SV4 + (unsigned int)((t2 * (p.dec_H / 2) + y2 / 2) * (p.dec_W / 2) + x2 / 2) * 4u;
+    }
 
     typedef const __attribute__((address_space(1))) void* gptr_t;
     typedef __attribute__((address_space(3))) void* lptr_t;
     const float* inv3 = reinterpret_cast<const float*>(p.w3 + FT_WL.inv_offset(C::COUT, C::MID));
-    const float* inv1 = reinterpret_cast<const float*>(p.w1 + FT_WL.inv_offset(C::MID, C::COUT));
+    const float* inv1 = reinterpret_cast<const float*>(p.w1 + FT_WL.inv_offset(C::N1, C::COUT));
 
     const int xpos = min(pos0 + lane, p.V - 1);
     auto dma_x = [&](const int c, const int buf) __attribute__((always_inline)) {
@@ -134,11 +148,12 @@
             xr[i] = __builtin_bit_cast(float, __builtin_amdgcn_raw_buffer_load_b32(rs, off, (unsigned int)(16 * (i >> 3) + (i & 7)) * V4, 0));
     };
     auto dma_tail_tab = [&]() __attribute__((always_inline)) {
-        constexpr int PIECES = (2 * C::MID + 255) / 256;
+        constexpr int PIECES = (2 * C::N1 + 255) / 256;
+        static_assert(PIECES <= C::NW, "one piece per wave");
         if (wave < PIECES) {
             const unsigned int f0 = (unsigned int)wave * 256u + opaque((unsigned int)lane) * 4u;
-            if (f0 < 2u * C::MID) {
-                const float* src = (f0 < (unsigned int)C::MID ? inv1 : p.b1 - C::MID) + (size_t)f0;
+            if (f0 < 2u * C::N1) {
+                const float* src = (f0 < (unsigned int)C::N1 ? inv1 : p.b1 - C::N1) + (size_t)f0;
                 __builtin_amdgcn_global_load_lds((gptr_t)src, (lptr_t)(xbuf + wave * 1024), 16, 0, 0);
             }
         }
@@ -243,7 +258,7 @@
             for (int r = 0; r < 16; ++r) acc3[m][r] = 0.f;
         const int co_j = j * C::CT;
         float rres[16];
-#pragma unroll 1
+#pragma unroll C::UNROLL3
         for (int c = 0; c < C::NC3; ++c) {
             if (c + 1 < C::NC3) { dma_x(c + 1, sb ^ 1); dma_w3(j, c + 1, sb ^ 1); }
             else { dma_w1(j, 0, 0); dma_tab(j, sb ^ 1); if constexpr (!DSV) load_identity(co_j, rres); }
@@ -304,6 +319,14 @@
                         *reinterpret_cast<float*>(yo + V * 8 + (size_t)lane_off) = v2;
                         *reinterpret_cast<float*>(yo + V * 12 + (size_t)lane_off) = v3;
                     }
+                    if constexpr (C::LAT) {
+                        const __amdgpu_buffer_rsrc_t rsub = __builtin_amdgcn_make_buffer_rsrc(p.xsub + (int64_t)co_j * p.sub_V, 0, (int)((unsigned int)C::CT * SV4), 0x00020000);
+                        const unsigned int row = (unsigned int)(m * 32 + 8 * q);
+                        __builtin_amdgcn_raw_buffer_store_b32(__builtin_bit_cast(unsigned int, v0), rsub, sub_off, (row + 0) * SV4, 0);
+                        __builtin_amdgcn_raw_buffer_store_b32(__builtin_bit_cast(unsigned int, v1), rsub, sub_off, (row + 1) * SV4, 0);
+                        __builtin_amdgcn_raw_buffer_store_b32(__builtin_bit_cast(unsigned int, v2), rsub, sub_off, (row + 2) * SV4, 0);
+                        __builtin_amdgcn_raw_buffer_store_b32(__builtin_bit_cast(unsigned int, v3), rsub, sub_off, (row + 3) * SV4, 0);
+                    }
                     split_pair_f16(v0, v1, hw[2 * q], lw[2 * q]);
                     split_pair_f16(v2, v3, hw[2 * q + 1], lw[2 * q + 1]);
                 }
@@ -331,11 +354,11 @@
                 if constexpr (DSV) { dma_wd(j + 1, 0, sb); load_xs(xr); }
                 else { dma_x(0, sb); dma_w3(j + 1, 0, sb); }
             } else dma_tail_tab();
-            const char* w1b = w1buf + (h & 1) * C::W1_HALF + (half * C::MID + l31) * 16;
+            const char* w1b = w1buf + (h & 1) * C::W1_HALF + (half * C::N1 + l31) * 16;
             f16x8 a_hi[2], a_lo[2];
             auto ld_a1 = [&](const int m1, const int k) __attribute__((always_inline)) {
-                a_hi[k] = *reinterpret_cast<const f16x8*>(w1b + ((0 * 2) * C::MID + m1 * 32) * 16);
-                a_lo[k] = *reinterpret_cast<const f16x8*>(w1b + ((1 * 2) * C::MID + m1 * 32) * 16);
+                a_hi[k] = *reinterpret_cast<const f16x8*>(w1b + ((0 * 2) * C::N1 + m1 * 32) * 16);
+                a_lo[k] = *reinterpret_cast<const f16x8*>(w1b + ((1 * 2) * C::N1 + m1 * 32) * 16);
             };
             ld_a1(0, 0);
 #pragma unroll
@@ -358,12 +381,12 @@
             for (int q = 0; q < 4; ++q) {
                 const int co4 = m1 * 32 + 8 * q + 4 * half;
                 const float4 sc = *reinterpret_cast<const float4*>(reinterpret_cast<const float*>(xbuf) + co4);
-                const float4 bv = *reinterpret_cast<const float4*>(reinterpret_cast<const float*>(xbuf) + C::MID + co4);
+                const float4 bv = *reinterpret_cast<const float4*>(reinterpret_cast<const float*>(xbuf) + C::N1 + co4);
                 char* zo = reinterpret_cast<char*>(p.z + (int64_t)(m1 * 32 + 8 * q) * p.z_cs);
-                *reinterpret_cast<float*>(zo + (size_t)z_off) = relu_keep_nan(__fadd_rn(__fmul_rn(acc1[m1][4 * q + 0], sc.x), bv.x));
-                *reinterpret_cast<float*>(zo + p.z_cs * 4 + (size_t)z_off) = relu_keep_nan(__fadd_rn(__fmul_rn(acc1[m1][4 * q + 1], sc.y), bv.y));
-                *reinterpret_cast<float*>(zo + p.z_cs * 8 + (size_t)z_off) = relu_keep_nan(__fadd_rn(__fmul_rn(acc1[m1][4 * q + 2], sc.z), bv.z));
-                *reinterpret_cast<float*>(zo + p.z_cs * 12 + (size_t)z_off) = relu_keep_nan(__fadd_rn(__fmul_rn(acc1[m1][4 * q + 3], sc.w), bv.w));
+                *reinterpret_cast<float*>(zo + (size_t)z_off) = slot_act<C::LAT>(__fadd_rn(__fmul_rn(acc1[m1][4 * q + 0], sc.x), bv.x));
+                *reinterpret_cast<float*>(zo + p.z_cs * 4 + (size_t)z_off) = slot_act<C::LAT>(__fadd_rn(__fmul_rn(acc1[m1][4 * q + 1], sc.y), bv.y));
+                *reinterpret_cast<float*>(zo + p.z_cs * 8 + (size_t)z_off) = slot_act<C::LAT>(__fadd_rn(__fmul_rn(acc1[m1][4 * q + 2], sc.z), bv.z));
+                *reinterpret_cast<float*>(zo + p.z_cs * 12 + (size_t)z_off) = slot_act<C::LAT>(__fadd_rn(__fmul_rn(acc1[m1][4 * q + 3], sc.w), bv.w));
             }
     }
 }
@@ -604,27 +627,30 @@
 #define FT_VMCNT(n) FT_VMCNT_(n)
 #define FT_SGB(mask, n) __builtin_amdgcn_sched_group_barrier(mask, n, 0)
 
-template <int MID_, int CT_, int DS_ = 0>
+template <int MID_, int CT_, int DS_ = 0, int N1_ = MID_, bool LAT_ = false>
 struct FusedTailR1Cfg {
     static constexpr int MID = MID_, CT = CT_, COUT = 4 * MID_;
+    static constexpr int N1 = N1_;
+    static constexpr bool LAT = LAT_;
+    static constexpr int EST = LAT ? 32 : 16;
     static constexpr int DS = DS_, NGD = DS_ / 16;
     static constexpr int NW = 4, NTHREADS = 64 * NW, P = 32 * NW;
     static constexpr int NC3 = MID / 32, NG = MID / 16, NCT = COUT / CT;
-    static constexpr int MI3 = CT / 32, MI1 = MID / 32;
+    static constexpr int MI3 = CT / 32, MI1 = N1 / 32;
     static constexpr int SC = 2;
     static constexpr int NS = NC3 / SC, NU = CT / 32;
     static constexpr int NSD = DS / 32 / SC;
     static_assert(DS % (32 * SC) == 0, "shortcut: whole stages");
     static constexpr int NX3 = SC * 2 * (MI3 / 2), NX1 = 2 * (MI1 / 2);
     static constexpr int W3_CHUNK = 8 * CT * 16, W3_BYTES = SC * W3_CHUNK;
-    static constexpr int W1_BYTES = 8 * MID * 16;
-    static_assert(W3_CHUNK == FT_WL.slab_bytes(CT, FT_WL.CK) && W1_BYTES == FT_WL.slab_bytes(MID, FT_WL.CK), "tile byte sizes follow the packed-weight layout");
+    static constexpr int W1_BYTES = 8 * N1 * 16;
+    static_assert(W3_CHUNK == FT_WL.slab_bytes(CT, FT_WL.CK) && W1_BYTES == FT_WL.slab_bytes(N1, FT_WL.CK), "tile byte sizes follow the packed-weight layout");
     static constexpr int TAB_BYTES = 1024;
     static constexpr int LDS_BYTES = 2 * W3_BYTES + 2 * W1_BYTES + 2 * TAB_BYTES;
     static constexpr int W3_PIECES = W3_BYTES / 1024 / NW, W1_PIECES = W1_BYTES / 1024 / NW;
     static constexpr int SL = 8 / NX1, S0 = NX1 / 4, M_PPS = 8 / S0;
     static_assert(NC3 % SC == 0 && MI3 % 2 == 0 && MI1 % 2 == 0 && W3_BYTES % (1024 * NW) == 0 && W1_BYTES % (1024 * NW) == 0 && 2 * CT * 4 <= TAB_BYTES, "whole DMA pieces per wave");
-    static_assert(LDS_BYTES <= 160 * 1024 && 2 * MID * 4 <= W3_BYTES && (NX1 == 8 || NX1 == 4) && NX3 == 8 && MI3 == 4 && NS >= 2 && NU >= 2 && NU % 2 == 0, "LDS / slice placement / identity buffer parity");
+    static_assert(LDS_BYTES <= 160 * 1024 && 2 * N1 * 4 <= W3_BYTES && 16 + EST <= 63 && (NX1 == 8 || NX1 == 4) && NX3 == 8 && MI3 == 4 && NS >= 2 && NU >= 2 && NU % 2 == 0, "LDS / slice placement / identity buffer parity");
     static_assert(W3_PIECES == 8 && W1_PIECES <= 8, "the pieces of a stage are requested in its first steps");
     static_assert(NG * 8 + MI1 * 16 <= 256, "the conv3 input and conv1's accumulators are the AGPR half of the register file");
 };
@@ -648,9 +674,15 @@
     const unsigned int lane_ld = (unsigned int)(4 * half) * V4 + (unsigned int)pos_c * 4u;
     const unsigned int lane_st = pos_ok ? lane_ld : 0xFFFFFF00u;
     const unsigned int tile_bytes = (unsigned int)C::CT * V4;
+    const unsigned int SV4 = C::LAT ? (unsigned int)p.sub_V * 4u : 0u;
+    unsigned int lane_sub = 0xFFFFFF00u;
+    if constexpr (C::LAT) {
+        const int hwp = p.dec_H * p.dec_W, t2 = pos_c / hwp, r2 = pos_c - t2 * hwp, y2 = r2 / p.dec_W, x2 = r2 - y2 * p.dec_W;
+        if (pos_ok && !((y2 | x2) & 1)) lane_sub = (unsigned int)(4 * half) * SV4 + (unsigned int)((t2 * (p.dec_H / 2) + y2 / 2) * (p.dec_W / 2) + x2 / 2) * 4u;
+    }
     typedef __attribute__((address_space(3))) void* lptr_t;
     const float* inv3 = reinterpret_cast<const float*>(p.w3 + FT_WL.inv_offset(C::COUT, C::MID));
-    const float* inv1 = reinterpret_cast<const float*>(p.w1 + FT_WL.inv_offset(C::MID, C::COUT));
+    const float* inv1 = reinterpret_cast<const float*>(p.w1 + FT_WL.inv_offset(C::N1, C::COUT));
 
     const unsigned int lane16 = (unsigned int)lane * 16u;
     const unsigned int lds_w3 = (unsigned int)(uintptr_t)(lptr_t)w3buf, lds_w1 = (unsigned int)(uintptr_t)(lptr_t)w1buf;
@@ -831,6 +863,7 @@
             for (int r = 0; r < 16; ++r) acc3[m][r] = 0.f;
         const float* tab = reinterpret_cast<const float*>(tabbuf + (j & 1) * C::TAB_BYTES) + 4 * half;
         const ft_rsrc_t ry = rsrc_of(p.y, j);
+        const ft_rsrc_t rsub = __builtin_amdgcn_make_buffer_rsrc(C::LAT ? p.xsub + (int64_t)j * C::CT * p.sub_V : p.y, 0, (int)((unsigned int)C::CT * SV4), 0x00020000);
         unsigned int hw[8], lw[8];
         f16x8 b_hi[2][2], b_lo[2][2];
         auto e_slice = [&](const int u, const int q4) __attribute__((always_inline)) {
@@ -850,6 +883,12 @@
             __builtin_amdgcn_raw_buffer_store_b32(__builtin_bit_cast(unsigned int, v1), ry, lane_st, (unsigned int)(c4 + 1) * V4, 0);
             __builtin_amdgcn_raw_buffer_store_b32(__builtin_bit_cast(unsigned int, v2), ry, lane_st, (unsigned int)(c4 + 2) * V4, 0);
             __builtin_amdgcn_raw_buffer_store_b32(__builtin_bit_cast(unsigned int, v3), ry, lane_st, (unsigned int)(c4 + 3) * V4, 0);
+            if constexpr (C::LAT) {
+                __builtin_amdgcn_raw_buffer_store_b32(__builtin_bit_cast(unsigned int, v0), rsub, lane_sub, (unsigned int)(c4 + 0) * SV4, 0);
+                __builtin_amdgcn_raw_buffer_store_b32(__builtin_bit_cast(unsigned int, v1), rsub, lane_sub, (unsigned int)(c4 + 1) * SV4, 0);
+                __builtin_amdgcn_raw_buffer_store_b32(__builtin_bit_cast(unsigned int, v2), rsub, lane_sub, (unsigned int)(c4 + 2) * SV4, 0);
+                __builtin_amdgcn_raw_buffer_store_b32(__builtin_bit_cast(unsigned int, v3), rsub, lane_sub, (unsigned int)(c4 + 3) * SV4, 0);
+            }
             split_pair_f16(v0, v1, hw[2 * q4], lw[2 * q4]);
             split_pair_f16(v2, v3, hw[2 * q4 + 1], lw[2 * q4 + 1]);
         };
@@ -904,12 +943,12 @@
 #pragma unroll
                 for (int i = 0; i < 6; ++i) {
                     FT_SGB(0x008, 1); FT_SGB(0x100, 1);
-                    if (st + 1 == C::NS && s >= C::NX3 / 2) { FT_SGB(0x002, 7); FT_SGB(0x040, 1); }
+                    if (st + 1 == C::NS && s >= C::NX3 / 2) { FT_SGB(0x002, 7); FT_SGB(0x040, C::LAT ? 2 : 1); }
                     else FT_SGB(0x002, 2);
                 }
             }
             __builtin_amdgcn_sched_barrier(0);
-            if (st + 1 == C::NS) FT_VMCNT(16);
+            if (st + 1 == C::NS) FT_VMCNT(C::EST);
             else FT_VMCNT(0);
             if (st + 2 == C::NS) tab_store(j);
             __syncthreads();
@@ -919,14 +958,14 @@
         e_perm(1, b_hi[0][1], b_lo[0][1]);
 #pragma unroll
         for (int u = 0; u < C::NU; ++u) {
-            const char* w1b = w1buf + eb * C::W1_BYTES + (half * C::MID + l31) * 16;
+            const char* w1b = w1buf + eb * C::W1_BYTES + (half * C::N1 + l31) * 16;
             f16x8 a_hi[3][2], a_lo[3][2], a_his[2][2];
             auto ld1 = [&](const int s, const int k) __attribute__((always_inline)) {
                 const int g = s / (C::MI1 / 2), mp = s % (C::MI1 / 2);
 #pragma unroll
                 for (int e = 0; e < 2; ++e) {
-                    a_hi[k][e] = *reinterpret_cast<const f16x8*>(w1b + (((g * 2 + 0) * 2) * C::MID + (2 * mp + e) * 32) * 16);
-                    a_lo[k][e] = *reinterpret_cast<const f16x8*>(w1b + (((g * 2 + 1) * 2) * C::MID + (2 * mp + e) * 32) * 16);
+                    a_hi[k][e] = *reinterpret_cast<const f16x8*>(w1b + (((g * 2 + 0) * 2) * C::N1 + (2 * mp + e) * 32) * 16);
+                    a_lo[k][e] = *reinterpret_cast<const f16x8*>(w1b + (((g * 2 + 1) * 2) * C::N1 + (2 * mp + e) * 32) * 16);
                 }
             };
             ld1(0, 0);
@@ -961,18 +1000,18 @@
                 const int g = s / (C::MI1 / 2), mp = s % (C::MI1 / 2);
                 mma6(acc1[2 * mp], acc1[2 * mp + 1], a_hi[s % 3], a_lo[s % 3], a_his[s & 1], b_hi[u & 1][g], b_lo[u & 1][g]);
 #pragma unroll
-                for (int i = 0; i < 6; ++i) { FT_SGB(0x008, 1); FT_SGB(0x100, 1); FT_SGB(0x002, 7 * C::SL); FT_SGB(0x040, C::SL); FT_SGB(0x020, 3); }
+                for (int i = 0; i < 6; ++i) { FT_SGB(0x008, 1); FT_SGB(0x100, 1); FT_SGB(0x002, 7 * C::SL); FT_SGB(0x040, C::SL * (C::LAT ? 2 : 1)); FT_SGB(0x020, 3); }
             }
             __builtin_amdgcn_sched_barrier(0);
-            if (u + 1 < C::NU) FT_VMCNT(DSV ? 16 : 32);
+            if (u + 1 < C::NU) FT_VMCNT(DSV ? C::EST : 16 + C::EST);
             else FT_VMCNT(DSV ? 0 : 16);
             __syncthreads();
             eb ^= 1;
         }
     }
-    static_assert(C::MID / 4 <= 64, "one lane per four channels");
-    if (wave < 2 && lane < C::MID / 4)
-        *reinterpret_cast<float4*>(w3buf + wave * (C::MID * 4) + lane * 16) = *reinterpret_cast<const float4*>((wave == 0 ? inv1 : p.b1) + lane * 4);
+    static_assert(C::N1 / 4 <= 64, "one lane per four channels");
+    if (wave < 2 && lane < C::N1 / 4)
+        *reinterpret_cast<float4*>(w3buf + wave * (C::N1 * 4) + lane * 16) = *reinterpret_cast<const float4*>((wave == 0 ? inv1 : p.b1) + lane * 4);
     __syncthreads();
     if (pos_ok) {
         const int hwp = p.dec_H * p.dec_W;
@@ -985,12 +1024,12 @@
             for (int q = 0; q < 4; ++q) {
                 const int co4 = m1 * 32 + 8 * q + 4 * half;
                 const float4 sc = *reinterpret_cast<const float4*>(ttab + co4);
-                const float4 bv = *reinterpret_cast<const float4*>(ttab + C::MID + co4);
+                const float4 bv = *reinterpret_cast<const float4*>(ttab + C::N1 + co4);
                 char* zo = reinterpret_cast<char*>(p.z + (int64_t)(m1 * 32 + 8 * q) * p.z_cs);
-                *reinterpret_cast<float*>(zo + (size_t)z_off) = relu_keep_nan(__fadd_rn(__fmul_rn(acc1[m1][4 * q + 0], sc.x), bv.x));
-                *reinterpret_cast<float*>(zo + p.z_cs * 4 + (size_t)z_off) = relu_keep_nan(__fadd_rn(__fmul_rn(acc1[m1][4 * q + 1], sc.y), bv.y));
-                *reinterpret_cast<float*>(zo + p.z_cs * 8 + (size_t)z_off) = relu_keep_nan(__fadd_rn(__fmul_rn(acc1[m1][4 * q + 2], sc.z), bv.z));
-                *reinterpret_cast<float*>(zo + p.z_cs * 12 + (size_t)z_off) = relu_keep_nan(__fadd_rn(__fmul_rn(acc1[m1][4 * q + 3], sc.w), bv.w));
+                *reinterpret_cast<float*>(zo + (size_t)z_off) = slot_act<C::LAT>(__fadd_rn(__fmul_rn(acc1[m1][4 * q + 0], sc.x), bv.x));
+                *reinterpret_cast<float*>(zo + p.z_cs * 4 + (size_t)z_off) = slot_act<C::LAT>(__fadd_rn(__fmul_rn(acc1[m1][4 * q + 1], sc.y), bv.y));
+                *reinterpret_cast<float*>(zo + p.z_cs * 8 + (size_t)z_off) = slot_act<C::LAT>(__fadd_rn(__fmul_rn(acc1[m1][4 * q + 2], sc.z), bv.z));
+                *reinterpret_cast<float*>(zo + p.z_cs * 12 + (size_t)z_off) = slot_act<C::LAT>(__fadd_rn(__fmul_rn(acc1[m1][4 * q + 3], sc.w), bv.w));
             }
     }
 }
@@ -1025,10 +1064,45 @@
     return STEMSEG_OK;
 }
 
+constexpr int FT_STAGE_END_TAG = 52;
+template <class C, class K>
+static int launch_stage_end_cfg(K kernel, const FusedTailParams& p, hipStream_t s) {
+    const double flops = 2.0 * ((double)C::MID + C::N1) * C::COUT * (double)p.V;
+    void* ev = profile_begin(FT_STAGE_END_TAG, flops, s);
+    hipLaunchKernelGGL(kernel, dim3((unsigned)ceil_div(p.V, C::P)), dim3(C::NTHREADS), 0, s, p);
+    profile_end(ev, s);
+    SS_LAUNCH_CHECK();
+    return STEMSEG_OK;
+}
+
 bool fused_tail_supported(int mid) { return mid == 64 || mid == 128 || mid == 256; }
 
 bool fused_shortcut_supported(int mid, int cin, int64_t V) {
     return ((mid == 64 && cin == 64) || (mid == 128 && cin == 256)) && (int64_t)cin * V * 4 < (1ll << 32) - (1 << 20) && (int64_t)128 * V * 4 < (1ll << 32) - (1 << 20);
+}
+
+bool fused_stage_end_supported(int mid, int64_t V) {
+    return (mid == 64 || mid == 128 || mid == 256) && V > 0 && V <= (1ll << 27) && (int64_t)128 * V * 4 < (1ll << 32) - (1 << 20);
+}
+
+int launch_fused_stage_end(int mid, const unsigned int* x16, const float* w3, const float* b3, const float* res, float* y, const float* wl, const float* bl,
+                           float* lat, float* xsub, int T, int h, int w, hipStream_t s) {
+    const int64_t V = (int64_t)T * h * w;
+    SS_CHECK_ARG(x16 && w3 && b3 && res && y && wl && bl && lat && xsub, "fused_stage_end: null pointer");
+    SS_CHECK_ARG(T > 0 && h > 0 && w > 0 && h % 2 == 0 && w % 2 == 0 && fused_stage_end_supported(mid, V), "fused_stage_end: mid = %d, %d planes of %d x %d (even)", mid, T, h, w);
+    SS_CHECK_ARG(reinterpret_cast<uintptr_t>(x16) % 16 == 0 && reinterpret_cast<uintptr_t>(w3) % 16 == 0 && reinterpret_cast<uintptr_t>(wl) % 16 == 0 &&
+                 reinterpret_cast<uintptr_t>(b3) % 16 == 0 && reinterpret_cast<uintptr_t>(bl) % 16 == 0, "fused_stage_end: 16-byte aligned operands");
+    FusedTailParams p;
+    p.x16 = x16; p.w3 = reinterpret_cast<const char*>(w3); p.b3 = b3; p.res = res; p.y = y;
+    p.w1 = reinterpret_cast<const char*>(wl); p.b1 = bl;
+    p.z = lat; p.z_cs = V; p.z_ts = (int64_t)h * w; p.z_ys = w; p.dec_H = h; p.dec_W = w;
+    p.V = (int)V;
+    p.xs = nullptr; p.wd = nullptr; p.bd = nullptr;
+    p.xsub = xsub; p.sub_V = (int)((int64_t)T * (h / 2) * (w / 2));
+    if (mid == 256) { using C = FusedTailR1Cfg<256, 128, 0, 256, true>; return launch_stage_end_cfg<C>(fused_tail_r1_kernel<C>, p, s); }
+    if (mid == 128) { using C = FusedTailR1Cfg<128, 128, 0, 256, true>; return launch_stage_end_cfg<C>(fused_tail_r1_kernel<C>, p, s); }
+    using C = FusedTailCfg<64, 64, 128, 0, 256, true>;
+    return launch_stage_end_cfg<C>(fused_tail_kernel<C>, p, s);
 }
 
 int launch_fused_tail(int mid, const unsigned int* x16, const float* w3, const float* b3, const float* res, float* y, const float* w1, const float* b1,
@@ -1049,6 +1123,7 @@
     p.z = z.ptr; p.z_cs = z.c_stride; p.z_ts = z.t_stride; p.z_ys = z.y_stride; p.dec_H = dec_H; p.dec_W = dec_W;
     p.V = (int)V;
     p.xs = ds_x; p.wd = reinterpret_cast<const char*>(ds_w); p.bd = ds_b;
+    p.xsub = nullptr; p.sub_V = 0;
     if (ds_x && mid == 128) return launch_fused_r1_cfg<FusedTailR1Cfg<128, 128, 256>>(p, s);
     if (ds_x) return launch_fused_cfg<FusedTailCfg<64, 128, 128, 64>>(p, s);
     if (mid == 256) {
diff --git a/stem-seg_amd/csrc/common.h b/stem-seg_amd/csrc/common.h
--- a/stem-seg_amd/csrc/common.h
+++ b/stem-seg_amd/csrc/common.h
@@ -102,6 +102,7 @@
     int64_t in_bs = 0, out_bs = 0, gn_bs = 0;
     unsigned int* p16_out = nullptr;
     int* p16_done = nullptr;
+    int p16_keep_plan = 0;
     int zero_t_halo = 0;
 };
 int launch_conv3d(const StemsegVolume& in, const float* packed_w, const float* bias, const StemsegVolume& out,
@@ -115,6 +116,9 @@
                       const float* ds_w = nullptr, const float* ds_b = nullptr);
 bool fused_shortcut_supported(int mid, int cin, int64_t V);
 int launch_gn_stats(const float* x, int C, int64_t S, int groups, float eps, float* stats, double* scratch, hipStream_t s);
+bool fused_stage_end_supported(int mid, int64_t V);
+int launch_fused_stage_end(int mid, const unsigned int* x16, const float* w3, const float* b3, const float* res, float* y, const float* wl, const float* bl,
+                           float* lat, float* xsub, int T, int h, int w, hipStream_t s);
 constexpr int GN_SLOT_CAP = 32768;
 static inline int64_t gn_scratch_doubles(int Cout, int groups) { return (int64_t)groups * GN_SLOT_CAP * 2 > (int64_t)groups * 128 ? (int64_t)groups * GN_SLOT_CAP * 2 : (int64_t)groups * 128; }
 int launch_conv3d_gn(const StemsegVolume& in, const float* packed_w, const float* bias, const StemsegVolume& out, int kt, int kh, int kw,
diff --git a/stem-seg_amd/csrc/conv_igemm.h b/stem-seg_amd/csrc/conv_igemm.h
--- a/stem-seg_amd/csrc/conv_igemm.h
+++ b/stem-seg_amd/csrc/conv_igemm.h
@@ -985,8 +985,9 @@
     float* scratch;
     int64_t scratch_floats;
     const PlanCtx* plan;
-    LaunchCtx without_scratch() const { return LaunchCtx{s, nullptr, 0, plan}; }
-    LaunchCtx without_plan() const { return LaunchCtx{s, scratch, scratch_floats, nullptr}; }
+    bool p16_keep_plan = false;
+    LaunchCtx without_scratch() const { return LaunchCtx{s, nullptr, 0, plan, p16_keep_plan}; }
+    LaunchCtx without_plan() const { return LaunchCtx{s, scratch, scratch_floats, nullptr, p16_keep_plan}; }
 };
 
 template <class C>
@@ -1012,7 +1013,7 @@
     const int64_t plan_scratch = plan ? plan->scratch_floats : L.scratch_floats / p.nb;
     const int64_t wg_target = (C::X6 && C::NWAVES >= 8) ? 320 : 640;
     while (scratch && ksplit * 2 <= 16 && ksplit * 2 <= nchunks && wgs * ksplit * 2 <= wg_target && slab_plan * ksplit * 2 <= plan_scratch) ksplit *= 2;
-    if (p.out_p16 && C::F16 && wgs >= 128) ksplit = 1;
+    if (p.out_p16 && C::F16 && wgs >= 128 && !L.p16_keep_plan) ksplit = 1;
     return ksplit;
 }
 
diff --git a/stem-seg_amd/csrc/conv_igemm.hip b/stem-seg_amd/csrc/conv_igemm.hip
--- a/stem-seg_amd/csrc/conv_igemm.hip
+++ b/stem-seg_amd/csrc/conv_igemm.hip
@@ -176,7 +176,7 @@
         pc = &pc_store;
     }
     const ConvKParams& d = pc ? pc->shape : p;
-    const LaunchCtx L{s, scratch, scratch_floats, pc};
+    const LaunchCtx L{s, scratch, scratch_floats, pc, epi && epi->p16_keep_plan};
     if (k4) return launch_stem_f16x3(p, L);
     if (prec == STEMSEG_PRECISION_BF16X6) return launch_split_family<2>(p, d, L, tile_cfg, k3, k2);
     if (prec == STEMSEG_PRECISION_F16X3) return launch_split_family<3>(p, d, L, tile_cfg, k3, k2);
diff --git a/stem-seg_amd/csrc/encoder.hip b/stem-seg_amd/csrc/encoder.hip
--- a/stem-seg_amd/csrc/encoder.hip
+++ b/stem-seg_amd/csrc/encoder.hip
@@ -353,6 +353,7 @@
     int h[4], w[4];
     int64_t V[4];
     int64_t S0, X1, A, B, Cst[4], M1[4], M2, DS, XS, L[4], FO[4], SK, SKfloats, total;
+    int64_t LAT[3];
     int64_t S2D, s2d_ts, s2d_pitch;
     int groups, s3, mid[4];
     int64_t M1S[4];
@@ -431,14 +432,43 @@
     p.plan_SKfloats = ENC_PLAN_SK_FLOATS;
     p.SKfloats = ENC_PLAN_SK_FLOATS * (d->plan_frames > 0 ? std::max<int64_t>(1, ceil_div(d->T, d->plan_frames)) : 1);
     p.SK = take(p.SKfloats);
+    p.LAT[0] = p.S0;
+    p.LAT[1] = p.X1;
+    p.LAT[2] = take(256 * p.V[2]);
     p.total = off;
     SS_CHECK_ARG(!p.guards.full, "encoder: the plan has more than %d workspace slices (GuardList)", WS_MAX_GUARDS);
     return STEMSEG_OK;
 }
 
+static int stage_end_mask(const StemsegEncoderDesc* d, const EncoderPlan& p) {
+    int mask = 0;
+    for (int k = 0; k < 3; ++k) {
+        const int h = p.h[k], w = p.w[k], mid = p.mid[k];
+        bool ok = ((d->fuse_tail >> k) & 1) && !((d->fuse_tail >> (6 + k)) & 1) && d->precision == STEMSEG_PRECISION_F16X3 && p.groups == 1 && !p.s3 &&
+                  mid * 4 == (256 << k) && p.nblk[k] >= 2 && fused_stage_end_supported(mid, p.V[k]) && (int64_t)p.T * (h + 2) * (w + 4) <= (1ll << 27);
+        Padded2D gf0(256, p.T, h, w);
+        const unsigned gq0 = (unsigned)((w + 1) / 4 + 1);
+        ok = ok && h % 2 == 0 && w % 4 == 0 && p.h[k + 1] == h / 2 && p.w[k + 1] == w / 2 && gf0.pitch % 4 == 0 && (int64_t)4 * gq0 <= gf0.pitch &&
+             (int64_t)256 * p.T * (h / 2 + 1) * gq0 < (1ll << 32) - 256 && gf0.ts % 4 == 0;
+        const int64_t v_plan = p.plan_frames > 0 ? p.V[k] / p.T * p.plan_frames : p.V[k];
+        ok = ok && ceil_div(v_plan, 256) >= 128;
+        if (ok) mask |= 1 << k;
+    }
+    return mask;
+}
+
 }
 
 using namespace stemseg;
+
+extern "C" int stemseg_hip_encoder_stage_end_mask(const StemsegEncoderDesc* desc, int32_t* mask_out) {
+    EncoderPlan p;
+    int rc = make_encoder_plan(desc, p);
+    if (rc) return rc;
+    SS_CHECK_ARG(mask_out, "encoder_stage_end_mask: null pointer");
+    *mask_out = stage_end_mask(desc, p);
+    return STEMSEG_OK;
+}
 
 extern "C" size_t stemseg_hip_encoder_workspace_bytes(const StemsegEncoderDesc* desc) {
     EncoderPlan p;
@@ -560,6 +590,10 @@
     float* x = ws + p.X1;
     int cin = 64, bi = 0;
     bool conv1_done = false;
+    const int end_mask = stage_end_mask(desc, p);
+    bool lat_ok[3], end_done[3] = {false, false, false};
+    for (int k = 0; k < 3; ++k)
+        lat_ok[k] = ((end_mask >> k) & 1) && reinterpret_cast<uintptr_t>(ws + p.L[k]) % 16 == 0 && reinterpret_cast<uintptr_t>(ws + p.LAT[k]) % 16 == 0;
     for (int st = 0; st < 4; ++st) {
         const int mid = p.mid[st], cout = 256 << st, h = p.h[st], w = p.w[st];
         const int64_t V = p.V[st];
@@ -571,7 +605,9 @@
                          "encoder_forward: null weights for block %d", bi);
             SS_CHECK_ARG(!first || (wts->down_w[bi] && wts->down_b[bi]), "encoder_forward: block %d needs a projection shortcut", bi);
             float* xin = x;
-            if (stride2) {
+            if (stride2 && end_done[st - 1]) {
+                xin = ws + p.XS;
+            } else if (stride2) {
                 void* ev = profile_begin(49, 4.0 * 2.0 * (double)cin * V, s);
                 const int64_t ss_items = (int64_t)cin * T * h * (w / 4);
                 if (w % 4 == 0 && ss_items < (1ll << 31))
@@ -595,6 +631,7 @@
             }
             const bool want_fuse = ((desc->fuse_tail >> st) & 1) && prec == STEMSEG_PRECISION_F16X3 && b + 1 < p.nblk[st] && !grouped && p.groups == 1 &&
                                    mid * 4 == cout && fused_tail_supported(mid) && V <= (1ll << 27) && (int64_t)T * (h + 2) * (w + 4) <= (1ll << 27);
+            const bool want_end = st < 3 && b + 1 == p.nblk[st] && lat_ok[st];
             int p16_done = 0;
             if (grouped) {
                 rc = launch_grouped_conv(halo2d_view(m1, mid, T, h1, w1), wts->conv2_w[bi], wts->conv2_b[bi], dense_volume(ws + p.M2, mid, T, h, w), p.groups,
@@ -603,6 +640,7 @@
                 ConvEpilogue e2 = epi_for(T);
                 e2.relu = 1;
                 if (want_fuse) { e2.p16_out = reinterpret_cast<unsigned int*>(ws + p.M2); e2.p16_done = &p16_done; }
+                if (want_end) { e2.p16_out = reinterpret_cast<unsigned int*>(ws + p.M2); e2.p16_done = &p16_done; e2.p16_keep_plan = 1; }
                 rc = launch_conv3d(halo2d_view(m1, mid, T, h, w), wts->conv2_w[bi], wts->conv2_b[bi], dense_volume(ws + p.M2, mid, T, h, w), 1, 3, 3, 0, s,
                                    ws + p.SK, p.SKfloats, &e2);
             }
@@ -624,6 +662,12 @@
                                        ds_in_tail ? xin : nullptr, cin, ds_in_tail ? wts->down_w[bi] : nullptr, ds_in_tail ? wts->down_b[bi] : nullptr);
                 if (rc) return rc;
                 conv1_done = true;
+            } else if (want_end && p16_done) {
+                rc = launch_fused_stage_end(mid, reinterpret_cast<const unsigned int*>(ws + p.M2), wts->conv3_w[bi], wts->conv3_b[bi], idt, y, wts->fpn_inner_w[st],
+                                            wts->fpn_inner_b[st], ws + p.LAT[st], ws + p.XS, T, h, w, s);
+                if (rc) return rc;
+                end_done[st] = true;
+                conv1_done = false;
             } else {
                 ConvEpilogue e3 = epi_for(T);
                 e3.relu = 1; e3.res = idt; e3.res_cs = V; e3.res_ts = 0; e3.res_ys = 0;
@@ -644,15 +688,19 @@
         const bool lat_dense = k < 3 && h % 2 == 0 && w % 4 == 0 && p.h[k + 1] == h / 2 && p.w[k + 1] == w / 2 && gf0.pitch % 4 == 0 &&
                                (int64_t)4 * gq0 <= gf0.pitch && (int64_t)256 * T * (h / 2 + 1) * gq0 < (1ll << 32) - 256 &&
                                (reinterpret_cast<uintptr_t>(ws + p.L[k]) % 16 == 0) && gf0.ts % 4 == 0 && (reinterpret_cast<uintptr_t>(ws + p.A) % 16 == 0);
-        if (lat_dense) {
-            ConvEpilogue ed = epi_for(T);
-            rc = launch_conv3d(flat_view(ws + p.Cst[k], 256 << k, p.V[k]), wts->fpn_inner_w[k], wts->fpn_inner_b[k], flat_view(ws + p.A, 256, p.V[k]), 1, 1, 1, 0, s,
-                               ws + p.SK, p.SKfloats, &ed);
-            if (rc) return rc;
+        const bool lat_stored = k < 3 && end_done[k];
+        const float* lat_map = lat_stored ? ws + p.LAT[k] : ws + p.A;
+        if (lat_dense || lat_stored) {
+            if (!lat_stored) {
+                ConvEpilogue ed = epi_for(T);
+                rc = launch_conv3d(flat_view(ws + p.Cst[k], 256 << k, p.V[k]), wts->fpn_inner_w[k], wts->fpn_inner_b[k], flat_view(ws + p.A, 256, p.V[k]), 1, 1, 1, 0, s,
+                                   ws + p.SK, p.SKfloats, &ed);
+                if (rc) return rc;
+            }
             Padded2D gc0(256, T, p.h[k + 1], p.w[k + 1]);
             void* ev = profile_begin(50, 4.0 * 256.0 * (2.0 * p.V[k] + p.V[k + 1]), s);
             const int64_t items = (int64_t)256 * T * (h / 2 + 1) * gq0;
-            hipLaunchKernelGGL(upsample2x_add_dense_vec4x2_kernel, dim3((unsigned)ceil_div(items, 256)), dim3(256), 0, s, ws + p.L[k], (const float*)(ws + p.A),
+            hipLaunchKernelGGL(upsample2x_add_dense_vec4x2_kernel, dim3((unsigned)ceil_div(items, 256)), dim3(256), 0, s, ws + p.L[k], lat_map,
                                (const float*)(ws + p.L[k + 1] + gc0.interior), h, w, gq0, (unsigned)items, gf0.ts, (int)gf0.pitch, gc0.ts, (int)gc0.pitch);
             profile_end(ev, s);
             SS_LAUNCH_CHECK();
@@ -661,7 +709,7 @@
                            ws + p.SK, p.SKfloats, &e);
         if (rc) return rc;
         }
-        if (k < 3 && !lat_dense) {
+        if (k < 3 && !lat_dense && !lat_stored) {
             Padded2D gf(256, T, h, w), gc(256, T, p.h[k + 1], p.w[k + 1]);
             void* ev = profile_begin(50, 4.0 * 256.0 * (2.0 * p.V[k] + p.V[k + 1]), s);
             const unsigned gq = (unsigned)((w + 1) / 4 + 1);
diff --git a/stem-seg_amd/stemseg_amd/hip.py b/stem-seg_amd/stemseg_amd/hip.py
--- a/stem-seg_amd/stemseg_amd/hip.py
+++ b/stem-seg_amd/stemseg_amd/hip.py
@@ -100,6 +100,7 @@
     "stemseg_hip_padded_geometry": (C.c_int, [_I32, _I32, _I32, _I32, C.POINTER(_I64)]),
     "stemseg_hip_pack_conv_weight": (C.c_int, [_P, _P, _I32, _I32, _I32, _P]),
     "stemseg_hip_encoder_plan_offsets": (C.c_int, [_P, _P]),
+    "stemseg_hip_encoder_stage_end_mask": (C.c_int, [_P, C.POINTER(_I32)]),
     "stemseg_hip_packed_weight_bytes_prec": (C.c_int64, [_I32, _I32, _I32, _I32]),
     "stemseg_hip_pack_conv_weight_prec": (C.c_int, [_P, _P, _I32, _I32, _I32, _I32, _P]),
     "stemseg_hip_conv3d": (C.c_int, [C.POINTER(Volume), _P, _P, C.POINTER(Volume), _I32, _I32, _I32, _I32, _P, _I64, C.POINTER(ConvEpilogue), _P]),
@@ -231,7 +232,7 @@
     check(lib().stemseg_hip_profile_enable(int(on)))
 
 
-PROFILE_CONV_TAGS = {"conv3x3x3": (9, 8, 4, 2), "conv1x3x3": (36, 28, 27, 24, 22), "conv1x1x1": (18, 17, 14, 16, 12, 19)}
+PROFILE_CONV_TAGS = {"conv3x3x3": (9, 8, 4, 2), "conv1x3x3": (36, 28, 27, 24, 22), "conv1x1x1": (18, 17, 14, 16, 12, 19, 52)}
 PROFILE_HBM_TAGS = {40: "upsample_trilinear", 41: "gn_stats (partial + finalize)", 42: "gn_relu (apply)", 43: "gn_relu_pool (apply + AvgPool3d)",
                     44: "heads", 45: "fg_gather (count + scan + scatter)", 46: "cluster (all rounds + final)", 47: "stem_conv7x7",
                     48: "maxpool3x3s2", 49: "subsample2", 50: "upsample2x_add (FPN top-down)"}
```

After: 126.3, median of 6. 1.2% higher.
